# linnanwang/FastGen

Hardware: AMD Instinct MI355X
Metric: images/sec at 4-step distilled (DMD2) sampling (higher is better)
Workload: dtype fp32 (tensors, accumulate) with split-bf16 x3 MFMA conv products; 1 GPU; EDM CIFAR-10 32x32 SongUNet (55.7M params) DMD2 4-step 'sde' sampling, batch=512 per GPU; global_batch=512, sample_steps=4, parallelism=replicas x1 (no data-path collective), graph=True

## Files before the change

### fastgen_amd/_lib.py

```python
import ctypes
import os
from ctypes import POINTER, c_char_p, c_double, c_float, c_int, c_int64, c_size_t, c_uint64, c_void_p

_HERE = os.path.dirname(os.path.abspath(__file__))
LIB_PATH = os.path.join(_HERE, "libfastgen_amd.so")

FG_MAX_LEVELS = 8
FG_DTYPE_F32, FG_DTYPE_BF16, FG_DTYPE_BF16X3, FG_DTYPE_FP8 = 0, 1, 2, 3
DTYPE_NAMES = {"fp32": FG_DTYPE_F32, "bf16": FG_DTYPE_BF16, "bf16x3": FG_DTYPE_BF16X3, "fp8": FG_DTYPE_FP8}
FG_SAMPLE_SDE, FG_SAMPLE_ODE = 0, 1
SAMPLE_TYPES = {"sde": FG_SAMPLE_SDE, "ode": FG_SAMPLE_ODE}
FG_LOOP_X0, FG_LOOP_MEANFLOW, FG_LOOP_EULER = 0, 1, 2
LOOP_KINDS = {"x0": FG_LOOP_X0, "meanflow": FG_LOOP_MEANFLOW, "euler": FG_LOOP_EULER}
FG_SCHEDULE_EDM, FG_SCHEDULE_RF = 0, 1
FG_DROP_PRECOND_INPUT, FG_DROP_PRECOND_OUTPUT = 1, 2
FG_BWD_DECODER, FG_BWD_ENCODER, FG_BWD_EMBED = 1, 2, 4
FG_MODEL_SONGUNET, FG_MODEL_DHARIWAL = 0, 1
(FG_TRAIN_OP_HEAD_GRAD, FG_TRAIN_OP_STEM_OPERAND, FG_TRAIN_OP_INPUT_GRAD, FG_TRAIN_OP_ADD_NCHW_TO_NHWC, FG_TRAIN_OP_SILU_BWD, FG_TRAIN_OP_JVP_COEF,
 FG_TRAIN_OP_JVP_EMBED, FG_TRAIN_OP_JVP_INPUT, FG_TRAIN_OP_JVP_OUTPUT) = range(9)


class fg_edm_config(ctypes.Structure):
    _fields_ = [
        ("img_resolution", c_int), ("img_channels", c_int), ("label_dim", c_int), ("augment_dim", c_int),
# ... 16 lines not shown


class fg_dit_config(ctypes.Structure):
    _fields_ = [("input_size", c_int), ("patch_size", c_int), ("in_channels", c_int), ("hidden_size", c_int), ("depth", c_int),
                ("num_heads", c_int), ("mlp_hidden", c_int), ("embedding_rows", c_int), ("r_timestep", c_int), ("compute_dtype", c_int)]


class fg_wan_config(ctypes.Structure):
    _fields_ = [("num_heads", c_int), ("head_dim", c_int), ("in_channels", c_int), ("out_channels", c_int), ("text_dim", c_int),
                ("freq_dim", c_int), ("ffn_dim", c_int), ("num_layers", c_int), ("rope_max_seq_len", c_int), ("chunk_size", c_int),
                ("total_num_frames", c_int), ("eps", c_float), ("compute_dtype", c_int)]


class fg_wan_ext_config(ctypes.Structure):
    _fields_ = [("r_timestep", c_int), ("time_cond_diff", c_int)]


class fg_wan_i2v_config(ctypes.Structure):
    _fields_ = [("latent_channels", c_int), ("mask_channels", c_int), ("image_dim", c_int)]


class fg_wan_ti2v_config(ctypes.Structure):
    _fields_ = [("latent_channels", c_int)]


class fg_wan_vace_config(ctypes.Structure):
    _fields_ = [("vace_in_channels", c_int), ("num_vace_layers", c_int), ("vace_layers", c_int * 64)]


class fg_wan_block_taps(ctypes.Structure):
    _fields_ = [("attn1", c_void_p), ("x_attn1", c_void_p), ("attn2", c_void_p), ("x_attn2", c_void_p), ("x_ffn", c_void_p)]


class fg_dit_sampler_config(ctypes.Structure):
    _fields_ = [("t_scale", c_double), ("guidance_scale", c_double), ("use_sit_convention", c_int), ("time_cond_diff", c_int),
                ("net_pred_flow", c_int), ("schedule", c_int)]


class fg_wan_sampler_config(ctypes.Structure):
    _fields_ = [("t_scale", c_double), ("context_noise", c_double), ("net_pred_flow", c_int), ("schedule", c_int), ("prefill_frames", c_int)]


class fg_wan_guided_sampler_config(ctypes.Structure):
    _fields_ = [("t_scale", c_double), ("context_noise", c_double), ("guidance", c_int)]


class fg_attention_plan(ctypes.Structure):
    _fields_ = [("kernel", c_int), ("nsplit", c_int), ("t_cut", c_int), ("sample_major", c_int), ("refusal", c_int), ("grid", c_int64),
                ("scratch_bytes", c_size_t)]


class fg_edm_conv_plan(ctypes.Structure):
    _fields_ = [("kernel", c_int), ("stat_slots", c_int)]


FG_EDM_PACK_GENERIC, FG_EDM_PACK_WS, FG_EDM_PACK_X3WS, FG_EDM_PACK_X3SUB = range(4)
FG_EDM_CONV_GENERIC, FG_EDM_CONV_WS, FG_EDM_CONV_X3WS = 1, 2, 3
FG_EDM_PACK_STEM, FG_EDM_PACK_AUX = 0, 1


class fg_gemm_plan(ctypes.Structure):
    _fields_ = [("refusal", c_int), ("kernel", c_int), ("tile_n", c_int), ("epilogue", c_int), ("ksplit", c_int), ("xn", c_int), ("grid", c_int),
                ("lds_bytes", c_int), ("row0", c_int), ("rows", c_int), ("pieces", c_int)]


FG_FA_TILE128, FG_FA_TILE128_W3, FG_FA_TILE128_REG, FG_FA_WIDE, FG_FA_WIDE_CUT, FG_FA_SEQ72, FG_FA_TILE72, FG_FA_TILE72_W3 = range(1, 9)
FG_FA_REFUSE_ARG, FG_FA_REFUSE_OFFSET, FG_FA_REFUSE_PATH = 1, 2, 3
FG_GEMM_REG, FG_GEMM_PP, FG_GEMM_PP_NARROW, FG_GEMM_PP_SPLITK = range(1, 5)
FG_GEMM_EPI_TOK, FG_GEMM_EPI_HEADS, FG_GEMM_EPI_RAW, FG_GEMM_EPI_TOK32, FG_GEMM_EPI_SPLIT, FG_GEMM_EPI_HEADS32 = range(6)
FG_GEMM_REFUSE_ARG, FG_GEMM_REFUSE_OFFSET, FG_GEMM_REFUSE_FORM, FG_GEMM_REFUSE_PIECE = 1, 2, 3, 4


SIGNATURES = {
    "fg_last_error": (c_char_p, []),
    "fg_version": (c_char_p, []),
    "fg_graph_stats": (None, [POINTER(c_uint64), POINTER(c_uint64)]),
    "fg_edm_create": (c_int, [POINTER(fg_edm_config), POINTER(c_void_p)]),
    "fg_edm_destroy": (None, [c_void_p]),
    "fg_edm_num_params": (c_int, [c_void_p]),
    "fg_edm_param_info": (c_int, [c_void_p, c_int, POINTER(c_char_p), POINTER(c_int), POINTER(c_int64)]),
    "fg_edm_bind_param": (c_int, [c_void_p, c_char_p, c_void_p, c_int64]),
    "fg_edm_pack_weights": (c_int, [c_void_p, c_void_p]),
    "fg_edm_workspace_bytes": (c_size_t, [c_void_p, c_int]),
    "fg_edm_forward": (c_int, [c_void_p, c_void_p, c_void_p, c_void_p, c_void_p, c_void_p, c_void_p, c_int, c_void_p,
                               c_size_t, c_void_p]),
    "fg_edm_num_feature_taps": (c_int, [c_void_p]),
    "fg_edm_feature_info": (c_int, [c_void_p, c_int, POINTER(c_char_p), POINTER(c_int), POINTER(c_int)]),
    "fg_edm_forward_features": (c_int, [c_void_p, c_void_p, c_void_p, c_void_p, c_void_p, c_void_p, POINTER(c_void_p), c_int,
                                        c_void_p, c_size_t, c_void_p]),
    "fg_sampler_run": (c_int, [c_void_p, c_void_p, c_void_p, POINTER(c_double), c_int, c_int, c_int, c_void_p, c_uint64,
                               c_void_p, c_int, c_void_p, c_size_t, c_int, c_void_p]),
    "fg_edm_t_list": (c_int, [c_int, POINTER(c_double)]),
    "fg_rf_t_list": (c_int, [c_int, POINTER(c_double)]),
    "fg_edm_profile_begin": (c_int, [c_void_p]),
    "fg_edm_profile_end": (c_int, [c_void_p, POINTER(c_int64), POINTER(c_double), POINTER(c_double)]),
    "fg_edm_num_blocks": (c_int, [c_void_p]),
    "fg_edm_block_info": (c_int, [c_void_p, c_int, POINTER(c_char_p), POINTER(c_int), POINTER(c_int), POINTER(c_int),
                                  POINTER(c_int), POINTER(c_int)]),
    "fg_edm_run_block": (c_int, [c_void_p, c_int, c_void_p, c_int, c_void_p, c_int, c_void_p, c_void_p, c_int, c_void_p,
                                 c_size_t, c_void_p]),
    "fg_op_gn_coeffs": (c_int, [c_void_p, c_int, c_void_p, c_int, c_void_p, c_void_p, c_float, c_void_p, c_int, c_int, c_void_p]),
    "fg_op_adm_conv_pack_bytes": (c_size_t, [c_int, c_int, c_int, c_int]),
    "fg_op_adm_conv_pack": (c_int, [c_int, c_void_p, c_void_p, c_int, c_int, c_int, c_void_p]),
    "fg_op_adm_conv": (c_int, [c_int, c_int, c_void_p, c_int, c_void_p, c_int, c_int, c_int, c_int, c_int, c_void_p, c_int, c_void_p,
                               c_void_p, c_void_p, c_int, c_void_p, c_int, c_void_p]),
    "fg_op_adm_conv_ex": (c_int, [c_int, c_int, c_void_p, c_int, c_void_p, c_int, c_int, c_int, c_int, c_int, c_void_p, c_int, c_int, c_void_p,
# ... 130 lines not shown
    "fg_wan_create_ti2v": (c_int, [POINTER(fg_wan_config), POINTER(fg_wan_ext_config), POINTER(fg_wan_ti2v_config), POINTER(c_void_p)]),
    "fg_wan_set_first_frame": (c_int, [c_void_p, c_void_p, c_int, c_int, c_int, c_void_p]),
    "fg_wan_first_frame_read": (c_int, [c_void_p, c_void_p, c_void_p]),
    "fg_wan_create_vace": (c_int, [POINTER(fg_wan_config), POINTER(fg_wan_ext_config), POINTER(fg_wan_vace_config), POINTER(c_void_p)]),
    "fg_wan_set_vace_scale": (c_int, [c_void_p, POINTER(c_float), c_int, c_void_p]),
    "fg_wan_vace_context_workspace_bytes": (c_size_t, [c_void_p, c_int, c_int, c_int, c_int]),
    "fg_wan_set_vace_context": (c_int, [c_void_p, c_void_p, c_int, c_int, c_int, c_int, c_int, c_void_p, c_size_t, c_void_p]),
    "fg_wan_vace_context_read": (c_int, [c_void_p, c_void_p, c_void_p]),
    "fg_op_wan_vace_patch_embed": (c_int, [c_void_p, c_void_p, c_void_p, c_void_p, c_int, c_int, c_int, c_int, c_int, c_int, c_int, c_void_p]),
    "fg_op_wan_patch_embed": (c_int, [c_void_p, c_void_p, c_void_p, c_void_p, c_void_p, c_int, c_int, c_int, c_int, c_int, c_int, c_int, c_void_p]),
    "fg_op_wan_final": (c_int, [c_void_p, c_void_p, c_void_p, c_void_p, c_void_p, c_void_p, c_int, c_int, c_int, c_int, c_int, c_int, c_float, c_int,
                                c_void_p]),
    "fg_op_wan_dual_cross_attention": (c_int, [c_void_p, c_int, c_int64, c_void_p, c_void_p, c_int, c_int64, c_int, c_void_p, c_void_p, c_int,
                                               c_int64, c_int, c_void_p, c_int, c_int64, c_int, c_int, c_int, c_void_p]),
    "fg_disc_edm_num_params": (c_int, [c_int]),
    "fg_disc_edm_workspace_bytes": (c_size_t, [c_int, c_int]),
    "fg_disc_edm_run": (c_int, [c_void_p, c_int, c_void_p, c_void_p, c_void_p, c_void_p, c_void_p, c_int, c_void_p, c_size_t, c_void_p]),
    "fg_edm_jvp": (c_int, [c_void_p, c_void_p, c_void_p, c_void_p, c_void_p, c_void_p, c_void_p, c_void_p, c_void_p, c_void_p, c_int,
                           c_void_p, c_size_t, c_void_p]),
    "fg_edm_set_dropout": (c_int, [c_void_p, c_float, c_uint64]),
    "fg_op_gn_workspace_bytes": (c_size_t, [c_int, c_int]),
    "fg_op_gn_act": (c_int, [c_int, c_int, c_void_p, c_int, c_void_p, c_int, c_void_p, c_void_p, c_float, c_void_p, c_int, c_int, c_int,
                             c_float, ctypes.c_uint32, c_uint64, c_void_p, c_size_t, c_void_p]),
    "fg_op_gn_backward": (c_int, [c_int, c_int, c_void_p, c_int, c_void_p, c_int, c_void_p, c_int, c_void_p, c_void_p, c_float, c_void_p,
                                  c_void_p, c_void_p, c_int, c_float, c_void_p, c_void_p, c_int, c_int, c_int, c_int, c_float,
                                  ctypes.c_uint32, c_uint64, c_void_p, c_size_t, c_void_p]),
    "fg_op_gn_jvp": (c_int, [c_int, c_int, c_void_p, c_int, c_void_p, c_int, c_void_p, c_void_p, c_void_p, c_float, c_void_p, c_int, c_int,
                             c_float, ctypes.c_uint32, c_uint64, c_void_p, c_size_t, c_void_p]),
    "fg_op_attention_backward_workspace_bytes": (c_size_t, [c_int, c_int, c_int, c_int]),
    "fg_op_attention_backward": (c_int, [c_int, c_void_p, c_void_p, c_void_p, c_void_p, c_void_p, c_void_p, c_void_p, c_void_p, c_int, c_int,
                                         c_int, c_void_p, c_size_t, c_void_p]),
    "fg_op_attention_jvp": (c_int, [c_int, c_void_p, c_void_p, c_void_p, c_void_p, c_void_p, c_void_p, c_void_p, c_int, c_int, c_int,
                                    c_void_p, c_size_t, c_void_p]),
    "fg_op_colsum": (c_int, [c_int, c_void_p, c_int, c_int, c_void_p, c_int, c_int, c_float, c_int, c_void_p]),
    "fg_op_batchsum_add": (c_int, [c_void_p, c_void_p, c_void_p, c_int, c_int, c_int, c_void_p]),
    "fg_op_linear_backward": (c_int, [c_int, c_void_p, c_void_p, c_void_p, c_void_p, c_void_p, c_void_p, c_int, c_int, c_int, c_float, c_int,
                                      c_void_p]),
    "fg_op_dgrad_weights": (c_int, [c_void_p, c_void_p, c_int, c_int, c_int, c_int, c_void_p]),
    "fg_op_train_elementwise": (c_int, [c_int, c_int, c_void_p, c_void_p, c_void_p, c_void_p, c_void_p, c_void_p, c_int, c_int, c_int, c_int,
                                        c_double, c_double, c_int, c_void_p]),
    "fg_op_edm_conv_pack_bytes": (c_size_t, [c_int, c_int, c_int, c_int, c_int]),
    "fg_op_edm_conv_pack": (c_int, [c_int, c_int, c_void_p, c_void_p, c_int, c_int, c_int, c_int, c_void_p]),
    "fg_op_edm_conv_plan": (c_int, [c_int, c_int, c_int, c_int, c_int, c_int, c_int, c_int, c_int, c_int, c_int, c_int, c_int,
                                    POINTER(fg_edm_conv_plan)]),
    "fg_op_edm_conv": (c_int, [c_int, c_int, c_int, c_int, c_int, c_void_p, c_int, c_void_p, c_int, c_int, c_int, c_int, c_void_p, c_void_p,
                               c_void_p, c_void_p, c_void_p, c_int, c_void_p, c_int, c_float, c_void_p, c_int, c_void_p, c_void_p, c_void_p,
                               c_void_p, c_void_p]),
    "fg_op_edm_gn_finalize": (c_int, [c_void_p, c_int, c_int, c_void_p, c_int, c_int, c_void_p, c_void_p, c_float, c_void_p, c_void_p, c_int,
                                      c_int, c_void_p]),
    "fg_op_edm_gn_silu_pool": (c_int, [c_int, c_void_p, c_void_p, c_void_p, c_int, c_int, c_int, c_void_p]),
    "fg_op_edm_attention": (c_int, [c_int, c_void_p, c_void_p, c_void_p, c_void_p, c_int, c_int, c_void_p]),
    "fg_op_edm_attn_merge_weights": (c_int, [c_void_p, c_void_p, c_void_p, c_void_p, c_void_p, c_int, c_void_p]),
    "fg_op_edm_attention_merged": (c_int, [c_void_p, c_void_p, c_void_p, c_void_p, c_void_p, c_float, c_void_p, c_void_p, c_int, c_void_p]),
    "fg_op_edm_head_pack_bytes": (c_size_t, [c_int, c_int, c_int]),
    "fg_op_edm_stem": (c_int, [c_int, c_void_p, c_void_p, c_void_p, c_void_p, c_void_p, c_void_p, c_void_p, c_int, c_int, c_int, c_void_p]),
    "fg_op_edm_conv_in": (c_int, [c_int, c_void_p, c_void_p, c_void_p, c_void_p, c_void_p, c_int, c_int, c_int, c_int, c_void_p]),
    "fg_op_edm_aux_head": (c_int, [c_int, c_void_p, c_void_p, c_void_p, c_void_p, c_void_p, c_void_p, c_void_p, c_void_p, c_int, c_int, c_int,
                                   c_void_p]),
    "fg_op_edm_aux_out": (c_int, [c_int, c_void_p, c_void_p, c_void_p, c_void_p, c_void_p, c_void_p, c_void_p, c_int, c_int, c_int, c_int,
                                  c_void_p]),
    "fg_op_dropout_mask": (c_int, [c_void_p, c_int64, c_float, ctypes.c_uint32, c_uint64, c_void_p]),
    "fg_edm_set_augment": (c_int, [c_void_p, c_void_p]),
    "fg_edm_set_training": (c_int, [c_void_p, c_int]),
    "fg_op_images_to_u8": (c_int, [c_void_p, c_void_p, c_int64, c_int, c_int, c_int, c_void_p]),
    "fg_op_randn": (c_int, [c_void_p, c_int64, c_uint64, c_uint64, c_void_p]),
    "fg_op_attention": (c_int, [c_void_p, c_void_p, c_void_p, c_void_p, c_int, c_int, c_int, c_int, c_int, c_void_p]),
    "fg_op_attention_split": (c_int, [c_void_p, c_void_p, c_void_p, c_void_p, c_int, c_int, c_int, c_int, c_int, c_int, c_void_p]),
    "fg_op_attention_plan": (c_int, [c_int, c_int, c_int, c_int, c_int, c_int, c_int, c_int, c_int, POINTER(fg_attention_plan)]),
    "fg_op_attention_ex": (c_int, [c_void_p, c_int, c_int64, c_void_p, c_void_p, c_int, c_int64, c_void_p, c_int, c_int64, c_int, c_int, c_int,
                                   c_int, c_int, c_int, c_int, c_int, c_void_p]),
    "fg_op_dit_attention": (c_int, [c_int, c_void_p, c_void_p, c_void_p, c_void_p, c_int, c_int, c_int, c_int, c_size_t, c_int, c_void_p]),
    "fg_op_gemm_plan": (c_int, [c_int, c_int, c_int, c_int, c_int, c_int, c_size_t, c_int, c_int, c_int, c_int, POINTER(fg_gemm_plan)]),
    "fg_op_gemm_bf16": (c_int, [c_void_p, c_void_p, c_void_p, c_void_p, c_int, c_int, c_int, c_int, c_void_p, c_int, c_int, c_void_p,
                                c_int, c_void_p]),
    "fg_op_quant_rows_fp8": (c_int, [c_int, c_void_p, c_void_p, c_void_p, c_int64, c_int, c_void_p]),
    "fg_op_gemm_fp8": (c_int, [c_void_p, c_void_p, c_void_p, c_void_p, c_int, c_int, c_int, c_int, c_void_p, c_int, c_int, c_void_p,
                               c_int, c_void_p, c_void_p, c_void_p]),
    "fg_op_dit_ln_modulate_fp8": (c_int, [c_void_p, c_void_p, c_int, c_int, c_int, c_void_p, c_void_p, c_int, c_int, c_int, c_void_p]),
    "fg_op_gemm_x3": (c_int, [c_void_p, c_void_p, c_void_p, c_void_p, c_int, c_int, c_int, c_int, c_void_p, c_int, c_int, c_void_p,
                              c_int, c_void_p]),
}

_lib = None


def lib():
    global _lib
    if _lib is None:
        if not os.path.exists(LIB_PATH):
            raise RuntimeError(
                f"{LIB_PATH} not found: build it with `python -c 'import __graft_entry__ as g; g.build()'` "
                "(or `make -C fastgen_amd/csrc`).  fastgen_amd has no non-HIP fallback.")
        L = ctypes.CDLL(LIB_PATH)
        for name, (res, args) in SIGNATURES.items():
            fn = getattr(L, name)
            fn.restype = res
            fn.argtypes = args
        _lib = L
    return _lib


def graph_stats():
    c, n = c_uint64(), c_uint64()
    lib().fg_graph_stats(ctypes.byref(c), ctypes.byref(n))
    return c.value, n.value

# ... 10 lines not shown
```

### fastgen_amd/csrc/attn.hip

```cpp
#include <cstdlib>
#include "common.h"
#include "misc.h"

namespace {

template <typename T>
struct PFrag;
template <>
struct PFrag<__bf16> {
    static __device__ __forceinline__ Frag8<__bf16> make(const f32x16& p, int s) {
        Frag8<__bf16> f;
#pragma unroll
        for (int j = 0; j < 8; ++j) f.v[j] = (__bf16)p[8 * s + j];
        return f;
    }
};
template <>
struct PFrag<float> {
    static __device__ __forceinline__ Frag8<float> make(const f32x16& p, int s) {
        Frag8<float> f;
        f.lo = f32x4{p[8 * s + 0], p[8 * s + 1], p[8 * s + 2], p[8 * s + 3]};
        f.hi = f32x4{p[8 * s + 4], p[8 * s + 5], p[8 * s + 6], p[8 * s + 7]};
        return f;
    }
// ... 225 lines not shown
#pragma unroll
            for (int j = 0; j < 8; ++j) pf[kt][s2].v[j] = (__bf16)(st[kt][8 * s2 + j] * inv);
        __builtin_amdgcn_sched_barrier(0);
    }

    __builtin_amdgcn_sched_barrier(0);
    __bf16* obase = out + ((size_t)n * Tn + q0) * D + r;
#pragma unroll 1
    for (int dg = 0; dg < 2; ++dg) {
        f32x16 o[4];
#pragma unroll
        for (int d = 0; d < 4; ++d)
#pragma unroll
            for (int i = 0; i < 16; ++i) o[d][i] = 0.f;
        asm volatile("" ::: "memory");
        stage_v(0, smem);
        __syncthreads();
#pragma unroll
        for (int t = 0; t < 4; ++t) {
            const char* cur = smem + (t & 1) * ATT_BUF;
            if (t + 1 < 4) stage_v(t + 1, smem + ((t + 1) & 1) * ATT_BUF);
#pragma unroll
            for (int sub = 0; sub < 2; ++sub)
#pragma unroll
                for (int s2 = 0; s2 < 2; ++s2)
#pragma unroll
                    for (int d = 0; d < 4; ++d) {
                        const char* p = cur + ((dg * 4 + d) * 32 + r) * VPITCH + (sub * 32 + 16 * s2 + 4 * h) * 2;
                        const bf16x4 lo = *reinterpret_cast<const bf16x4*>(p);
                        const bf16x4 hi = *reinterpret_cast<const bf16x4*>(p + 16);
                        Frag8<__bf16> vf;
                        vf.v = bf16x8{lo[0], lo[1], lo[2], lo[3], hi[0], hi[1], hi[2], hi[3]};
                        mma16(o[d], pf[t * 2 + sub][s2], vf);
                    }
            __syncthreads();
            __builtin_amdgcn_sched_barrier(0);
        }
#pragma unroll
        for (int d = 0; d < 4; ++d)
#pragma unroll
            for (int i = 0; i < 16; ++i) obase[(size_t)acc_row(i, h) * D + (dg * 4 + d) * 32] = (__bf16)o[d][i];
    }
}

constexpr int X3_KP = 272, X3_VP = 136;
constexpr int X3_PLANE = 64 * X3_KP;
constexpr int X3_BUF = 2 * X3_PLANE;

struct AttnMerge {
    const float2* ab;
    const float* bp;
    float2* stats;
    float scale;
};

template <bool MRG>
__global__ __launch_bounds__(256, 2) void attention_x3_lds_kernel(const float* __restrict__ q, const float* __restrict__ k,
                                                                  const float* __restrict__ vt, float* __restrict__ out, int B,
                                                                  AttnMerge mg) {
    constexpr int Tn = 256, D = 256;
    extern __shared__ __attribute__((aligned(16))) char smem[];
    const int tid = threadIdx.x, lane = tid & 63, wave = tid >> 6;
    const int r = lane & 31, h = lane >> 5;
    const int n = blockIdx.x >> 1;
    const int q0 = (blockIdx.x & 1) * 128 + wave * 32;

    auto stage_k = [&](int s, char* buf) {
        const float* src = k + ((size_t)n * Tn + (s & 3) * 64) * D + (s >> 2) * 128;
        f32x4 cf[4];
        if constexpr (MRG) {
            const f32x4* cp = reinterpret_cast<const f32x4*>(mg.ab + (size_t)n * D + (s >> 2) * 128 + (tid & 15) * 8);
#pragma unroll
            for (int j = 0; j < 4; ++j) cf[j] = cp[j];
        }
#pragma unroll
        for (int b2 = 0; b2 < 2; ++b2) {
#pragma unroll
            for (int i = b2 * 2; i < b2 * 2 + 2; ++i) {
                const int idx = tid + 256 * i, row = idx >> 4, c = idx & 15;
                float x[8];
                widen8(load_frag(src + (size_t)row * D + c * 8), x);
                if constexpr (MRG) {
#pragma unroll
                    for (int j = 0; j < 8; ++j) x[j] = fmaf(x[j], cf[j >> 1][2 * (j & 1)], cf[j >> 1][2 * (j & 1) + 1]);
                }
                bf16x8 hi, lo;
                split8(x, hi, lo);
                *reinterpret_cast<bf16x8*>(buf + row * X3_KP + c * 16) = hi;
                *reinterpret_cast<bf16x8*>(buf + X3_PLANE + row * X3_KP + c * 16) = lo;
            }
            __builtin_amdgcn_sched_barrier(0);
        }
    };
    auto stage_v = [&](int s, char* buf) {
        const float* src = vt + ((size_t)n * D + (s >> 2) * 128) * Tn + (s & 3) * 64;
#pragma unroll
        for (int b2 = 0; b2 < 2; ++b2) {
#pragma unroll
            for (int i = b2 * 2; i < b2 * 2 + 2; ++i) {
                const int idx = tid + 256 * i, row = idx >> 3, c = idx & 7;
                float x[8];
                widen8(load_frag(src + (size_t)row * Tn + c * 8), x);
                bf16x8 hi, lo;
                split8(x, hi, lo);
                bf16x4* dh = reinterpret_cast<bf16x4*>(buf + row * X3_VP + c * 16);
                dh[0] = bf16x4{hi[0], hi[1], hi[2], hi[3]};
// ... 70 lines not shown
    }

    float* obase = out + ((size_t)n * Tn + q0) * D + r;
    stage_v(0, smem);
    __syncthreads();
    f32x16 o[4];
#pragma unroll
    for (int s = 0; s < 8; ++s) {
        const char* cur = smem + (s & 1) * X3_BUF;
        if ((s & 3) == 0) {
#pragma unroll
            for (int d = 0; d < 4; ++d)
#pragma unroll
                for (int i = 0; i < 16; ++i) o[d][i] = 0.f;
        }
        if (s + 1 < 8) stage_v(s + 1, smem + ((s + 1) & 1) * X3_BUF);
#pragma unroll
        for (int sub = 0; sub < 2; ++sub)
#pragma unroll
            for (int s2 = 0; s2 < 2; ++s2)
#pragma unroll
                for (int d = 0; d < 4; ++d) {
                    const char* p = cur + (d * 32 + r) * X3_VP + (sub * 32 + 16 * s2 + 4 * h) * 2;
                    const bf16x4 a0 = *reinterpret_cast<const bf16x4*>(p), a1 = *reinterpret_cast<const bf16x4*>(p + 16);
                    const bf16x4 b0 = *reinterpret_cast<const bf16x4*>(p + X3_PLANE), b1 = *reinterpret_cast<const bf16x4*>(p + X3_PLANE + 16);
                    Frag8<bf16x3> vf;
                    vf.hi = bf16x8{a0[0], a0[1], a0[2], a0[3], a1[0], a1[1], a1[2], a1[3]};
                    vf.lo = bf16x8{b0[0], b0[1], b0[2], b0[3], b1[0], b1[1], b1[2], b1[3]};
                    mma16(o[d], pf[(s & 3) * 2 + sub][s2], vf);
                }
        __syncthreads();
        __builtin_amdgcn_sched_barrier(0);
        if ((s & 3) == 3) {
            if constexpr (MRG) {
                const float* xbase = k + ((size_t)n * Tn + q0) * D + r;
#pragma unroll
                for (int d = 0; d < 4; ++d) {
                    const int col = ((s >> 2) * 4 + d) * 32;
                    const float bias = mg.bp[col + r];
                    float sv = 0.f, qv = 0.f;
#pragma unroll
                    for (int i = 0; i < 16; ++i) {
                        const size_t off = (size_t)acc_row(i, h) * D + col;
                        const float v = (o[d][i] + bias + xbase[off]) * mg.scale;
                        obase[off] = v;
                        sv += v;
                        qv += v * v;
                    }
                    if (mg.stats) {
                        sv += __shfl_xor(sv, 32), qv += __shfl_xor(qv, 32);
                        sv += __shfl_xor(sv, 1), qv += __shfl_xor(qv, 1);
                        sv += __shfl_xor(sv, 2), qv += __shfl_xor(qv, 2);
                        if (h == 0 && (r & 3) == 0)
                            mg.stats[((size_t)n * 8 + (blockIdx.x & 1) * 4 + wave) * (D / 4) + ((col + r) >> 2)] = make_float2(sv, qv);
                    }
                }
            } else {
#pragma unroll
                for (int d = 0; d < 4; ++d)
#pragma unroll
                    for (int i = 0; i < 16; ++i) obase[(size_t)acc_row(i, h) * D + ((s >> 2) * 4 + d) * 32] = o[d][i];
            }
        }
    }
}

__global__ void attn_merge_weights_kernel(const float* __restrict__ qkv_w, const float* __restrict__ qkv_b, const float* __restrict__ proj_w,
                                          float* __restrict__ w_out, float* __restrict__ b_out, int C) {
    const int o = blockIdx.x % C;
    const bool val = blockIdx.x >= C;
    for (int i = threadIdx.x; i <= C; i += blockDim.x) {
        double acc = 0.0;
        for (int c = 0; c < C; ++c) {
            const double l = val ? proj_w[(size_t)o * C + c] : qkv_w[(size_t)(3 * c + 1) * C + o];
            const int row = 3 * c + (val ? 2 : 0);
            acc += l * (double)(i < C ? qkv_w[(size_t)row * C + i] : qkv_b[row]);
        }
        if (i < C)
            w_out[(size_t)blockIdx.x * C + i] = (float)acc;
        else
            b_out[blockIdx.x] = (float)acc;
    }
}

template <bool MRG>
int x3_lds_prepare() {
    static bool done[16] = {};
    const int dev = fg_device_slot();
    if (dev < 0) return (int)hipErrorInvalidDevice;
    if (!done[dev]) {
        hipError_t e = hipFuncSetAttribute(reinterpret_cast<const void*>(attention_x3_lds_kernel<MRG>), hipFuncAttributeMaxDynamicSharedMemorySize, 2 * X3_BUF);
        if (e != hipSuccess) return (int)e;
        done[dev] = true;
    }
    return 0;
}

}

int launch_attn_merge_weights(const float* qkv_w, const float* qkv_b, const float* proj_w, float* w_out, float* b_out, int C, hipStream_t s) {
    hipLaunchKernelGGL(attn_merge_weights_kernel, dim3(2 * C), dim3(256), 0, s, qkv_w, qkv_b, proj_w, w_out, b_out, C);
    return (int)hipGetLastError();
}

int launch_attention_merged(const float* qm, const float* x_mid, const float2* ab, const float* vmt, const float* bp, float scale, float* out,
                            float2* stats, int B, hipStream_t s) {
    const int rc = x3_lds_prepare<true>();
    if (rc || !qm) return rc;
    hipLaunchKernelGGL(attention_x3_lds_kernel<true>, dim3(B * 2), dim3(256), 2 * X3_BUF, s, qm, x_mid, vmt, out, B, AttnMerge{ab, bp, stats, scale});
    return (int)hipGetLastError();
}

int launch_attention(int dtype, const void* q, const void* k, const void* vt, void* out, int B, int T, hipStream_t s) {
    if (T != 256 && T != 64) return (int)hipErrorInvalidValue;
    const int nt = T / 32;
    const int waves = B * nt;
    dim3 grid((waves + 3) / 4), block(256);
    if (dtype == 1 && nt == 8) {
        static bool attr_done_dev[16] = {};
        const int dev = fg_device_slot();
        if (dev < 0) return (int)hipErrorInvalidDevice;
        bool& attr_done = attr_done_dev[dev];
        if (!attr_done) {
            hipError_t e = hipFuncSetAttribute(reinterpret_cast<const void*>(attention_lds_kernel), hipFuncAttributeMaxDynamicSharedMemorySize, 2 * ATT_BUF);
            if (e != hipSuccess) return (int)e;
            attr_done = true;
        }
        if (!q) return 0;
        hipLaunchKernelGGL(attention_lds_kernel, dim3(B * 2), block, 2 * ATT_BUF, s, (const __bf16*)q, (const __bf16*)k, (const __bf16*)vt, (__bf16*)out, B);
        return (int)hipGetLastError();
    }
    static const bool x3_lds = [] {
        const char* e = getenv("FASTGEN_AMD_ATTN_X3_LDS");
        return !(e && e[0] == '0');
    }();
    if (dtype == 2 && nt == 8 && x3_lds) {
        const int rc = x3_lds_prepare<false>();
        if (rc || !q) return rc;
        hipLaunchKernelGGL(attention_x3_lds_kernel<false>, dim3(B * 2), block, 2 * X3_BUF, s, (const float*)q, (const float*)k, (const float*)vt, (float*)out, B,
                           AttnMerge{});
        return (int)hipGetLastError();
    }
    if (!q) return 0;
    if (dtype == 2) {
        if (nt == 8)
            hipLaunchKernelGGL((attention_kernel<bf16x3, 8>), grid, block, 0, s, (const float*)q, (const float*)k, (const float*)vt, (float*)out, B);
        else
            hipLaunchKernelGGL((attention_kernel<bf16x3, 2>), grid, block, 0, s, (const float*)q, (const float*)k, (const float*)vt, (float*)out, B);
    } else if (dtype) {
        if (nt == 8)
            hipLaunchKernelGGL((attention_kernel<__bf16, 8>), grid, block, 0, s, (const __bf16*)q, (const __bf16*)k, (const __bf16*)vt, (__bf16*)out, B);
        else
            hipLaunchKernelGGL((attention_kernel<__bf16, 2>), grid, block, 0, s, (const __bf16*)q, (const __bf16*)k, (const __bf16*)vt, (__bf16*)out, B);
    } else {
        if (nt == 8)
            hipLaunchKernelGGL((attention_kernel<float, 8>), grid, block, 0, s, (const float*)q, (const float*)k, (const float*)vt, (float*)out, B);
        else
            hipLaunchKernelGGL((attention_kernel<float, 2>), grid, block, 0, s, (const float*)q, (const float*)k, (const float*)vt, (float*)out, B);
    }
    return (int)hipGetLastError();
}
```

### fastgen_amd/csrc/conv.h

```cpp
#pragma once
#include <hip/hip_runtime.h>

struct ConvArgs {
    const void* src1;
    const void* src2;
    int C1, C2;
    int Hs, Ws;
    int H, W;
    int B;
    const float2* ab;
    const void* wpack;
    const void* wpack_ws;
    const float* bias;
    const float* temb;
    int temb_stride;
    const void* resid;
    int rshift = 0;
    float scale;
    void* out;
    int Cout;
    float2* stats;
    int dbg;
    void* q_out;
    void* k_out;
    void* vt_out;
    const float* gate = nullptr;
    int gate_stride = 0;
    int act = 0;
    int heads = 0, head_dim = 0;
    size_t heads_lo_off = 0;
};

enum { PRO_NONE = 0, PRO_GN = 1, PRO_GN_SILU = 2 };
enum { RES_NONE = 0, RES_DOWN = 1, RES_UP = 2, RES_SUBPIX = 3 };
enum { OUT_NHWC = 0, OUT_QKV = 1, OUT_TOK = 2, OUT_HEADS = 3, OUT_QV = 4 };

int launch_conv_fused(int dtype, int ks, int pro, int res, int outmode, const ConvArgs& a, hipStream_t stream);
int conv_stat_slots(int W);
bool conv_ws_supported(int dtype, int ks, int pro, int res, int outmode, const ConvArgs& a);
bool conv_ws_enabled();
int launch_conv_ws(int res, const ConvArgs& a, hipStream_t stream, bool prepare_only, int pro = PRO_GN_SILU);
bool conv_ws_shape_ok(int dtype, int cout, int cin, int res);
int launch_pack_conv_weights_ws(const float* w_oihw, void* wpack_ws, int cout, int cin, hipStream_t stream);
bool conv_x3ws_supported(int ks, int pro, int res, int outmode, const ConvArgs& a);
bool conv_x3ws_shape_ok(int cout, int cin, int res);
int conv_x3ws_stat_slots(int W, int res);
int launch_conv_x3ws(int res, const ConvArgs& a, hipStream_t stream, bool prepare_only, int pro = PRO_GN_SILU);
int launch_pack_conv_weights_x3ws(const float* w_oihw, void* wpack_ws, int cout, int cin, hipStream_t stream);
int launch_pack_conv_weights_x3sub(const float* w_oihw, void* wpack_sub, int cout, int cin, hipStream_t stream);
int conv_subpix_mode();
int conv_launch_stat_slots(int dtype, int ks, int pro, int res, int outmode, const ConvArgs& a);
int launch_conv_ws_debug(const ConvArgs& a, int abl, hipStream_t stream);
int launch_conv_debug(int dtype, const ConvArgs& a, hipStream_t stream);
int conv_prepare_all(int dtype);
size_t conv_pack_elems(int cout, int cin, int ks);
int launch_pack_conv_weights(int dtype, const float* w_oihw, void* wpack, int cout, int cin, int ks, int qkv_perm,
                             hipStream_t stream);
```

### fastgen_amd/csrc/conv.hip

```cpp
#include "common.h"
#include "conv.h"
#include <stdlib.h>
#include <string.h>

#include <type_traits>

namespace {

constexpr int PITCH = 144;
constexpr int NTHR = 256;

template <int KS, int LOGW>
struct Geom {
    static constexpr int W = 1 << LOGW;
    static constexpr int LOGTW = (LOGW == 5) ? 4 : LOGW;
    static constexpr int TW = 1 << LOGTW;
    static constexpr int LOGTH = 3;
    static constexpr int TH = 1 << LOGTH;
    static constexpr int IMGS = 128 / (TH * TW);
    static constexpr int TCOLS = W / TW;
    static constexpr int TPI = (IMGS > 1) ? 1 : (W / TH) * TCOLS;
    static constexpr int PAD = KS / 2;
    static constexpr int HW_ = TW + 2 * PAD;
    static constexpr int HH_ = TH + 2 * PAD;
// ... 535 lines not shown
        if (res == RES_NONE) return launch_w<T, 3, PRO_GN_SILU, RES_NONE, OUT_NHWC>(a, s);
        if (res == RES_UP) return launch_w<T, 3, PRO_GN_SILU, RES_UP, OUT_NHWC>(a, s);
    }
    if (ks == 3 && pro == PRO_NONE && res == RES_NONE) return launch_w<T, 3, PRO_NONE, RES_NONE, OUT_NHWC>(a, s);
    if (ks == 1 && pro == PRO_NONE) {
        if (res == RES_NONE) return launch_w<T, 1, PRO_NONE, RES_NONE, OUT_NHWC>(a, s);
        if (res == RES_DOWN) return launch_w<T, 1, PRO_NONE, RES_DOWN, OUT_NHWC>(a, s);
        if (res == RES_UP) return launch_w<T, 1, PRO_NONE, RES_UP, OUT_NHWC>(a, s);
    }
    return (int)hipErrorInvalidValue;
}

int dispatch_t(int dtype, int ks, int pro, int res, int outmode, const ConvArgs& a, hipStream_t s) {
    switch (dtype) {
        case 0: return launch_t<float>(ks, pro, res, outmode, a, s);
        case 1: return launch_t<__bf16>(ks, pro, res, outmode, a, s);
        case 2: return launch_t<bf16x3>(ks, pro, res, outmode, a, s);
    }
    return (int)hipErrorInvalidValue;
}

}

int launch_conv_debug(int dtype, const ConvArgs& a, hipStream_t stream) {
    if (dtype != 1 || a.W != 32) return (int)hipErrorInvalidValue;
    g_debug_extra_lds = (a.dbg & 16) ? 48 * 1024 : 0;
    switch (a.dbg & 15) {
        case 0: return launch_one<__bf16, 3, PRO_GN_SILU, RES_NONE, 5, OUT_NHWC, 0>(a, stream);
        case 1: return launch_one<__bf16, 3, PRO_GN_SILU, RES_NONE, 5, OUT_NHWC, 1>(a, stream);
        case 2: return launch_one<__bf16, 3, PRO_GN_SILU, RES_NONE, 5, OUT_NHWC, 2>(a, stream);
        case 3: return launch_one<__bf16, 3, PRO_GN_SILU, RES_NONE, 5, OUT_NHWC, 3>(a, stream);
        case 4: return launch_one<__bf16, 3, PRO_GN_SILU, RES_NONE, 5, OUT_NHWC, 4>(a, stream);
        case 5: return launch_one<__bf16, 3, PRO_GN_SILU, RES_NONE, 5, OUT_NHWC, 5>(a, stream);
        case 6: return launch_one<__bf16, 3, PRO_GN_SILU, RES_NONE, 5, OUT_NHWC, 6>(a, stream);
        case 7: return launch_one<__bf16, 3, PRO_GN_SILU, RES_NONE, 5, OUT_NHWC, 7>(a, stream);
    }
    return (int)hipErrorInvalidValue;
}

int launch_conv_fused(int dtype, int ks, int pro, int res, int outmode, const ConvArgs& a, hipStream_t stream) {
    const int kc = dtype == 1 ? DT<__bf16>::KC : DT<float>::KC;
    if (a.H != a.W || (a.W != 8 && a.W != 16 && a.W != 32)) return (int)hipErrorInvalidValue;
    const bool tok = outmode == OUT_TOK || outmode == OUT_HEADS;
    if ((a.C1 % kc) || (a.C2 % kc) || (a.Cout % (tok ? 64 : 256)) || a.B <= 0) return (int)hipErrorInvalidValue;
    if (outmode == OUT_HEADS && (a.heads <= 0 || (a.head_dim % 4) || a.Cout != 3 * a.heads * a.head_dim || ((a.heads * a.head_dim) % 64) ||
                                 !a.q_out || !a.k_out || !a.vt_out))
        return (int)hipErrorInvalidValue;
    if (res == RES_NONE && (a.Hs != a.H || a.Ws != a.W)) return (int)hipErrorInvalidValue;
    if (res == RES_DOWN && (a.Hs != 2 * a.H || a.Ws != 2 * a.W)) return (int)hipErrorInvalidValue;
    if ((res == RES_UP || res == RES_SUBPIX) && (2 * a.Hs != a.H || 2 * a.Ws != a.W)) return (int)hipErrorInvalidValue;
    if (pro != PRO_NONE && !a.ab) return (int)hipErrorInvalidValue;
    if (outmode == OUT_QKV && (a.Cout != 768 || a.W > 16)) return (int)hipErrorInvalidValue;
    if (outmode == OUT_QV && (a.Cout != 512 || a.W != 16 || dtype != 2 || !a.q_out || !a.vt_out)) return (int)hipErrorInvalidValue;
    if (conv_ws_enabled() && conv_ws_supported(dtype, ks, pro, res, outmode, a)) return launch_conv_ws(res, a, stream, false, pro);
    if (dtype == 2 && conv_ws_enabled() && conv_x3ws_supported(ks, pro, res, outmode, a)) return launch_conv_x3ws(res, a, stream, false, pro);
    if (res == RES_SUBPIX || a.rshift) return (int)hipErrorInvalidValue;
    return dispatch_t(dtype, ks, pro, res, outmode, a, stream);
}

bool conv_ws_enabled() {
    static const bool on = [] {
        const char* e = getenv("FASTGEN_AMD_CONV_WS");
        return !(e && e[0] == '0');
    }();
    return on;
}

int conv_subpix_mode() {
    static const int mode = [] {
        const char* e = getenv("FASTGEN_AMD_CONV_SUBPIX");
        if (e && e[0] == '0') return 0;
        return (e && !strcmp(e, "skip")) ? 1 : 2;
    }();
    return mode;
}

int conv_launch_stat_slots(int dtype, int ks, int pro, int res, int outmode, const ConvArgs& a) {
    if (dtype == 2 && conv_ws_enabled() && conv_x3ws_supported(ks, pro, res, outmode, a)) return conv_x3ws_stat_slots(a.W, res);
    return conv_stat_slots(a.W);
}

int conv_stat_slots(int W) { return W == 32 ? Geom<3, 5>::TPI : (W == 16 ? Geom<3, 4>::TPI : Geom<3, 3>::TPI); }

int conv_prepare_all(int dtype) {
    g_prepare_only = true;
    int rc = 0;
    ConvArgs a{};
    a.B = 1;
    a.Cout = 256;
    const int ws[3] = {8, 16, 32};
    for (int wi = 0; wi < 3 && !rc; ++wi) {
        a.W = a.H = ws[wi];
        for (int res = 0; res < 3 && !rc; ++res) {
            if (res != RES_DOWN)
                rc = dispatch_t(dtype, 3, PRO_GN_SILU, res, OUT_NHWC, a, nullptr);
            if (!rc) rc = dispatch_t(dtype, 1, PRO_NONE, res, OUT_NHWC, a, nullptr);
        }
        if (!rc) rc = dispatch_t(dtype, 3, PRO_NONE, RES_NONE, OUT_NHWC, a, nullptr);
        if (!rc && a.W <= 16) rc = dispatch_t(dtype, 1, PRO_GN, RES_NONE, OUT_QKV, a, nullptr);
        if (!rc && a.W == 16 && dtype == 2) rc = dispatch_t(dtype, 1, PRO_GN, RES_NONE, OUT_QV, a, nullptr);
        if (!rc && a.W == 16) rc = dispatch_t(dtype, 1, PRO_NONE, RES_NONE, OUT_TOK, a, nullptr);
        if (!rc && a.W == 16) rc = dispatch_t(dtype, 1, PRO_NONE, RES_NONE, OUT_HEADS, a, nullptr);
    }
    g_prepare_only = false;
    if (!rc && dtype == 2) {
        ConvArgs w{};
        for (int res : {RES_NONE, RES_UP})
            for (int ww : {32, 16, 8}) {
                if (ww == 8 && res != RES_NONE) continue;
                w.W = w.H = ww;
                if (!rc) rc = launch_conv_x3ws(res, w, nullptr, true, PRO_GN_SILU);
                if (!rc && res == RES_NONE) rc = launch_conv_x3ws(res, w, nullptr, true, PRO_NONE);
            }
        for (int ws_ : {16, 8}) {
            w.Ws = w.Hs = ws_;
            w.W = w.H = 2 * ws_;
            if (!rc) rc = launch_conv_x3ws(RES_SUBPIX, w, nullptr, true, PRO_GN_SILU);
        }
    }
    if (!rc && dtype == 1) {
        ConvArgs w{};
        for (int res : {RES_NONE, RES_UP}) {
            w.W = w.H = 32;
            if (!rc) rc = launch_conv_ws(res, w, nullptr, true);
            if (res == RES_NONE) {
                w.C1 = -128;
                if (!rc) rc = launch_conv_ws(res, w, nullptr, true);
                w.C1 = 0;
            }
            w.W = w.H = 16;
            if (!rc) rc = launch_conv_ws(res, w, nullptr, true);
        }
// ... 19 lines not shown
```

### fastgen_amd/csrc/conv_ws3.hip

```cpp
#include "common.h"
#include "conv.h"

namespace {

constexpr int X3_NTHR = 768;
constexpr int X3_KC = 32;
constexpr int X3_PA = 16;
constexpr int X3_PLANE = 3072;
constexpr int X3_ABUF = 8 * X3_PLANE;
constexpr int X3_RING = 4;
constexpr int X3_HOFF = 128 * 512;
constexpr int X3_LDS = X3_HOFF + X3_RING * X3_ABUF;
constexpr int X3_TAPB = 2048;

template <int LOGW>
struct X3Geom {
    static constexpr int W = 1 << LOGW;
    static constexpr int TW = 16, TH = 8;
    static constexpr int IPT = LOGW == 3 ? 2 : 1;
    static constexpr int TCOLS = LOGW == 3 ? 1 : W / TW;
    static constexpr int TPI = LOGW == 3 ? 1 : (W / TH) * TCOLS;
    static constexpr int HW_ = LOGW == 3 ? 2 * W + 3 : TW + 2, HH_ = TH + 2;
    static constexpr int HALO_PIX = HW_ * HH_;
    static constexpr int RS = HW_ * X3_PA;
    static_assert(HALO_PIX * X3_PA <= X3_PLANE && HALO_PIX <= 192, "one halo plane; three producer passes of 64 pixels");
};

__device__ __forceinline__ void x3_barrier() {
    asm volatile("s_waitcnt lgkmcnt(0)\n\ts_barrier" ::: "memory");
}

struct X3Frag {
    bf16x8 hi, lo;
};

template <int RES, int LOGW, int PRO>
__global__ __launch_bounds__(X3_NTHR) void conv3_x3ws_kernel(const ConvArgs a, const int ntiles) {
    using G = X3Geom<LOGW>;
    constexpr bool SUB = RES == RES_SUBPIX;
    constexpr int NTAP = SUB ? 4 : 9;
    constexpr int RN = SUB ? 4 : 3;
    constexpr int NQ = 4 * NTAP;
    constexpr int X3_STEPB = NTAP * X3_TAPB;
    extern __shared__ __attribute__((aligned(16))) char smem[];
    char* const hbuf = smem;
    char* const ring = smem + X3_HOFF;

    const int tid = threadIdx.x;
    const int lane = tid & 63;
    const int wave = __builtin_amdgcn_readfirstlane(tid >> 6);
    const int Cin = a.C1 + a.C2;
    const int nchunk = Cin / X3_KC;
    const int G8 = (int)gridDim.x >> 3;
    const int wg = ((gridDim.x & 7) == 0) ? ((int)blockIdx.x & 7) * G8 + ((int)blockIdx.x >> 3) : (int)blockIdx.x;
    const int gstride = (int)gridDim.x;
    const int my_tiles = (ntiles - wg + gstride - 1) / gstride;
    const int S = my_tiles * nchunk;
    const int NSTEP = S + 3;
    const int H = SUB ? a.Hs : a.H;

    if (wave < 8) {
        const int grp = wave >> 2, wl = wave & 3;
        const int col = lane & 15, g4 = lane >> 4;
        const size_t wstride = (size_t)nchunk * NTAP * 1024;
        const __amdgpu_buffer_rsrc_t wrs = __builtin_amdgcn_make_buffer_rsrc(
            const_cast<__bf16*>(reinterpret_cast<const __bf16*>(a.wpack_ws) + (size_t)(grp * 8 + wl * 2) * wstride), 0, 0x7fffffff,
            0x00020000);
        const int wvoff = lane * 16;
        const int wsb = (int)(wstride * 2);
        const int wphb = SUB ? 16 * wsb : 0;
        int tcur = wg;
        auto load_w = [&](int byte_off) -> X3Frag {
            X3Frag f;
            f.hi = __builtin_bit_cast(bf16x8, __builtin_amdgcn_raw_buffer_load_b128(wrs, wvoff, byte_off, 0));
            f.lo = __builtin_bit_cast(bf16x8, __builtin_amdgcn_raw_buffer_load_b128(wrs, wvoff, byte_off + 1024, 0));
            return f;
        };
        X3Frag wq[RN][2];
#pragma unroll
        for (int j = 0; j < RN; ++j)
#pragma unroll
            for (int nt = 0; nt < 2; ++nt) wq[j][nt] = load_w((tcur & 3) * wphb + nt * wsb + (SUB ? j : 3 * j) * X3_TAPB);

        f32x4 acc[8][2];
#pragma unroll
        for (int m = 0; m < 8; ++m)
#pragma unroll
            for (int nt = 0; nt < 2; ++nt) acc[m][nt] = f32x4{0.f, 0.f, 0.f, 0.f};

// ... 178 lines not shown
            off2[i] = (pix * (unsigned)a.C2 + oct * 8) * 4u;
        }
        abn = a.ab + (size_t)n * Cin;
    };
    auto stage_load = [&](Staged& st, int t, int c32) __attribute__((always_inline)) {
        if (c32 == 0) tile_setup(t);
        const bool first = c32 * X3_KC < a.C1;
        const char* base = first ? reinterpret_cast<const char*>(src1) + c32 * (X3_KC * 4)
                                 : reinterpret_cast<const char*>(src2) + (c32 * X3_KC - a.C1) * 4;
#pragma unroll
        for (int i = 0; i < 3; ++i) {
            const char* p = base + (first ? off1[i] : off2[i]);
            st.raw[i][0] = *reinterpret_cast<const f32x4*>(p);
            st.raw[i][1] = *reinterpret_cast<const f32x4*>(p + 16);
        }
        if (PRO == PRO_NONE) return;
        const float2* p = abn + c32 * X3_KC + oct * 8;
#pragma unroll
        for (int j = 0; j < 8; j += 2) {
            const f32x4 q = *reinterpret_cast<const f32x4*>(p + j);
            st.ab[j] = make_float2(q[0], q[1]);
            st.ab[j + 1] = make_float2(q[2], q[3]);
        }
    };
    auto stage_store = [&](const Staged& st, char* abuf) __attribute__((always_inline)) {
#pragma unroll
        for (int i = 0; i < 3; ++i) {
            float v[8];
#pragma unroll
            for (int j = 0; j < 8; ++j) {
                v[j] = st.raw[i][j >> 2][j & 3];
                if (PRO != PRO_NONE) v[j] = silu_f<true>(fmaf(v[j], st.ab[j].x, st.ab[j].y));
            }
            bf16x8 hi, lo;
            split8(v, hi, lo);
            typedef __attribute__((ext_vector_type(4))) unsigned u32x4;
            u32x4 wh = __builtin_bit_cast(u32x4, hi), wl_ = __builtin_bit_cast(u32x4, lo);
#pragma unroll
            for (int j = 0; j < 4; ++j) {
                wh[j] = valid[i] ? wh[j] : 0u;
                wl_[j] = valid[i] ? wl_[j] : 0u;
            }
            if (i < 2 || third) {
                *reinterpret_cast<u32x4*>(abuf + hlds[i]) = wh;
                *reinterpret_cast<u32x4*>(abuf + hlds[i] + 4 * X3_PLANE) = wl_;
            }
        }
    };

    const int chq = lane & 31, psub = lane >> 5;
    float* const out = reinterpret_cast<float*>(a.out);
    const float* const resid = reinterpret_cast<const float*>(a.resid);
    const bool has_resid = __builtin_amdgcn_readfirstlane(resid != nullptr);
    auto retire_half = [&](int t, int half) __attribute__((always_inline)) {
        int n, slot, row0, col0;
        tile_coord(t, n, slot, row0, col0);
        const int co = half * 128 + chq * 4;
        const int nimg = G::IPT == 2 ? min(2, a.B - n) : 1;
        f32x4 radd[G::IPT];
#pragma unroll
        for (int k = 0; k < G::IPT; ++k) {
            radd[k] = f32x4{0.f, 0.f, 0.f, 0.f};
            if (a.bias) radd[k] = *reinterpret_cast<const f32x4*>(a.bias + co);
            const int nk = G::IPT == 2 ? min(n + k, a.B - 1) : n;
            if (a.temb) radd[k] += *reinterpret_cast<const f32x4*>(a.temb + (size_t)nk * a.temb_stride + co);
            radd[k] *= a.scale;
        }
        constexpr int OW = SUB ? 2 * G::W : G::W, OST = SUB ? 2 : 1;
        const int ph = t & 3;
        const size_t tb = SUB ? (((size_t)n * (2 * H) + 2 * row0 + (ph >> 1)) * OW + 2 * col0 + (ph & 1)) * 256 + co
                              : (((size_t)n * H + row0) * G::W + col0) * 256 + co;
        const int rs = (SUB || G::IPT == 2) ? 0 : a.rshift;
        const size_t rtb = (SUB || G::IPT == 2) ? tb : (((size_t)n * (H >> rs) + (row0 >> rs)) * (G::W >> rs) + (col0 >> rs)) * 256 + co;
        float ssum[G::IPT] = {}, ssq[G::IPT] = {};
#pragma unroll 1
        for (int grp8 = 0; grp8 < 2; ++grp8) {
            f32x4 rr[8], dv[8];
            unsigned go[8];
#pragma unroll
            for (int j = 0; j < 8; ++j) {
                const int px = pw * 32 + 2 * (grp8 * 8 + j) + psub;
                unsigned rgo;
                if (G::IPT == 2) {
                    go[j] = (unsigned)((((j >> 2) * OW + OST * (px >> 4)) * OW + OST * (px & 7)) * 256);
                    rgo = go[j];
                } else {
                    go[j] = (unsigned)((OST * (px >> 4) * OW + OST * (px & 15)) * 256);
                    rgo = SUB ? go[j] : (unsigned)((((px >> 4) >> rs) * (G::W >> rs) + ((px & 15) >> rs)) * 256);
                }
                rr[j] = f32x4{0.f, 0.f, 0.f, 0.f};
                if (has_resid && (G::IPT == 1 || (j >> 2) < nimg)) rr[j] = *reinterpret_cast<const f32x4*>(resid + rtb + rgo);
                dv[j] = *reinterpret_cast<const f32x4*>(hbuf + px * 512 + ((chq ^ (px & 7)) << 4));
            }
#pragma unroll
            for (int j = 0; j < 8; ++j) {
                const int k = G::IPT == 2 ? j >> 2 : 0;
                if (G::IPT == 2 && k >= nimg) continue;
                f32x4 v;
#pragma unroll
                for (int e = 0; e < 4; ++e) v[e] = fmaf(dv[j][e], a.scale, radd[k][e]);
                if (has_resid) {
#pragma unroll
                    for (int e = 0; e < 4; ++e) v[e] = fmaf(rr[j][e], a.scale, v[e]);
                }
                *reinterpret_cast<f32x4*>(out + tb + go[j]) = v;
                ssum[k] += (v[0] + v[1]) + (v[2] + v[3]);
                ssq[k] += (v[0] * v[0] + v[1] * v[1]) + (v[2] * v[2] + v[3] * v[3]);
            }
        }
#pragma unroll
        for (int k = 0; k < G::IPT; ++k) {
            ssum[k] += __shfl_xor(ssum[k], 32);
            ssq[k] += __shfl_xor(ssq[k], 32);
            const size_t sl = SUB ? ((size_t)(n + k) * G::TPI + slot) * 4 + ph : (size_t)(n + k) * G::TPI + slot;
            if (a.stats && psub == 0 && k < nimg) a.stats[(sl * 4 + pw) * 64 + half * 32 + chq] = make_float2(ssum[k], ssq[k]);
        }
    };

    auto advance = [&](int& t, int& cc) {
        if (++cc == nchunk) {
            cc = 0;
            t += gstride;
        }
    };
    Staged st;
    int t1 = wg, c1 = 0;
    stage_load(st, t1, c1);
    stage_store(st, ring);
    advance(t1, c1);
    x3_barrier();
    int sa = 0;
    for (int s = 0; s < NSTEP; ++s) {
        const bool more = s + 1 < S;
        if (more) stage_load(st, t1, c1);
        if (sa == 0 && s >= nchunk && s <= S) retire_half(wg + (s / nchunk - 1) * gstride, 0);
        if (sa == 2 % nchunk && s - 2 >= nchunk && s - 2 <= S && (s - 2) % nchunk == 0) retire_half(wg + ((s - 2) / nchunk - 1) * gstride, 1);
        if (more) {
            stage_store(st, ring + ((s + 1) & 3) * X3_ABUF);
            advance(t1, c1);
        }
        if (++sa == nchunk) sa = 0;
        x3_barrier();
    }
}

__global__ void pack_conv_weights_x3ws_kernel(const float* __restrict__ w, __bf16* __restrict__ out, int cout, int cin) {
    const size_t total = (size_t)cout * cin * 9;
    const int nstep = cin / X3_KC;
    for (size_t idx = (size_t)blockIdx.x * blockDim.x + threadIdx.x; idx < total; idx += (size_t)gridDim.x * blockDim.x) {
        size_t t = idx;
        const int j = t % 8; t /= 8;
        const int lane = t % 64; t /= 64;
        const int tap = t % 9; t /= 9;
        const int step = t % nstep; t /= nstep;
        const int n16 = (int)t;
        const int co = n16 * 16 + (lane & 15);
        const int ci = step * X3_KC + 8 * (lane >> 4) + j;
        const float v = w[((size_t)co * cin + ci) * 9 + tap];
        const __bf16 hi = (__bf16)v;
        const size_t o = (idx / 512) * 1024 + (idx % 512);
        out[o] = hi;
        out[o + 512] = (__bf16)(v - (float)hi);
    }
}

__global__ void pack_conv_weights_x3sub_kernel(const float* __restrict__ w, __bf16* __restrict__ out, int cout, int cin) {
    const size_t total = (size_t)16 * cout * cin;
    const int nstep = cin / X3_KC, ng = cout / 16;
    for (size_t idx = (size_t)blockIdx.x * blockDim.x + threadIdx.x; idx < total; idx += (size_t)gridDim.x * blockDim.x) {
        size_t t = idx;
        const int j = t % 8; t /= 8;
        const int lane = t % 64; t /= 64;
        const int tap = t % 4; t /= 4;
        const int step = t % nstep; t /= nstep;
        const int n16 = t % ng; t /= ng;
        const int py = (int)t >> 1, px = (int)t & 1, ty = tap >> 1, tx = tap & 1;
        const int co = n16 * 16 + (lane & 15);
        const int ci = step * X3_KC + 8 * (lane >> 4) + j;
        const int ky0 = py ? 2 * ty : ty, ky1 = py ? ty + 1 : 2 * ty;
        const int kx0 = px ? 2 * tx : tx, kx1 = px ? tx + 1 : 2 * tx;
        const float* wp = w + ((size_t)co * cin + ci) * 9;
        float v = 0.f;
        for (int ky = ky0; ky <= ky1; ++ky)
            for (int kx = kx0; kx <= kx1; ++kx) v += wp[ky * 3 + kx];
        const __bf16 hi = (__bf16)v;
        const size_t o = (idx / 512) * 1024 + (idx % 512);
        out[o] = hi;
        out[o + 512] = (__bf16)(v - (float)hi);
    }
}

int g_x3_cus[16] = {};

template <int RES, int LOGW, int PRO>
int launch_x3_one(const ConvArgs& a, hipStream_t stream, bool prepare_only) {
    using G = X3Geom<LOGW>;
    auto kern = conv3_x3ws_kernel<RES, LOGW, PRO>;
    int dev = 0;
    if (hipGetDevice(&dev) != hipSuccess || dev < 0 || dev >= 16) return (int)hipErrorInvalidDevice;
    static bool attr_done[16] = {};
    if (!attr_done[dev]) {
        hipError_t e = hipFuncSetAttribute(reinterpret_cast<const void*>(kern), hipFuncAttributeMaxDynamicSharedMemorySize, X3_LDS);
        if (e != hipSuccess) return (int)e;
        attr_done[dev] = true;
    }
    if (!g_x3_cus[dev]) {
        int n = 0;
        if (hipDeviceGetAttribute(&n, hipDeviceAttributeMultiprocessorCount, dev) != hipSuccess || n <= 0) return (int)hipErrorUnknown;
        g_x3_cus[dev] = n;
    }
    if (prepare_only) return 0;
    const int ntiles = (a.B * G::TPI + G::IPT - 1) / G::IPT * (RES == RES_SUBPIX ? 4 : 1);
    const int grid = ntiles < g_x3_cus[dev] ? ntiles : g_x3_cus[dev];
    hipLaunchKernelGGL(kern, dim3(grid), dim3(X3_NTHR), X3_LDS, stream, a, ntiles);
    return (int)hipGetLastError();
}

}

int conv_x3ws_stat_slots(int W, int res) {
    if (res == RES_SUBPIX) return (W == 32 ? X3Geom<4>::TPI : X3Geom<3>::TPI) * 16;
    return (W == 32 ? X3Geom<5>::TPI : W == 16 ? X3Geom<4>::TPI : X3Geom<3>::TPI) * 4;
}

bool conv_x3ws_shape_ok(int cout, int cin, int res) {
    return cout == 256 && (res == 32 || res == 16 || res == 8) && (cin % X3_KC) == 0 && cin / X3_KC >= 4;
}

bool conv_x3ws_supported(int ks, int pro, int res, int outmode, const ConvArgs& a) {
    const int cin = a.C1 + a.C2;
    const size_t src_bytes = (size_t)a.B * a.Hs * a.Ws * (size_t)(a.C1 > a.C2 ? a.C1 : a.C2) * 4;
    if (src_bytes >= (1ull << 32)) return false;
    if (res == RES_SUBPIX)
        return ks == 3 && outmode == OUT_NHWC && pro == PRO_GN_SILU && a.ab && a.H == a.W && a.Hs == a.Ws && a.H == 2 * a.Hs && (a.Ws == 16 || a.Ws == 8) &&
               conv_x3ws_shape_ok(a.Cout, cin, a.Ws) && (a.C1 % X3_KC) == 0 && a.wpack_ws && !a.rshift;
    if (ks != 3 || outmode != OUT_NHWC || a.H != a.W || !conv_x3ws_shape_ok(a.Cout, cin, a.W) || (a.C1 % X3_KC) || !a.wpack_ws) return false;
    if (a.W == 8 && res != RES_NONE) return false;
    if (a.rshift && (a.rshift != 1 || !a.resid || a.W == 8 || res != RES_NONE)) return false;
    if (pro == PRO_NONE) return res == RES_NONE && a.Hs == a.H && a.Ws == a.W;
    return pro == PRO_GN_SILU && (res == RES_NONE || res == RES_UP) && a.ab != nullptr;
}

int launch_conv_x3ws(int res, const ConvArgs& a, hipStream_t stream, bool prepare_only, int pro) {
    if (res == RES_SUBPIX) {
        if (pro != PRO_GN_SILU || (a.Ws != 16 && a.Ws != 8)) return (int)hipErrorInvalidValue;
        return a.Ws == 16 ? launch_x3_one<RES_SUBPIX, 4, PRO_GN_SILU>(a, stream, prepare_only) : launch_x3_one<RES_SUBPIX, 3, PRO_GN_SILU>(a, stream, prepare_only);
    }
    if (pro == PRO_NONE || a.W == 8) {
        if (res != RES_NONE) return (int)hipErrorInvalidValue;
        if (a.W == 8)
            return pro == PRO_NONE ? launch_x3_one<RES_NONE, 3, PRO_NONE>(a, stream, prepare_only)
                                   : launch_x3_one<RES_NONE, 3, PRO_GN_SILU>(a, stream, prepare_only);
        return a.W == 32 ? launch_x3_one<RES_NONE, 5, PRO_NONE>(a, stream, prepare_only) : launch_x3_one<RES_NONE, 4, PRO_NONE>(a, stream, prepare_only);
    }
    if (a.W == 32)
        return res == RES_UP ? launch_x3_one<RES_UP, 5, PRO_GN_SILU>(a, stream, prepare_only) : launch_x3_one<RES_NONE, 5, PRO_GN_SILU>(a, stream, prepare_only);
    return res == RES_UP ? launch_x3_one<RES_UP, 4, PRO_GN_SILU>(a, stream, prepare_only) : launch_x3_one<RES_NONE, 4, PRO_GN_SILU>(a, stream, prepare_only);
}

int launch_pack_conv_weights_x3ws(const float* w_oihw, void* wpack_ws, int cout, int cin, hipStream_t stream) {
    const size_t total = (size_t)cout * cin * 9;
    const int grid = (int)((total + 255) / 256 < 4096 ? (total + 255) / 256 : 4096);
    hipLaunchKernelGGL(pack_conv_weights_x3ws_kernel, dim3(grid), dim3(256), 0, stream, w_oihw, (__bf16*)wpack_ws, cout, cin);
    return (int)hipGetLastError();
}

int launch_pack_conv_weights_x3sub(const float* w_oihw, void* wpack_sub, int cout, int cin, hipStream_t stream) {
    const size_t total = (size_t)16 * cout * cin;
    const int grid = (int)((total + 255) / 256 < 4096 ? (total + 255) / 256 : 4096);
    hipLaunchKernelGGL(pack_conv_weights_x3sub_kernel, dim3(grid), dim3(256), 0, stream, w_oihw, (__bf16*)wpack_sub, cout, cin);
    return (int)hipGetLastError();
}
```

### fastgen_amd/csrc/engine.hip

```cpp
#include <hip/hip_runtime.h>

#include <atomic>
#include <cmath>
#include <cstdarg>
#include <cstdio>
#include <cstdlib>
#include <cstring>
#include <string>
#include <map>
#include <vector>

#include "../../include/fastgen_amd.h"
#include "common.h"
#include "adm.h"
#include "edm2.h"
#include "conv.h"
#include "misc.h"

namespace {

thread_local std::string g_err;

int fail(int code, const char* fmt, ...) {
    char buf[512];
// ... 31 lines not shown
    int temb_off = 0;
    int norm0_w = -1, norm0_b = -1, conv0_w = -1, conv0_b = -1, aff_w = -1, aff_b = -1, norm1_w = -1, norm1_b = -1,
        conv1_w = -1, conv1_b = -1, skip_w = -1, skip_b = -1, norm2_w = -1, norm2_b = -1, qkv_w = -1, qkv_b = -1,
        proj_w = -1, proj_b = -1, w = -1, b = -1;
    void *p_conv0 = nullptr, *p_conv1 = nullptr, *p_skip = nullptr, *p_qkv = nullptr, *p_proj = nullptr;
    void *p_conv0_ws = nullptr, *p_conv1_ws = nullptr;
    void* p_conv0_sub = nullptr;
    int tap = -1;
    float* qkv_bias = nullptr;
    void* p_qv = nullptr;
    float* qv_bias = nullptr;
    void* p_aux = nullptr;
    void* p_stem = nullptr;
};

struct Arena {
    char* base = nullptr;
    size_t off = 0, cap = 0;
    bool dry = false;
    void* take(size_t bytes) {
        off = (off + 255) & ~(size_t)255;
        void* p = dry ? nullptr : base + off;
        off += bytes;
        return p;
    }
    template <typename T>
    T* get(size_t n) {
        return reinterpret_cast<T*>(take(n * sizeof(T)));
    }
};

struct Act {
    void* p = nullptr;
    float2* st = nullptr;
    int slots = 0;
};

struct AdmWs {
    float *e2 = nullptr, *lab = nullptr;
    float2* part = nullptr;
    std::vector<float*> skip;
    float *xa = nullptr, *xb = nullptr, *h = nullptr, *s = nullptr, *t1 = nullptr, *qkv = nullptr, *a = nullptr;
};
struct AdmNet;

struct Workspace {
    AdmWs adm;
    float *coef, *emb0, *emb1, *emb, *temb;
    float2 *ab0, *ab1, *ab2;
    float2 *mr0 = nullptr, *mr1 = nullptr, *mr2 = nullptr;
    void* a1d = nullptr;
    bool infer = false;
    DropArgs drop;
    std::vector<Act> skip;
    Act xa, xb, h, xattn;
    void *sbuf, *aout, *pool;
    void *cvt1, *cvt2;
    void *q, *k, *vt;
    float *x, *x_pred, *eps;
    double* tl;
    uint64_t* seed;
};

struct BlockStash {
    void* h = nullptr;
    float2 *ab0 = nullptr, *ab1 = nullptr, *ab2 = nullptr, *mr0 = nullptr, *mr1 = nullptr, *mr2 = nullptr;
    void *xattn = nullptr, *q = nullptr, *k = nullptr, *vt = nullptr, *aout = nullptr;
    void* a1d = nullptr;
    uint32_t index = 0;
};
struct TrainStash {
    std::vector<Act> dec_store;
    std::vector<BlockStash> blocks;
    float2* aux_ab = nullptr;
    float2* aux_mr = nullptr;
    float* raw_out = nullptr;
};

struct HandleBase {
    std::vector<Param> params;
    std::string name_prefix;
    std::vector<void*> owned;
    bool packed = false, device_ready = false;

    HandleBase() = default;
    HandleBase(const HandleBase&) = delete;
    HandleBase& operator=(const HandleBase&) = delete;
    ~HandleBase() {
        for (void* p : owned) (void)hipFree(p);
    }
    int find(const std::string& n) const {
        for (size_t i = 0; i < params.size(); ++i)
            if (params[i].name == n) return (int)i;
        return -1;
    }
    int add(const std::string& n, std::initializer_list<int64_t> shp) {
        Param p;
        p.name = name_prefix + n;
        p.ndim = (int)shp.size();
        p.numel = 1;
        int i = 0;
        for (int64_t s : shp) {
            p.shape[i++] = s;
            p.numel *= s;
        }
        params.push_back(p);
// ... 444 lines not shown
        if (b.kind == K_BLOCK) h->blocks.push_back(&b);
    for (auto& b : h->dec)
        if (b.kind == K_BLOCK) h->blocks.push_back(&b);
}

int check_supported(const fg_edm* h) {
    const fg_edm_config& c = h->cfg;
    const int kc = h->dtype ? 64 : 32;
    if (c.img_resolution != 32 && c.img_resolution != 16 && c.img_resolution != 8)
        return fail(FG_EINVAL, "img_resolution %d unsupported (8, 16, 32)", c.img_resolution);
    if ((c.img_resolution >> (c.num_levels - 1)) < 8)
        return fail(FG_EINVAL, "lowest resolution %d < 8 unsupported", c.img_resolution >> (c.num_levels - 1));
    if (c.img_channels > 4) return fail(FG_EINVAL, "img_channels %d > 4 unsupported", c.img_channels);
    for (const Block* b : h->blocks) {
        if (b->cout != 256) return fail(FG_EINVAL, "%s: out_channels %d unsupported (kernels are tiled for 256)", b->key.c_str(), b->cout);
        if (b->cin % kc || (b->cin - b->skip_c) % kc)
            return fail(FG_EINVAL, "%s: in_channels %d not a multiple of %d", b->key.c_str(), b->cin, kc);
        if (b->attn && b->res_out > 16) return fail(FG_EINVAL, "%s: attention at %dx%d unsupported", b->key.c_str(), b->res_out, b->res_out);
    }
    return FG_OK;
}

void adm_build_layout(fg_edm* h);
int adm_check_supported(const fg_edm* h);
size_t adm_plan_workspace(const fg_edm* h, int B, Arena& A, Workspace& w);
int adm_pack_weights(fg_edm* h, hipStream_t s);
int adm_forward(fg_edm* h, const float* x_t, const double* t, int t_stride, const float* labels, float* out, int B, Workspace& w,
                hipStream_t s);
int adm_refuse(const fg_edm* h, const char* what) {
    return fail(FG_EINVAL, "%s is not implemented for DhariwalUNet (forward and sampling only)", what);
}

size_t plan_workspace(const fg_edm* h, int B, Arena& A, Workspace& w) {
    if (h->adm) return adm_plan_workspace(h, B, A, w);
    const fg_edm_config& c = h->cfg;
    const size_t tsz = h->dtype ? 2 : 4;
    const int R = c.img_resolution;
    size_t max_act = 0;
    int max_c = 0, max_attn_hw = 0;
    for (const Block& b : h->enc) max_act = std::max(max_act, (size_t)b.res_out * b.res_out * b.cout);
    for (const Block* b : h->blocks) {
        max_act = std::max(max_act, (size_t)b->res_out * b->res_out * b->cout);
        max_c = std::max(max_c, std::max(b->cin, b->cout));
        if (b->attn) max_attn_hw = std::max(max_attn_hw, b->res_out * b->res_out);
    }
    w.coef = A.get<float>(5 * (size_t)B);
    w.emb0 = A.get<float>((size_t)B * h->cond_ch);
    w.emb1 = A.get<float>((size_t)B * h->emb_ch);
    w.emb = A.get<float>((size_t)B * h->emb_ch);
    w.temb = A.get<float>((size_t)B * h->temb_total);
    w.ab0 = A.get<float2>((size_t)B * max_c);
    w.ab1 = A.get<float2>((size_t)B * max_c);
    w.ab2 = A.get<float2>((size_t)B * max_c);
    const size_t st_elems = (size_t)B * 32 * 64;
    auto act = [&](size_t elems, size_t st_n) {
        Act a;
        a.p = A.take(elems * tsz);
        a.st = A.get<float2>(st_n);
        return a;
    };
    w.skip.clear();
    for (const Block& b : h->enc)
        w.skip.push_back(act((size_t)B * b.res_out * b.res_out * b.cout,
                             (b.kind == K_STEM && b.p_stem) ? (size_t)B * b.res_out * b.res_out : st_elems));
    w.xa = act((size_t)B * max_act, st_elems);
    w.xb = act((size_t)B * max_act, st_elems);
    w.h = act((size_t)B * max_act, st_elems);
    w.sbuf = A.take((size_t)B * max_act * tsz);
    w.pool = A.take((size_t)B * max_act * tsz);
    w.cvt1 = A.take((size_t)B * max_act * 4 * tsz);
    w.cvt2 = A.take((size_t)B * max_act * 4 * tsz);
    w.xattn = act((size_t)B * max_attn_hw * 256, st_elems);
    w.aout = A.take((size_t)B * max_attn_hw * 256 * tsz);
    w.q = A.take((size_t)B * max_attn_hw * 256 * tsz);
    w.k = A.take((size_t)B * max_attn_hw * 256 * tsz);
    w.vt = A.take((size_t)B * max_attn_hw * 256 * tsz);
    const size_t img = (size_t)B * c.img_channels * R * R;
    w.x = A.get<float>(img);
    w.x_pred = A.get<float>(img);
    w.eps = A.get<float>(img);
    w.tl = A.get<double>(ScalarRing::kDoubles);
    w.seed = A.get<uint64_t>(8);
    return (A.off + 255) & ~(size_t)255;
}

int conv_launch(fg_edm* h, int ks, int pro, int res, int outmode, const ConvArgs& a, hipStream_t s) {
    const bool timed = h->prof_on && ks == 3 && res == RES_NONE && a.W == 32 && outmode == OUT_NHWC;
    hipEvent_t e0 = nullptr, e1 = nullptr;
    if (timed) {
        if (hipEventCreate(&e0) != hipSuccess || hipEventCreate(&e1) != hipSuccess) return (int)hipErrorUnknown;
        (void)hipEventRecord(e0, s);
    }
    const int rc = launch_conv_fused(h->cmode, ks, pro, res, outmode, a, s);
    if (timed) {
        (void)hipEventRecord(e1, s);
        h->prof_ev.push_back(e0);
        h->prof_ev.push_back(e1);
        h->prof_flops += 2.0 * a.B * a.H * a.W * (double)a.Cout * 9.0 * (a.C1 + a.C2);
    }
    return rc;
}

const float kSkipScale = (float)std::sqrt(0.5);
const float kBlockEps = 1e-6f;

int norm_coeffs(int dtype, const Act& x1, int c1, const Act& x2, int c2, const float* gamma, const float* beta, float2* ab,
                int B, int hw, hipStream_t s, float2* mr = nullptr) {
    if (x1.st && (!c2 || x2.st))
        HIP_TRY(launch_gn_finalize(x1.st, c1, x1.slots, c2 ? x2.st : nullptr, c2, c2 ? x2.slots : 0, gamma, beta, kBlockEps, ab, B, hw, s, mr));
    else
        HIP_TRY(launch_gn_coeffs(dtype, x1.p, c1, c2 ? x2.p : nullptr, c2, gamma, beta, kBlockEps, ab, B, hw, s, mr));
    return FG_OK;
}

void use_stash(Workspace& w, const BlockStash& st) {
    w.h.p = st.h;
    w.ab0 = st.ab0, w.ab1 = st.ab1, w.mr0 = st.mr0, w.mr1 = st.mr1;
    w.a1d = st.a1d;
    w.drop.block = st.index;
    if (st.xattn) {
        w.xattn.p = st.xattn;
        w.ab2 = st.ab2, w.mr2 = st.mr2;
        w.q = st.q, w.k = st.k, w.vt = st.vt, w.aout = st.aout;
    }
}
int block_index(const fg_edm* h, const Block* b) {
    for (size_t i = 0; i < h->blocks.size(); ++i)
        if (h->blocks[i] == b) return (int)i;
    return -1;
}

bool attn_merge_enabled() {
    static const bool on = [] {
        const char* e = getenv("FASTGEN_AMD_ATTN_MERGE");
        return !(e && e[0] == '0');
    }();
    return on;
}

int run_block(fg_edm* h, const Block& b, const Act& x1, int c1, const Act& x2, int c2, const float* temb, Act& out, int B,
              Workspace& w, hipStream_t s) {
    if (c1 + c2 != b.cin) return fail(FG_EINVAL, "%s: got %d+%d input channels, expected %d", b.key.c_str(), c1, c2, b.cin);
    const int hw_in = b.res_in * b.res_in, hw = b.res_out * b.res_out;
    const int res_mode = b.down ? RES_DOWN : (b.up ? RES_UP : RES_NONE);
    const int slots = conv_stat_slots(b.res_out);
    int rc;
    if ((rc = norm_coeffs(h->dtype, x1, c1, x2, c2, h->P(b.norm0_w), h->P(b.norm0_b), w.ab0, B, hw_in, s, w.mr0))) return rc;
    ConvArgs a{};
    a.src1 = x1.p; a.src2 = c2 ? x2.p : nullptr; a.C1 = c1; a.C2 = c2;
    a.Hs = a.Ws = b.res_in; a.H = a.W = b.res_out; a.B = B;
    a.ab = w.ab0; a.wpack = b.p_conv0; a.wpack_ws = b.p_conv0_ws; a.bias = h->P(b.conv0_b);
    a.temb = temb + b.temb_off; a.temb_stride = h->temb_total;
    a.resid = nullptr; a.scale = 1.0f; a.out = w.h.p; a.Cout = b.cout; a.stats = w.h.st;
    const bool x3_up = b.up && w.infer && !w.a1d && h->cmode == FG_DTYPE_BF16X3 && conv_ws_enabled();
    bool sub0 = false;
    if (x3_up && conv_subpix_mode() == 2 && b.p_conv0_sub) {
        ConvArgs p = a;
        p.wpack_ws = b.p_conv0_sub;
        sub0 = conv_x3ws_supported(3, PRO_GN_SILU, RES_SUBPIX, OUT_NHWC, p);
    }
    if (sub0) {
        a.wpack_ws = b.p_conv0_sub;
        w.h.slots = conv_launch_stat_slots(h->cmode, 3, PRO_GN_SILU, RES_SUBPIX, OUT_NHWC, a);
        HIP_TRY(conv_launch(h, 3, PRO_GN_SILU, RES_SUBPIX, OUT_NHWC, a, s));
    } else if (b.down && !c2) {
        HIP_TRY(launch_gn_silu_pool(h->dtype, x1.p, w.ab0, w.pool, B, b.res_out, b.res_out, c1, s));
        a.src1 = w.pool; a.Hs = a.Ws = b.res_out; a.ab = nullptr;
        w.h.slots = conv_launch_stat_slots(h->cmode, 3, PRO_NONE, RES_NONE, OUT_NHWC, a);
        HIP_TRY(conv_launch(h, 3, PRO_NONE, RES_NONE, OUT_NHWC, a, s));
    } else {
        w.h.slots = conv_launch_stat_slots(h->cmode, 3, PRO_GN_SILU, res_mode, OUT_NHWC, a);
        HIP_TRY(conv_launch(h, 3, PRO_GN_SILU, res_mode, OUT_NHWC, a, s));
    }
    ConvArgs d{};
    d.src1 = w.h.p; d.C1 = b.cout; d.Hs = d.Ws = d.H = d.W = b.res_out; d.B = B;
    d.ab = w.ab1; d.wpack = b.p_conv1; d.wpack_ws = b.p_conv1_ws; d.bias = h->P(b.conv1_b);
    d.scale = kSkipScale; d.Cout = b.cout;
    const void* resid = x1.p;
    if (b.has_skip) {
        bool low = false;
        if (x3_up && conv_subpix_mode() >= 1) {
            ConvArgs p = d;
            p.resid = w.sbuf; p.rshift = 1;
            low = conv_x3ws_supported(3, PRO_GN_SILU, RES_NONE, OUT_NHWC, p);
        }
        ConvArgs k{};
        k.src1 = x1.p; k.src2 = c2 ? x2.p : nullptr; k.C1 = c1; k.C2 = c2;
        k.Hs = k.Ws = b.res_in; k.H = k.W = low ? b.res_in : b.res_out; k.B = B;
        k.wpack = b.p_skip; k.bias = h->P(b.skip_b); k.scale = 1.0f; k.out = w.sbuf; k.Cout = b.cout;
        HIP_TRY(conv_launch(h, 1, PRO_NONE, low ? RES_NONE : res_mode, OUT_NHWC, k, s));
        resid = w.sbuf;
        d.rshift = low ? 1 : 0;
    }
    HIP_TRY(launch_gn_finalize(w.h.st, b.cout, w.h.slots, nullptr, 0, 0, h->P(b.norm1_w), h->P(b.norm1_b), kBlockEps, w.ab1, B, hw, s, w.mr1));
    Act& x_mid = b.attn ? w.xattn : out;
    d.resid = resid; d.out = x_mid.p; d.stats = x_mid.st;
    if (w.a1d) {
        HIP_TRY(launch_gn_act(h->dtype, 0, w.h.p, b.cout, nullptr, 0, w.ab1, w.a1d, B, b.res_out, 0, s, w.drop));
        d.src1 = w.a1d; d.ab = nullptr;
        x_mid.slots = conv_launch_stat_slots(h->cmode, 3, PRO_NONE, RES_NONE, OUT_NHWC, d);
        HIP_TRY(conv_launch(h, 3, PRO_NONE, RES_NONE, OUT_NHWC, d, s));
    } else {
        x_mid.slots = conv_launch_stat_slots(h->cmode, 3, PRO_GN_SILU, RES_NONE, OUT_NHWC, d);
        HIP_TRY(conv_launch(h, 3, PRO_GN_SILU, RES_NONE, OUT_NHWC, d, s));
    }
    if (b.attn) {
        HIP_TRY(launch_gn_finalize(x_mid.st, b.cout, x_mid.slots, nullptr, 0, 0, h->P(b.norm2_w), h->P(b.norm2_b), kBlockEps, w.ab2, B, hw, s, w.mr2));
        ConvArgs q{};
        q.src1 = x_mid.p; q.C1 = b.cout; q.Hs = q.Ws = q.H = q.W = b.res_out; q.B = B;
        if (w.infer && !w.a1d && h->cmode == FG_DTYPE_BF16X3 && hw == 256 && b.cout == 256 && b.p_qv && attn_merge_enabled()) {
            q.ab = w.ab2; q.wpack = b.p_qv; q.bias = b.qv_bias; q.scale = 1.0f; q.Cout = 2 * b.cout;
            q.q_out = w.q; q.vt_out = w.vt;
            HIP_TRY(conv_launch(h, 1, PRO_GN, RES_NONE, OUT_QV, q, s));
            HIP_TRY(launch_attention_merged((const float*)w.q, (const float*)x_mid.p, w.ab2, (const float*)w.vt, h->P(b.proj_b), kSkipScale,
                                            (float*)out.p, out.st, B, s));
            out.slots = 8;
            return FG_OK;
        }
        q.ab = w.ab2; q.wpack = b.p_qkv; q.bias = b.qkv_bias; q.scale = 1.0f; q.Cout = 3 * b.cout;
        q.q_out = w.q; q.k_out = w.k; q.vt_out = w.vt;
        HIP_TRY(conv_launch(h, 1, PRO_GN, RES_NONE, OUT_QKV, q, s));
        HIP_TRY(launch_attention(h->cmode, w.q, w.k, w.vt, w.aout, B, hw, s));
        ConvArgs p{};
        p.src1 = w.aout; p.C1 = b.cout; p.Hs = p.Ws = p.H = p.W = b.res_out; p.B = B;
        p.wpack = b.p_proj; p.bias = h->P(b.proj_b); p.resid = x_mid.p; p.scale = kSkipScale; p.out = out.p; p.Cout = b.cout;
        p.stats = out.st;
        HIP_TRY(conv_launch(h, 1, PRO_NONE, RES_NONE, OUT_NHWC, p, s));
        out.slots = slots;
    }
    return FG_OK;
}

int run_mapping(fg_edm* h, const float* labels, int B, Workspace& w, hipStream_t s) {
    const fg_edm_config& c = h->cfg;
    HIP_TRY(launch_mapping_in(w.coef + B, w.coef + 4 * (size_t)B, h->freqs, labels, c.label_dim,
                              h->P(h->find("model.map_label.weight")), h->P(h->find("model.map_label.bias")), w.emb0, B,
                              h->cond_ch, h->noise_ch, s, h->augment, h->augment ? h->P(h->find("model.map_augment.weight")) : nullptr, c.augment_dim));
    HIP_TRY(launch_linear(w.emb0, h->P(h->find("model.map_layer0.weight")), h->P(h->find("model.map_layer0.bias")), w.emb1,
                          B, h->cond_ch, h->emb_ch, 1, s));
    HIP_TRY(launch_linear(w.emb1, h->P(h->find("model.map_layer1.weight")), h->P(h->find("model.map_layer1.bias")), w.emb, B,
                          h->emb_ch, h->emb_ch, 1, s));
    HIP_TRY(launch_linear(w.emb, h->aff_w, h->aff_b, w.temb, B, h->emb_ch, h->temb_total, 0, s));
    return FG_OK;
}

int run_forward(fg_edm* h, const float* x_t, const double* t, int t_stride, const double* r, int r_stride,
                const float* labels, float* out, int B, Workspace& w, hipStream_t s, float* const* feats = nullptr,
                bool early = false, TrainStash* ts = nullptr) {
    if (h->adm) return adm_forward(h, x_t, t, t_stride, labels, out, B, w, s);
    const fg_edm_config& c = h->cfg;
    HIP_TRY(launch_precond_coef(t, t_stride, c.r_timestep ? r : nullptr, r_stride, c.sigma_data, h->shift(), 1e-6,
                                c.drop_precond, w.coef, B, s));
    int rc = run_mapping(h, labels, B, w, s);
    if (rc) return rc;
    w.drop = DropArgs{};
    w.infer = ts == nullptr;
    if (ts && h->dropout_p > 0.f) w.drop.p = h->dropout_p, w.drop.seed = h->dropout_seed;
    const Act none;
    const Act* x = nullptr;
    for (size_t i = 0; i < h->enc.size(); ++i) {
        const Block& b = h->enc[i];
        if (b.kind == K_STEM) {
            if (b.p_stem) {
                HIP_TRY(launch_stem(h->dtype, x_t, w.coef, b.p_stem, h->P(b.b), w.skip[i].p, w.skip[i].st, B, b.res_out, b.cin, s));
                w.skip[i].slots = b.res_out * b.res_out / 32;
            } else {
                HIP_TRY(launch_conv_in(h->dtype, x_t, w.coef, h->P(b.w), h->P(b.b), w.skip[i].p, B, b.res_out, b.cin, b.cout, s));
                w.skip[i].st = nullptr;
            }
        } else {
            if (ts) use_stash(w, ts->blocks[block_index(h, &b)]);
            rc = run_block(h, b, *x, b.cin, none, 0, w.temb, w.skip[i], B, w, s);
            if (rc) return rc;
            if (feats && b.tap >= 0 && feats[b.tap])
                HIP_TRY(launch_act_to_nchw(h->dtype, w.skip[i].p, feats[b.tap], B, b.cout, b.res_out * b.res_out, s));
        }
        x = &w.skip[i];
    }
    if (early) return FG_OK;
    int sp = (int)h->enc.size();
    Act* pong[2] = {&w.xa, &w.xb};
    int cur = 0;
    size_t di = 0;
    const float2* aux_ab = nullptr;
    for (const Block& b : h->dec) {
        if (b.kind == K_BLOCK) {
            const Act& x2 = b.skip_c ? w.skip[--sp] : none;
            Act& dst = ts ? ts->dec_store[di++] : *pong[cur];
            if (ts) use_stash(w, ts->blocks[block_index(h, &b)]);
            rc = run_block(h, b, *x, b.cin - b.skip_c, x2, b.skip_c, w.temb, dst, B, w, s);
            if (rc) return rc;
            x = &dst;
            cur ^= 1;
        } else if (b.kind == K_AUX_NORM) {
            if (ts) w.ab0 = ts->aux_ab, w.mr0 = ts->aux_mr;
            if ((rc = norm_coeffs(h->dtype, *x, b.cin, none, 0, h->P(b.w), h->P(b.b), w.ab0, B, b.res_in * b.res_in, s, ts ? w.mr0 : nullptr))) return rc;
            aux_ab = w.ab0;
        } else if (b.kind == K_AUX_CONV) {
            if (b.p_aux)
                HIP_TRY(launch_aux_head(h->cmode, x->p, aux_ab, b.p_aux, h->P(b.b), x_t, w.coef, out, B, b.cin, b.cout, s, ts ? ts->raw_out : nullptr));
            else
                HIP_TRY(launch_aux_out(h->dtype, x->p, aux_ab, h->P(b.w), h->P(b.b), x_t, w.coef, out, B, b.res_out, b.cin, b.cout, s, ts ? ts->raw_out : nullptr));
        }
    }
    return FG_OK;
}

int enqueue_sampler(fg_edm* h, const float* noise, const float* labels, const double* t_list, int steps, int type,
                    int loop, const float* eps, float* out, int B, Workspace& w, hipStream_t s) {
    const fg_edm_config& c = h->cfg;
    const int64_t total = (int64_t)B * c.img_channels * c.img_resolution * c.img_resolution;
    const StudentLoop L{noise, t_list, steps, type, c.schedule, total, w.x, w.eps, eps, w.tl, w.seed, out, s};
    if (loop == FG_LOOP_MEANFLOW)
        return meanflow_loop(L, w.x_pred, [&](int i, float* u) {
            return run_forward(h, w.x, w.tl + i, 0, w.tl + (type == FG_SAMPLE_SDE ? steps : i + 1), 0, labels, u, B, w, s);
        });
    return x0_loop(L, w.x_pred, [&](int i, float* pred) { return run_forward(h, w.x, w.tl + i, 0, w.tl + steps, 0, labels, pred, B, w, s); });
}

int ensure_device_state(fg_edm* h) {
    if (h->device_ready) return FG_OK;
    int rc;
    const size_t tsz = h->dtype ? 2 : 4;
    for (Block* b : h->blocks) {
        if ((rc = h->alloc(&b->p_conv0, conv_pack_elems(b->cout, b->cin, 3) * tsz))) return rc;
        if ((rc = h->alloc(&b->p_conv1, conv_pack_elems(b->cout, b->cout, 3) * tsz))) return rc;
        const bool x3 = h->cmode == FG_DTYPE_BF16X3;
        if ((x3 ? conv_x3ws_shape_ok(b->cout, b->cin, b->res_out) : conv_ws_shape_ok(h->cmode, b->cout, b->cin, b->res_out)) && !b->down &&
            (rc = h->alloc(&b->p_conv0_ws, conv_pack_elems(b->cout, b->cin, 3) * tsz)))
            return rc;
        if ((x3 ? conv_x3ws_shape_ok(b->cout, b->cout, b->res_out) : conv_ws_shape_ok(h->cmode, b->cout, b->cout, b->res_out)) &&
            (rc = h->alloc(&b->p_conv1_ws, conv_pack_elems(b->cout, b->cout, 3) * tsz)))
            return rc;
        if (x3 && b->up && conv_x3ws_shape_ok(b->cout, b->cin, b->res_in) && (rc = h->alloc(&b->p_conv0_sub, conv_pack_elems(b->cout, b->cin, 4) * 4)))
            return rc;
        if (b->has_skip && (rc = h->alloc(&b->p_skip, conv_pack_elems(b->cout, b->cin, 1) * tsz))) return rc;
        if (b->attn) {
            if ((rc = h->alloc(&b->p_qkv, conv_pack_elems(3 * b->cout, b->cout, 1) * tsz))) return rc;
            if ((rc = h->alloc(&b->p_proj, conv_pack_elems(b->cout, b->cout, 1) * tsz))) return rc;
            if ((rc = h->alloc((void**)&b->qkv_bias, sizeof(float) * 3 * b->cout))) return rc;
            if (x3 && b->cout == 256 && b->res_out == 16) {
                if ((rc = h->alloc(&b->p_qv, conv_pack_elems(2 * b->cout, b->cout, 1) * tsz))) return rc;
                if ((rc = h->alloc((void**)&b->qv_bias, sizeof(float) * 2 * b->cout))) return rc;
                if (!h->qv_w && (rc = h->alloc((void**)&h->qv_w, sizeof(float) * 2 * b->cout * b->cout))) return rc;
            }
        }
    }
    for (Block& b : h->enc)
        if (b.kind == K_STEM && stem_supported(b.res_out, b.cin, b.cout))
// ... 326 lines not shown
    for (int i = 0; i < 3; ++i) HIP_TRY(run());
    HIP_TRY(hipEventRecord(e0, nullptr));
    for (int i = 0; i < iters; ++i) HIP_TRY(run());
    HIP_TRY(hipEventRecord(e1, nullptr));
    HIP_TRY(hipEventSynchronize(e1));
    float ms = 0.f;
    HIP_TRY(hipEventElapsedTime(&ms, e0, e1));
    if (ms_out) *ms_out = ms / iters;
    (void)hipEventDestroy(e0); (void)hipEventDestroy(e1);
    (void)hipFree(x); (void)hipFree(out); (void)hipFree(resid); (void)hipFree(bias); (void)hipFree(ab); (void)hipFree(wp);
    return FG_OK;
}

int fg_edm_num_blocks(const fg_edm* h) {
    if (h && h->adm) return adm_num_blocks(h);
    return h ? (int)h->blocks.size() : 0;
}

int fg_edm_block_info(const fg_edm* h, int index, const char** key, int* cin, int* cout, int* res_in, int* res_out,
                      int* has_attention) {
    if (h && h->adm) return adm_block_info(h, index, key, cin, cout, res_in, res_out, has_attention);
    if (!h || index < 0 || index >= (int)h->blocks.size()) return fail(FG_EINVAL, "block index out of range");
    const Block* b = h->blocks[index];
    if (key) *key = b->key.c_str();
    if (cin) *cin = b->cin;
    if (cout) *cout = b->cout;
    if (res_in) *res_in = b->res_in;
    if (res_out) *res_out = b->res_out;
    if (has_attention) *has_attention = b->attn ? 1 : 0;
    return FG_OK;
}

int fg_edm_run_block(fg_edm* h, int index, const float* x1, int c1, const float* x2, int c2, const float* emb, float* out,
                     int batch, void* workspace, size_t workspace_bytes, void* stream) {
    if (!h || !x1 || !emb || !out) return fail(FG_EINVAL, "null argument");
    if (h->adm) return adm_run_block(h, index, x1, c1, x2, c2, emb, out, batch, workspace, workspace_bytes, (hipStream_t)stream);
    if (!h->packed) return fail(FG_ENOTREADY, "weights are not packed (call fg_edm_pack_weights)");
    if (index < 0 || index >= (int)h->blocks.size()) return fail(FG_EINVAL, "block index out of range");
    Workspace w;
    int rc0 = setup_ws(plan_workspace, h, batch, workspace, workspace_bytes, w);
    if (rc0) return rc0;
    hipStream_t s = (hipStream_t)stream;
    HIP_TRY(launch_linear(emb, h->aff_w, h->aff_b, w.temb, batch, h->emb_ch, h->temb_total, 0, s));
    const Block& b = *h->blocks[index];
    const size_t npix_in = (size_t)batch * b.res_in * b.res_in, npix_out = (size_t)batch * b.res_out * b.res_out;
    Act a1, a2;
    HIP_TRY(launch_to_act(h->dtype, x1, w.cvt1, (int64_t)npix_in * c1, s));
    a1.p = w.cvt1;
    if (c2) {
        HIP_TRY(launch_to_act(h->dtype, x2, w.cvt2, (int64_t)npix_in * c2, s));
        a2.p = w.cvt2;
    }
    w.infer = true;
    int rc = run_block(h, b, a1, c1, a2, c2, w.temb, w.xa, batch, w, s);
    if (rc) return rc;
    HIP_TRY(launch_from_act(h->dtype, w.xa.p, out, (int64_t)npix_out * b.cout, s));
    return FG_OK;
}

#include "engine_train.inc"
#include "engine_dit.inc"
#include "engine_wan.inc"
#include "engine_wan_jvp.inc"
#include "engine_sampler.inc"
#include "engine_edm2.inc"
#include "engine_edm2_jvp.inc"
#include "engine_train_ops.inc"
#include "engine_edm_ops.inc"

int fg_op_gn_coeffs(const float* x1, int c1, const float* x2, int c2, const float* gamma, const float* beta, float eps,
                    float* ab_out, int batch, int hw, void* stream) {
    if (!x1 || !gamma || !beta || !ab_out) return fail(FG_EINVAL, "null argument");
    HIP_TRY(launch_gn_coeffs(0, x1, c1, c2 ? x2 : nullptr, c2, gamma, beta, eps, (float2*)ab_out, batch, hw, (hipStream_t)stream));
    return FG_OK;
}

size_t fg_op_adm_conv_pack_bytes(int mode, int cout, int cin, int ks) {
    if ((mode != FG_DTYPE_BF16 && mode != FG_DTYPE_BF16X3) || (ks != 1 && ks != 3) || cout <= 0 || cin <= 0 || cin % 32) return 0;
    return adm_conv_pack_elems(mode, cout, cin, ks) * sizeof(__bf16);
}
int fg_op_adm_conv_pack(int mode, const float* w_oihw, void* packed, int cout, int cin, int ks, void* stream) {
    if (!fg_op_adm_conv_pack_bytes(mode, cout, cin, ks))
        return fail(FG_EINVAL, "fg_op_adm_conv_pack: mode %d (1 bf16, 2 bf16x3), ks %d (1, 3), cout %d > 0, cin %d (multiple of 32)", mode,
                    ks, cout, cin);
    if (!w_oihw || !packed) return fail(FG_EINVAL, "fg_op_adm_conv_pack: null pointer");
    HIP_TRY(adm_pack_conv_weights(mode, w_oihw, packed, cout, cin, ks, (hipStream_t)stream));
    return FG_OK;
}
int fg_op_adm_conv_ex(int mode, int ks, const float* src1, int c1, const float* src2, int c2, int batch, int hs, int h, int res_mode,
                      const float* ab, int ab_stride, int silu, const void* packed, const float* bias, const float* resid, int resid_mode,
                      float resid_scale, float clip, float* out, int cout, void* stream) {
    if ((mode != FG_DTYPE_BF16 && mode != FG_DTYPE_BF16X3) || (ks != 1 && ks != 3))
        return fail(FG_EINVAL, "fg_op_adm_conv: mode %d (1 bf16, 2 bf16x3), ks %d (1, 3)", mode, ks);
    if (c1 <= 0 || c1 % 32 || c2 < 0 || c2 % 32 || cout <= 0 || batch <= 0 || batch > 65535)
        return fail(FG_EINVAL, "fg_op_adm_conv: c1 %d > 0 and c2 %d >= 0 multiples of 32, cout %d > 0, batch %d in 1 .. 65535", c1, c2,
                    cout, batch);
    const bool res_ok = (res_mode == 0 && hs == h) || (res_mode == 1 && hs == 2 * h) || (res_mode == 2 && h == 2 * hs);
    if (h <= 0 || h > 4096 || !res_ok) return fail(FG_EINVAL, "fg_op_adm_conv: res_mode %d with hs %d, h %d", res_mode, hs, h);
    if (resid && (resid_mode < 0 || resid_mode > 2 || (resid_mode == 2 && h % 2)))
        return fail(FG_EINVAL, "fg_op_adm_conv: resid_mode %d (0, 1, 2 with h even) at h %d", resid_mode, h);
    if (ab_stride != -1 && ab_stride != 0 && ab_stride < c1 + c2)
        return fail(FG_EINVAL, "fg_op_adm_conv_ex: ab_stride %d (-1, 0 or >= c1 + c2 = %d)", ab_stride, c1 + c2);
    if (!std::isfinite(resid_scale) || !(clip >= 0.0f) || !std::isfinite(clip))
        return fail(FG_EINVAL, "fg_op_adm_conv_ex: resid_scale %g must be finite, clip %g finite and >= 0 (0: no clamp)", (double)resid_scale,
                    (double)clip);
    if (!src1 || (c2 && !src2) || !packed || !out) return fail(FG_EINVAL, "fg_op_adm_conv: null pointer");
// ... 453 lines not shown
```

### fastgen_amd/csrc/engine_edm_ops.inc

```

namespace {

bool al16(const void* p) { return !(((uintptr_t)p) & 15); }
bool al8(const void* p) { return !(((uintptr_t)p) & 7); }
int edm_storage(int dtype) { return dtype == FG_DTYPE_BF16 ? 1 : 0; }

bool edm_conv_generic_form(int dtype, int ks, int pro, int res, int outmode, int W) {
    if (outmode == OUT_QKV) return ks == 1 && pro == PRO_GN && res == RES_NONE;
    if (outmode == OUT_QV) return dtype == FG_DTYPE_BF16X3 && ks == 1 && pro == PRO_GN && res == RES_NONE && W == 16;
    if (ks == 3 && pro == PRO_GN_SILU) return res == RES_NONE || res == RES_UP;
    if (ks == 3 && pro == PRO_NONE) return res == RES_NONE;
    if (ks == 1 && pro == PRO_NONE) return res == RES_NONE || res == RES_DOWN || res == RES_UP;
    return false;
}

const char* edm_conv_shape(int dtype, int ks, int pro, int res, int outmode, int c1, int c2, int batch, int hs, int h, int cout, int rshift,
                           ConvArgs& a) {
    if (dtype != FG_DTYPE_F32 && dtype != FG_DTYPE_BF16 && dtype != FG_DTYPE_BF16X3) return "dtype must be 0 (fp32), 1 (bf16) or 2 (bf16x3)";
    if (ks != 1 && ks != 3) return "ks must be 1 or 3";
    if (pro != PRO_NONE && pro != PRO_GN && pro != PRO_GN_SILU) return "pro must be 0 (none), 1 (a x + b) or 2 (silu(a x + b))";
    if (res != RES_NONE && res != RES_DOWN && res != RES_UP && res != RES_SUBPIX) return "res must be 0 (none), 1 (down), 2 (up) or 3 (sub-pixel up)";
    if (outmode != OUT_NHWC && outmode != OUT_QKV && outmode != OUT_QV) return "outmode must be 0 (NHWC), 1 (q | k | v^T planes) or 4 (q' | v'^T planes)";
    if (h != 8 && h != 16 && h != 32) return "the output resolution must be 8, 16 or 32";
    if ((res == RES_NONE && hs != h) || (res == RES_DOWN && hs != 2 * h) || ((res == RES_UP || res == RES_SUBPIX) && 2 * hs != h))
        return "the source resolution must be h (res 0), 2 h (res 1) or h / 2 (res 2, 3)";
    const int kc = dtype == FG_DTYPE_BF16 ? 64 : 32;
    if (c1 <= 0 || c2 < 0 || (c1 % kc) || (c2 % kc)) return "c1 > 0 and c2 >= 0 must be multiples of the K step (64 in bf16, else 32)";
    if (batch <= 0 || batch > 65535) return "batch must be 1 .. 65535";
    if (outmode == OUT_NHWC && (cout <= 0 || (cout % 256))) return "cout must be a positive multiple of 256";
    if (outmode == OUT_QKV && (cout != 768 || h > 16)) return "the q | k | v^T form needs cout 768 at 8x8 or 16x16";
    if (outmode == OUT_QV && (cout != 512 || h != 16 || dtype != FG_DTYPE_BF16X3)) return "the q' | v'^T form needs cout 512 at 16x16 in bf16x3";
    if (rshift != 0 && rshift != 1) return "rshift must be 0 or 1";
    a.C1 = c1, a.C2 = c2, a.Hs = a.Ws = hs, a.H = a.W = h, a.B = batch, a.Cout = cout, a.rshift = rshift;
    return nullptr;
}

int edm_conv_kernel(int dtype, int ks, int pro, int res, int outmode, const ConvArgs& a, int* slots) {
    int kernel = 0;
    if (a.rshift && !(dtype == FG_DTYPE_BF16X3 && conv_ws_enabled() && conv_x3ws_supported(ks, pro, res, outmode, a)))
        kernel = 0;
    else if (conv_ws_enabled() && conv_ws_supported(dtype, ks, pro, res, outmode, a)) {
        const bool four_steps = pro != PRO_NONE && (a.C1 + a.C2) / 32 == 4;
        kernel = (four_steps && (res != RES_NONE || a.W != 32)) ? 0 : FG_EDM_CONV_WS;
    }
    else if (dtype == FG_DTYPE_BF16X3 && conv_ws_enabled() && conv_x3ws_supported(ks, pro, res, outmode, a))
        kernel = FG_EDM_CONV_X3WS;
    else if (res != RES_SUBPIX && !a.rshift && edm_conv_generic_form(dtype, ks, pro, res, outmode, a.W))
        kernel = FG_EDM_CONV_GENERIC;
    if (slots) *slots = kernel ? conv_launch_stat_slots(dtype, ks, pro, res, outmode, a) : 0;
    return kernel;
}

bool edm_gn_ok(int c1, int c2) {
    const int C = c1 + c2;
    if (c1 <= 0 || c2 < 0 || (c1 % 4) || (c2 % 4) || C < 16 || C > 512) return false;
    const int groups = C / 4 < 32 ? C / 4 : 32;
    return !(C % groups) && !((C / groups) % 4);
}

}

size_t fg_op_edm_conv_pack_bytes(int dtype, int layout, int cout, int cin, int ks) {
    if (cout <= 0 || cin <= 0 || cout > 4096 || cin > 4096) return 0;
    switch (layout) {
    case FG_EDM_PACK_GENERIC:
        if ((dtype != FG_DTYPE_F32 && dtype != FG_DTYPE_BF16 && dtype != FG_DTYPE_BF16X3) || (ks != 1 && ks != 3)) return 0;
        if ((cout % 32) || (cin % (dtype == FG_DTYPE_BF16 ? 64 : 32))) return 0;
        return conv_pack_elems(cout, cin, ks) * (dtype == FG_DTYPE_BF16 ? 2 : 4);
    case FG_EDM_PACK_WS:
        return dtype == FG_DTYPE_BF16 && ks == 3 && conv_ws_shape_ok(dtype, cout, cin, 32) ? conv_pack_elems(cout, cin, 3) * 2 : 0;
    case FG_EDM_PACK_X3WS:
        return dtype == FG_DTYPE_BF16X3 && ks == 3 && conv_x3ws_shape_ok(cout, cin, 32) ? conv_pack_elems(cout, cin, 3) * 4 : 0;
    case FG_EDM_PACK_X3SUB:
        return dtype == FG_DTYPE_BF16X3 && ks == 3 && conv_x3ws_shape_ok(cout, cin, 16) ? conv_pack_elems(cout, cin, 4) * 4 : 0;
    }
    return 0;
}

int fg_op_edm_conv_pack(int dtype, int layout, const float* w_oihw, void* packed, int cout, int cin, int ks, int qkv_perm, void* stream) {
    if (!fg_op_edm_conv_pack_bytes(dtype, layout, cout, cin, ks))
        return fail(FG_EINVAL, "fg_op_edm_conv_pack: no layout %d packing in dtype %d for cout %d, cin %d, ks %d", layout, dtype, cout, cin, ks);
    if (qkv_perm && (layout != FG_EDM_PACK_GENERIC || (cout % 3) || ks != 1))
        return fail(FG_EINVAL, "fg_op_edm_conv_pack: the q | k | v de-interleave belongs to the generic 1x1 layout with cout %d a multiple of 3", cout);
    if (!w_oihw || !packed) return fail(FG_EINVAL, "fg_op_edm_conv_pack: null pointer");
    if (!al16(packed)) return fail(FG_EINVAL, "fg_op_edm_conv_pack: packed must be 16-byte aligned");
    hipStream_t s = (hipStream_t)stream;
    switch (layout) {
    case FG_EDM_PACK_GENERIC: HIP_TRY(launch_pack_conv_weights(dtype, w_oihw, packed, cout, cin, ks, qkv_perm ? 1 : 0, s)); break;
    case FG_EDM_PACK_WS: HIP_TRY(launch_pack_conv_weights_ws(w_oihw, packed, cout, cin, s)); break;
    case FG_EDM_PACK_X3WS: HIP_TRY(launch_pack_conv_weights_x3ws(w_oihw, packed, cout, cin, s)); break;
    default: HIP_TRY(launch_pack_conv_weights_x3sub(w_oihw, packed, cout, cin, s)); break;
    }
    return FG_OK;
}

int fg_op_edm_conv_plan(int dtype, int ks, int pro, int res, int outmode, int c1, int c2, int batch, int hs, int h, int cout, int has_wpack_ws,
                        int rshift, fg_edm_conv_plan* plan) {
    if (!plan) return fail(FG_EINVAL, "fg_op_edm_conv_plan: null plan");
    plan->kernel = 0, plan->stat_slots = 0;
    ConvArgs a{};
    if (const char* why = edm_conv_shape(dtype, ks, pro, res, outmode, c1, c2, batch, hs, h, cout, rshift, a))
        return fail(FG_EINVAL, "fg_op_edm_conv_plan: %s", why);
    static const float2 some{};
    a.ab = pro != PRO_NONE ? &some : nullptr;
    a.wpack = &some;
    a.wpack_ws = has_wpack_ws ? &some : nullptr;
    a.resid = rshift ? &some : nullptr;
    plan->kernel = edm_conv_kernel(dtype, ks, pro, res, outmode, a, &plan->stat_slots);
    if (!plan->kernel)
        return fail(FG_EINVAL, "fg_op_edm_conv_plan: no kernel for ks %d, pro %d, res %d, outmode %d, rshift %d in dtype %d at %dx%d (wave-specialised weights %s)",
                    ks, pro, res, outmode, rshift, dtype, h, h, has_wpack_ws ? "given" : "absent");
    return FG_OK;
}

int fg_op_edm_conv(int dtype, int ks, int pro, int res, int outmode, const void* src1, int c1, const void* src2, int c2, int batch, int hs, int h,
                   const float* ab, const void* wpack, const void* wpack_ws, const float* bias, const float* temb, int temb_stride, const void* resid,
                   int rshift, float scale, void* out, int cout, float* stats, void* q_out, void* k_out, void* vt_out, void* stream) {
    ConvArgs a{};
    if (const char* why = edm_conv_shape(dtype, ks, pro, res, outmode, c1, c2, batch, hs, h, cout, rshift, a)) return fail(FG_EINVAL, "fg_op_edm_conv: %s", why);
    if (!std::isfinite(scale)) return fail(FG_EINVAL, "fg_op_edm_conv: scale must be finite");
    if (!src1 || (c2 && !src2) || !wpack) return fail(FG_EINVAL, "fg_op_edm_conv: null src1 / src2 / wpack");
    if (pro != PRO_NONE && !ab) return fail(FG_EINVAL, "fg_op_edm_conv: pro %d needs the coefficients ab", pro);
    if (outmode == OUT_NHWC) {
        if (!out || q_out || k_out || vt_out) return fail(FG_EINVAL, "fg_op_edm_conv: the NHWC form writes out alone");
        if (temb && (temb_stride < cout || (temb_stride % 4))) return fail(FG_EINVAL, "fg_op_edm_conv: temb_stride %d must be a multiple of 4, at least cout %d", temb_stride, cout);
        if (rshift && !resid) return fail(FG_EINVAL, "fg_op_edm_conv: rshift without a residual");
    } else {
        if (out || temb || resid || stats || rshift) return fail(FG_EINVAL, "fg_op_edm_conv: the plane forms take no out, temb, resid, rshift or stats");
        if (!q_out || !vt_out || (outmode == OUT_QKV) != (k_out != nullptr)) return fail(FG_EINVAL, "fg_op_edm_conv: q_out, vt_out (and k_out of the q | k | v^T form alone)");
        if (scale != 1.0f) return fail(FG_EINVAL, "fg_op_edm_conv: the v^T plane is stored unscaled: scale must be 1");
    }
    if (!al16(src1) || !al16(src2) || !al16(wpack) || !al16(wpack_ws) || !al16(ab) || !al16(bias) || !al16(temb) || !al16(resid) || !al16(out) ||
        !al16(q_out) || !al16(k_out) || !al16(vt_out) || !al8(stats))
        return fail(FG_EINVAL, "fg_op_edm_conv: tensors, weights, ab, bias and temb must be 16-byte aligned, stats 8-byte aligned");
    a.src1 = src1, a.src2 = c2 ? src2 : nullptr, a.ab = pro != PRO_NONE ? (const float2*)ab : nullptr;
    a.wpack = wpack, a.wpack_ws = wpack_ws, a.bias = bias, a.temb = temb, a.temb_stride = temb_stride, a.resid = resid;
    a.scale = scale, a.out = out, a.stats = (float2*)stats, a.q_out = q_out, a.k_out = k_out, a.vt_out = vt_out;
    if (!edm_conv_kernel(dtype, ks, pro, res, outmode, a, nullptr))
        return fail(FG_EINVAL, "fg_op_edm_conv: no kernel for ks %d, pro %d, res %d, outmode %d, rshift %d in dtype %d at %dx%d (wave-specialised weights %s)", ks,
                    pro, res, outmode, rshift, dtype, h, h, wpack_ws ? "given" : "absent");
    static bool prepared[3][16] = {};
    const int dev = fg_device_slot();
    if (dev < 0) return fail(FG_EHIP, "fg_op_edm_conv: no current device");
    if (!prepared[dtype][dev]) {
        if (conv_prepare_all(dtype) != 0) return fail(FG_EHIP, "hipFuncSetAttribute(dynamic LDS) failed");
        prepared[dtype][dev] = true;
    }
    HIP_TRY(launch_conv_fused(dtype, ks, pro, res, outmode, a, (hipStream_t)stream));
    return FG_OK;
}

int fg_op_edm_gn_finalize(const float* st1, int c1, int s1, const float* st2, int c2, int s2, const float* gamma, const float* beta, float eps,
                          float* ab, float* mr, int batch, int hw, void* stream) {
    if (!edm_gn_ok(c1, c2))
        return fail(FG_EINVAL, "fg_op_edm_gn_finalize: c1 %d > 0, c2 %d >= 0 multiples of 4, 16 <= c1 + c2 <= 512, groups of a multiple of 4 channels", c1, c2);
    if (s1 <= 0 || s1 > 4096 || (c2 && (s2 <= 0 || s2 > 4096))) return fail(FG_EINVAL, "fg_op_edm_gn_finalize: slot counts s1 %d, s2 %d must be 1 .. 4096", s1, s2);
    if (batch <= 0 || batch > 65535 || hw <= 0 || hw > (1 << 22)) return fail(FG_EINVAL, "fg_op_edm_gn_finalize: batch %d (1 .. 65535), hw %d (1 .. 2^22)", batch, hw);
    if (!(eps >= 0.f) || !std::isfinite(eps)) return fail(FG_EINVAL, "fg_op_edm_gn_finalize: eps must be finite and >= 0");
    if (!st1 || (c2 && !st2) || !gamma || !beta || !ab) return fail(FG_EINVAL, "fg_op_edm_gn_finalize: null pointer");
    if (!al8(st1) || !al8(st2) || !al8(ab) || !al8(mr)) return fail(FG_EINVAL, "fg_op_edm_gn_finalize: st1 / st2 / ab / mr must be 8-byte aligned");
    HIP_TRY(launch_gn_finalize((const float2*)st1, c1, s1, c2 ? (const float2*)st2 : nullptr, c2, c2 ? s2 : 0, gamma, beta, eps, (float2*)ab, batch, hw,
                               (hipStream_t)stream, (float2*)mr));
    return FG_OK;
}

int fg_op_edm_gn_silu_pool(int dtype, const void* x, const float* ab, void* out, int batch, int res_out, int c, void* stream) {
    if (dtype != FG_DTYPE_F32 && dtype != FG_DTYPE_BF16 && dtype != FG_DTYPE_BF16X3) return fail(FG_EINVAL, "fg_op_edm_gn_silu_pool: dtype %d (0, 1, 2)", dtype);
    if (c <= 0 || (c % 8) || c > 4096 || batch <= 0 || batch > 65535 || res_out <= 0 || res_out > 512)
        return fail(FG_EINVAL, "fg_op_edm_gn_silu_pool: c %d (a multiple of 8 up to 4096), batch %d (1 .. 65535), res_out %d (1 .. 512)", c, batch, res_out);
    if (!x || !ab || !out) return fail(FG_EINVAL, "fg_op_edm_gn_silu_pool: null pointer");
    if (!al16(x) || !al16(out) || !al8(ab)) return fail(FG_EINVAL, "fg_op_edm_gn_silu_pool: x / out must be 16-byte aligned, ab 8-byte aligned");
    HIP_TRY(launch_gn_silu_pool(edm_storage(dtype), x, (const float2*)ab, out, batch, res_out, res_out, c, (hipStream_t)stream));
    return FG_OK;
}

int fg_op_edm_attention(int dtype, const void* q, const void* k, const void* vt, void* out, int batch, int t, void* stream) {
    if (dtype != FG_DTYPE_F32 && dtype != FG_DTYPE_BF16 && dtype != FG_DTYPE_BF16X3) return fail(FG_EINVAL, "fg_op_edm_attention: dtype %d (0, 1, 2)", dtype);
    if ((t != 64 && t != 256) || batch <= 0 || batch > 65535) return fail(FG_EINVAL, "fg_op_edm_attention: t %d (64, 256), batch %d (1 .. 65535)", t, batch);
    if (!q || !k || !vt || !out) return fail(FG_EINVAL, "fg_op_edm_attention: null pointer");
    if (!al16(q) || !al16(k) || !al16(vt) || !al16(out)) return fail(FG_EINVAL, "fg_op_edm_attention: tensors must be 16-byte aligned");
    HIP_TRY(launch_attention(dtype, q, k, vt, out, batch, t, (hipStream_t)stream));
    return FG_OK;
}

int fg_op_edm_attn_merge_weights(const float* qkv_w, const float* qkv_b, const float* proj_w, float* w_out, float* b_out, int c, void* stream) {
    if (c <= 0 || c > 4096) return fail(FG_EINVAL, "fg_op_edm_attn_merge_weights: c %d (1 .. 4096)", c);
    if (!qkv_w || !qkv_b || !proj_w || !w_out || !b_out) return fail(FG_EINVAL, "fg_op_edm_attn_merge_weights: null pointer");
    HIP_TRY(launch_attn_merge_weights(qkv_w, qkv_b, proj_w, w_out, b_out, c, (hipStream_t)stream));
    return FG_OK;
}

int fg_op_edm_attention_merged(const float* qm, const float* x_mid, const float* ab, const float* vmt, const float* bp, float scale, float* out,
                               float* stats, int batch, void* stream) {
    if (batch <= 0 || batch > 32767) return fail(FG_EINVAL, "fg_op_edm_attention_merged: batch %d (1 .. 32767)", batch);
    if (!std::isfinite(scale)) return fail(FG_EINVAL, "fg_op_edm_attention_merged: scale must be finite");
    if (!qm || !x_mid || !ab || !vmt || !bp || !out) return fail(FG_EINVAL, "fg_op_edm_attention_merged: null pointer");
    if (!al16(qm) || !al16(x_mid) || !al16(ab) || !al16(vmt) || !al16(bp) || !al16(out) || !al8(stats))
        return fail(FG_EINVAL, "fg_op_edm_attention_merged: tensors, ab and bp must be 16-byte aligned, stats 8-byte aligned");
    HIP_TRY(launch_attention_merged(qm, x_mid, (const float2*)ab, vmt, bp, scale, out, (float2*)stats, batch, (hipStream_t)stream));
    return FG_OK;
}

size_t fg_op_edm_head_pack_bytes(int which, int dtype, int c) {
    if (dtype != FG_DTYPE_F32 && dtype != FG_DTYPE_BF16 && dtype != FG_DTYPE_BF16X3) return 0;
    if (which == FG_EDM_PACK_STEM) return stem_pack_elems() * (edm_storage(dtype) ? 2 : 4);
    if (which == FG_EDM_PACK_AUX) return c > 0 && c <= 4096 && !(c % (dtype == FG_DTYPE_BF16 ? 64 : 32)) ? aux_pack_elems(c) * (dtype == FG_DTYPE_BF16 ? 2 : 4) : 0;
    return 0;
}

int fg_op_edm_stem(int dtype, const float* x, const float* coef, const float* w_oihw, void* packed, const float* bias, void* out, float* stats, int batch,
                   int res, int cin, void* stream) {
    if (dtype != FG_DTYPE_F32 && dtype != FG_DTYPE_BF16 && dtype != FG_DTYPE_BF16X3) return fail(FG_EINVAL, "fg_op_edm_stem: dtype %d (0, 1, 2)", dtype);
    if (cin <= 0 || res <= 0 || res > 1024 || !stem_supported(res, cin, 128))
        return fail(FG_EINVAL, "fg_op_edm_stem: cin %d (9 cin <= 32), res %d (res^2 a multiple of 32, up to 1024)", cin, res);
    if (batch <= 0 || batch > 65535) return fail(FG_EINVAL, "fg_op_edm_stem: batch %d (1 .. 65535)", batch);
    if (!x || !coef || !w_oihw || !packed || !bias || !out) return fail(FG_EINVAL, "fg_op_edm_stem: null pointer");
    if (!al16(packed) || !al16(out) || !al8(stats)) return fail(FG_EINVAL, "fg_op_edm_stem: packed / out must be 16-byte aligned, stats 8-byte aligned");
    hipStream_t s = (hipStream_t)stream;
    const int st = edm_storage(dtype);
    HIP_TRY(launch_pack_stem_weights(st, w_oihw, packed, cin, s));
    HIP_TRY(launch_stem(st, x, coef, packed, bias, out, (float2*)stats, batch, res, cin, s));
    return FG_OK;
}

int fg_op_edm_conv_in(int dtype, const float* x, const float* coef, const float* w_oihw, const float* bias, void* out, int batch, int res, int cin, int cout,
                      void* stream) {
    if (dtype != FG_DTYPE_F32 && dtype != FG_DTYPE_BF16 && dtype != FG_DTYPE_BF16X3) return fail(FG_EINVAL, "fg_op_edm_conv_in: dtype %d (0, 1, 2)", dtype);
    if (cin <= 0 || cout <= 0 || (cout % 16) || (size_t)cin * 9 * cout * sizeof(float) > 64 * 1024)
        return fail(FG_EINVAL, "fg_op_edm_conv_in: cin %d > 0, cout %d a multiple of 16, 36 cin cout <= 65536 bytes of LDS", cin, cout);
    if (batch <= 0 || res <= 0 || res > 1024 || (int64_t)batch * res > (1 << 30)) return fail(FG_EINVAL, "fg_op_edm_conv_in: batch %d, res %d (1 .. 1024)", batch, res);
    if (!x || !coef || !w_oihw || !bias || !out) return fail(FG_EINVAL, "fg_op_edm_conv_in: null pointer");
    if (!al16(out)) return fail(FG_EINVAL, "fg_op_edm_conv_in: out must be 16-byte aligned");
    HIP_TRY(launch_conv_in(edm_storage(dtype), x, coef, w_oihw, bias, out, batch, res, cin, cout, (hipStream_t)stream));
    return FG_OK;
}

int fg_op_edm_aux_head(int dtype, const void* x, const float* ab, const float* w_oihw, void* packed, const float* bias, const float* x_t, const float* coef,
                       float* out, int batch, int c, int cout, void* stream) {
    if (dtype != FG_DTYPE_F32 && dtype != FG_DTYPE_BF16 && dtype != FG_DTYPE_BF16X3) return fail(FG_EINVAL, "fg_op_edm_aux_head: dtype %d (0, 1, 2)", dtype);
    if (c <= 0 || c > 4096 || cout <= 0 || !aux_head_supported(dtype, 32, c, cout))
        return fail(FG_EINVAL, "fg_op_edm_aux_head: c %d (a multiple of the K step: 64 in bf16, else 32), cout %d (1 .. 32)", c, cout);
    if (batch <= 0 || batch > 65535) return fail(FG_EINVAL, "fg_op_edm_aux_head: batch %d (1 .. 65535)", batch);
    if (!x || !ab || !w_oihw || !packed || !bias || !x_t || !coef || !out) return fail(FG_EINVAL, "fg_op_edm_aux_head: null pointer");
    if (!al16(x) || !al16(ab) || !al16(packed)) return fail(FG_EINVAL, "fg_op_edm_aux_head: x / ab / packed must be 16-byte aligned");
    hipStream_t s = (hipStream_t)stream;
    HIP_TRY(launch_pack_aux_weights(dtype, w_oihw, packed, c, cout, s));
    HIP_TRY(launch_aux_head(dtype, x, (const float2*)ab, packed, bias, x_t, coef, out, batch, c, cout, s));
    return FG_OK;
}

int fg_op_edm_aux_out(int dtype, const void* x, const float* ab, const float* w_oihw, const float* bias, const float* x_t, const float* coef, float* out,
                      int batch, int res, int c, int cout, void* stream) {
// ... 10 lines not shown
```

### fastgen_amd/csrc/misc.h

```cpp
#pragma once
#include <hip/hip_runtime.h>
#include <stdint.h>

int launch_gn_coeffs(int dtype, const void* x1, int c1, const void* x2, int c2, const float* gamma, const float* beta,
                     float eps, float2* ab, int batch, int hw, hipStream_t s, float2* mr = nullptr);
int launch_gn_finalize(const float2* st1, int c1, int s1, const float2* st2, int c2, int s2, const float* gamma,
                       const float* beta, float eps, float2* ab, int batch, int hw, hipStream_t s, float2* mr = nullptr);
int launch_precond_coef(const double* t, int t_stride, const double* r, int r_stride, double sigma_data,
                        double sigma_shift, double clamp_min, int drop, float* coef, int B, hipStream_t s);
int launch_mapping_in(const float* c_noise, const float* r_noise, const float* freqs, const float* labels, int label_dim,
                      const float* wl, const float* bl, float* out, int B, int N, int noise_ch, hipStream_t s, const float* aug = nullptr, const float* wa = nullptr, int aug_dim = 0);
inline bool linear_on_matrix_pipe(int I, int O) { return I % 16 == 0 && O % 32 == 0; }
int launch_linear(const float* x, const float* w, const float* bias, float* y, int B, int I, int O, int act_silu,
                  hipStream_t s);
int launch_conv_in(int dtype, const float* x, const float* c_in, const float* w, const float* bias, void* out, int B,
                   int res, int cin, int cout, hipStream_t s);
int launch_aux_out(int dtype, const void* x, const float2* ab, const float* w, const float* bias, const float* x_t,
                   const float* coef, float* out, int B, int res, int C, int cout, hipStream_t s, float* raw = nullptr);
int launch_latents(const float* noise, double tv, const double* tp, int ti, float* out, int64_t total, hipStream_t s);
int launch_forward_process(const float* x0, const float* eps, double tv, const double* tp, int ti, int sched, float* out,
                           int64_t total, hipStream_t s);
int launch_x0_to_eps(const float* xt, const float* x0, double tv, const double* tp, int ti, int sched, double clamp_min,
                     float* out, int64_t total, hipStream_t s);
int launch_meanflow_update(const float* x, const float* u, const double* tp, int ia, int ib, float* out, int64_t total,
                           hipStream_t s);
int launch_randn(float* out, int64_t total, uint64_t seed, uint64_t offset, const uint64_t* seed_dev, hipStream_t s);
int launch_embed_times(const double* tp, int ti, double tv, int ri, double rv, double scale, int sit, int diff, int f32in, float* te, float* re,
                       int n, hipStream_t s);
int launch_flow_to_x0(const float* xt, const float* v, const double* tp, int ti, float sign, float* out, int64_t total, hipStream_t s);
int launch_euler_step(const float* x, const float* v, const double* tp, int ti, float g, int cfg, float sign, float* out, float* out2,
                      int64_t total, hipStream_t s);
int launch_guided_multistep(const float* v, float* x, float* x2, float* x_last, float* m_prev, const double* tab, int guided, int first,
                            int64_t total, hipStream_t s);
int launch_copy_rows(const float* src, int64_t src_pitch, float* dst, int64_t dst_pitch, int64_t run, int64_t rows, hipStream_t s);
int launch_gn_silu_pool(int dtype, const void* x, const float2* ab, void* out, int B, int H, int W, int C, hipStream_t s);
int launch_to_act(int dtype, const float* in, void* out, int64_t total, hipStream_t s);
int launch_from_act(int dtype, const void* in, float* out, int64_t total, hipStream_t s);
struct DropArgs {
    float p = 0.f;
    uint32_t block = 0;
    uint64_t seed = 0;
};
int launch_dropout_mask(float* out, int64_t total, DropArgs drop, hipStream_t s);
int launch_gn_act(int dtype, int mode, const void* x1, int c1, const void* x2, int c2, const float2* ab, void* out, int B, int res, int rm,
                  hipStream_t s, DropArgs drop = DropArgs{});
int launch_gn_bwd(int dtype, int mode, const void* x1, int c1, const void* x2, int c2, const void* dact, int cd, const float2* ab,
                  const float2* mr, const float* gamma, float2* P, float2* S, float* dgamma, float* dbeta, const void* add, int ca,
                  float add_scale, void* dx, int B, int res, int rm, hipStream_t s, void* dx2 = nullptr, int accumulate = 0,
                  DropArgs drop = DropArgs{});
int launch_colsum(int dtype, const void* t, int ct, int C, float* out, int B, int hw, float scale, hipStream_t s, int out_stride = 0);
int launch_transpose_f32(const float* in, float* out, int R, int Cc, hipStream_t s);
int launch_batchsum_add(const float* in, float* out, int B, int C, hipStream_t s, float* out2 = nullptr, int in_stride = 0);
int launch_scale_to_act(int dtype, const float* in, void* out, float scale, int64_t total, hipStream_t s);
int launch_slice_to_f32(int dtype, const void* in, int cs, int c_off, float* out, int C, int64_t npix, hipStream_t s);
int launch_affine_bwd(const float* dtemb, const float* emb, const float* w, float* dw, float* demb, int B, int C, int K, hipStream_t s);
int launch_dgrad_weights(const float* w, float* wt, int cout, int cin, int cin_pad, int taps, hipStream_t s);
int launch_head_grad(int dtype, const float* dout, const float* c_out, void* out, int B, int C, int Cp, int hw, hipStream_t s);
int launch_stem_operand(int dtype, const float* x, const float* c_in, void* out, int B, int C, int Cp, int hw, hipStream_t s);
int launch_add_sub_tensor(const float* src, int Is, float* dst, int O, int I, int T, hipStream_t s);
int launch_pad_rows(const float* src, float* dst, int O, int Op, int IT, hipStream_t s);
int launch_add_act(int dtype, void* dst, const void* src, int64_t total, hipStream_t s);
int launch_silu_bwd(const float* dy, const float* pre, float* dpre, int total, hipStream_t s);
int launch_linear_bwd(const float* dy, const float* x, const float* w, float* dw, float* db, float* dx, int B, int C, int K,
                      float scale, hipStream_t s, int dy_stride = 0);
int launch_add_nchw_to_nhwc(int dtype, const float* src, void* dst, int B, int C, int hw, hipStream_t s);
int launch_input_grad(int dtype, const void* da, int cd, const float* c_in, const float* c_skip, const float* dout, float* dx, int B, int C, int hw,
                      hipStream_t s);
int launch_gn_jvp(int dtype, int mode, const void* x1, int c1, const void* x2, int c2, const void* xd, const float2* ab, const float2* mr,
                  float2* P, float2* S, void* out, int B, int res, hipStream_t s, DropArgs drop = DropArgs{});
int launch_jvp_coef(const double* t, const double* r, const float* vt, const float* vr, double sigma_data, double sigma_shift, int drop,
                    float* ct, int B, hipStream_t s);
int launch_jvp_embed(const float* c_noise, const float* r_noise, const float* dc, const float* dr, const float* freqs, float* out, int B,
                     int N, int noise_ch, hipStream_t s);
int launch_jvp_input(const float* vx, const float* x, const float* c_in, const float* dc_in, float* out, int B, int chw, hipStream_t s);
int launch_jvp_output(int dtype, const void* fd, int cf, const float* out, const float* x, const float* vx, const float* ct, float* jvp, int B, int C,
                      int hw, hipStream_t s);
int launch_fill_f32(float* p, float v, int n, hipStream_t s);
int launch_fill_f2(float2* p, float a, float b, int n, hipStream_t s);
int launch_attention_jvp(int dtype, const void* q, const void* k, const void* vt, const void* qd, const void* kd, const void* vtd, void* od,
                         void* scratch, int B, int T, int C, hipStream_t s);
size_t attention_backward_scratch_bytes(int dtype, int B, int T, int C);
int launch_attention_backward(int dtype, const void* q, const void* k, const void* vt, const void* dO, void* dq, void* dk, void* dvt,
                              void* scratch, int B, int T, int C, hipStream_t s);
int launch_qkv_interleave(int dtype, const void* dq, const void* dk, const void* dvt, void* out, int B, int T, int C, hipStream_t s);
int launch_nt_gemm(const void* A, const void* Bm, void* C, int M, int N, int K, float scale, int out_bf16, hipStream_t s);
int launch_transpose_bf16(const void* in, void* out, int R, int Cc, hipStream_t s);
int disc_num_params(int res);
size_t disc_workspace_bytes(int res, int B);
int disc_run(const float* feat, int res, const float* const* params, float* logits, const float* dlogits, float* dfeat,
             float* const* grads, int B, void* ws, hipStream_t s);
int conv_wgrad_supported(int res, int cin, int cout, int ks);
size_t conv_wgrad_workspace_bytes(int B, int res, int cin, int cout, int ks);
int launch_conv_wgrad(int mode, const void* act, const void* dy, float* dw, int B, int res, int cin, int cout, int ks, int accumulate,
                      void* workspace, hipStream_t s, float scale = 1.0f);
int launch_images_to_u8(const float* x, uint8_t* out, int64_t B, int C, int HW, hipStream_t s);
int launch_act_to_nchw(int dtype, const void* in, float* out, int B, int C, int HW, hipStream_t s);
int launch_nchw_to_nhwc(const float* in, float* out, int B, int C, int HW, hipStream_t s);

int launch_attention(int dtype, const void* q, const void* k, const void* vt, void* out, int B, int T, hipStream_t s);
int launch_attn_merge_weights(const float* qkv_w, const float* qkv_b, const float* proj_w, float* w_out, float* b_out, int C, hipStream_t s);
int launch_attention_merged(const float* qm, const float* x_mid, const float2* ab, const float* vmt, const float* bp, float scale, float* out,
                            float2* stats, int B, hipStream_t s);

size_t aux_pack_elems(int C);
int launch_pack_aux_weights(int dtype, const float* w, void* out, int C, int cout, hipStream_t s);
int aux_head_supported(int dtype, int res, int C, int cout);
int launch_aux_head(int dtype, const void* x, const float2* ab, const void* wpack, const float* bias, const float* x_t,
                    const float* coef, float* out, int B, int C, int cout, hipStream_t s, float* raw = nullptr);

int stem_supported(int res, int cin, int cout);
size_t stem_pack_elems();
int launch_pack_stem_weights(int dtype, const float* w, void* out, int cin, hipStream_t s);
int launch_stem(int dtype, const float* x, const float* c_in, const void* wpack, const float* bias, void* out, float2* stats,
                int B, int res, int cin, hipStream_t s);

int launch_dit_ln_modulate(int dtype, int D, const void* x, const float* mod, int mod_stride, int shift_off, int scale_off, void* y,
                           int ntok, int tokens_per_image, hipStream_t s);
int launch_dit_ln_modulate_split(int D, const float* x, const float* mod, int mod_stride, int shift_off, int scale_off, void* y, int ntok,
                                 int tokens_per_image, hipStream_t s);
int launch_dit_ln_modulate_fp8(int D, const void* x, const float* mod, int mod_stride, int shift_off, int scale_off, void* y, float* y_scale,
                               int ntok, int tokens_per_image, hipStream_t s);
int launch_dit_final(int dtype, int D, const void* x, const float* mod, const float* w, const float* bias, float* out, int ntok, int grid,
                     int p, int C, hipStream_t s);
int launch_dit_patch_embed(int dtype, const float* x, const float* w, const float* bias, const float* pos, void* out, int B, int C, int grid,
                           int p, int D, hipStream_t s);
int launch_dit_fourier(const float* t, float* f, int B, int dim, hipStream_t s);
int launch_dit_cond(const float* t_emb, const float* r_emb, const float* table, const int64_t* cls, float* c, float* sc, int B, int D,
                    int rows, int* err, hipStream_t s);
int launch_dit_attention(int mode, const void* q, const void* k, const void* vt, void* out, int B, int heads, int head_dim, int T, size_t lo_off,
                         hipStream_t s, int path = 0);
int launch_dit_fourier_jvp(const float* t, const float* td, float* f, float* fd, int B, int dim, hipStream_t s);
int launch_dit_silu_jvp(const float* v, const float* da, const float* db, float* sout, float* sd, int n, hipStream_t s);
int launch_dit_ln_modulate_jvp(int D, const float* x, const float* xd, const float* mod, const float* modd, int mod_stride, int shift_off,
                               int scale_off, void* y, void* yd, int ntok, int tokens_per_image, hipStream_t s);
int launch_dit_attention_jvp(const void* q, const void* k, const void* vt, const void* qd, const void* kd, const void* vtd, float* out, float* outd,
                             int B, int heads, int head_dim, int T, size_t lo_off, hipStream_t s);
int launch_dit_gelu_jvp(const float* h, const float* hd, void* a, void* ad, int64_t M, int K, hipStream_t s);
int launch_dit_gate_update(const float* h, const float* g, const float* gd, int gate_stride, int gate_rows, const float* x, float* xo, float* xdo,
                           int64_t M, int N, hipStream_t s);
int launch_dit_final_jvp(int D, const float* x, const float* xd, const float* mod, const float* modd, const float* w, const float* bias, float* out,
                         float* outd, int ntok, int grid, int p, int C, hipStream_t s);

struct GemmArgs {
    const void* A = nullptr;
    const void* W = nullptr;
    const float* bias = nullptr;
    void* out = nullptr;
    int M = 0, N = 0, K = 0;
    int act = 0;
    const float* gate = nullptr;
    int gate_stride = 0, gate_rows = 1;
    const void* resid = nullptr;
    void *q = nullptr, *k = nullptr, *vt = nullptr;
    int heads = 0, head_dim = 0, T = 0;
    int row0 = 0;
// ... 79 lines not shown
```

### fastgen_amd/csrc/misc.hip

```cpp
#include "common.h"
#include "misc.h"

namespace {

template <typename AT>
__global__ __launch_bounds__(512) void gn_coeffs_kernel(const AT* __restrict__ x1, int C1, const AT* __restrict__ x2,
                                                        int C2, const float* __restrict__ gamma,
                                                        const float* __restrict__ beta, float eps, float2* __restrict__ ab,
                                                        int hw, float2* __restrict__ mr) {
    const int C = C1 + C2;
    const int Q = C >> 2;
    const int lanes = blockDim.x / Q;
    const int groups = min(32, C / 4);
    const int cpg = C / groups;
    const int n = blockIdx.x;
    const int t = threadIdx.x;
    __shared__ double s_sum[512], s_sq[512];
    __shared__ float s_mean[32], s_rstd[32];
    float s = 0.f, ss = 0.f;
    if (t < Q * lanes) {
        const int q = t % Q, pl = t / Q;
        const int c = q * 4;
        const AT* base = (c < C1) ? x1 + (size_t)n * hw * C1 + c : x2 + (size_t)n * hw * C2 + (c - C1);
        const int stride = (c < C1) ? C1 : C2;
        for (int p = pl; p < hw; p += lanes) {
            const f32x4 v = load4(base + (size_t)p * stride);
            s += (v[0] + v[1]) + (v[2] + v[3]);
            ss += (v[0] * v[0] + v[1] * v[1]) + (v[2] * v[2] + v[3] * v[3]);
        }
    }
    s_sum[t] = s;
    s_sq[t] = ss;
    __syncthreads();
    if (t < groups) {
        double a = 0.0, b = 0.0;
        const int q0 = t * cpg / 4, q1 = (t + 1) * cpg / 4;
        for (int pl = 0; pl < lanes; ++pl)
            for (int q = q0; q < q1; ++q) {
                a += s_sum[pl * Q + q];
                b += s_sq[pl * Q + q];
            }
        const double cnt = (double)cpg * hw;
        const double mean = a / cnt;
        double var = b / cnt - mean * mean;
        if (var < 0.0) var = 0.0;
        s_mean[t] = (float)mean;
        s_rstd[t] = (float)(1.0 / sqrt(var + (double)eps));
        if (mr) mr[(size_t)n * groups + t] = make_float2(s_mean[t], s_rstd[t]);
    }
    __syncthreads();
    for (int c = t; c < C; c += blockDim.x) {
        const int g = c / cpg;
        const float a = s_rstd[g] * gamma[c];
        ab[(size_t)n * C + c] = make_float2(a, fmaf(-a, s_mean[g], beta[c]));
    }
}

__global__ __launch_bounds__(512) void gn_finalize_kernel(const float2* __restrict__ st1, int C1, int S1, const float2* __restrict__ st2, int C2,
                                                         int S2, const float* __restrict__ gamma, const float* __restrict__ beta, float eps,
                                                         float2* __restrict__ ab, int hw, float2* __restrict__ mr) {
    const int C = C1 + C2, Qt = C >> 2;
    const int groups = min(32, C / 4);
    const int cpg = C / groups;
    const int n = blockIdx.x;
    const int SG = (int)blockDim.x / Qt;
    __shared__ double ps[512], pq[512];
    const int q = threadIdx.x % Qt, sg = threadIdx.x / Qt;
    if (sg < SG) {
        const bool first = q * 4 < C1;
        const float2* st = first ? st1 : st2;
        const int S = first ? S1 : S2;
        const int Q = (first ? C1 : C2) >> 2;
        const int ql = first ? q : q - (C1 >> 2);
        double s = 0.0, v2 = 0.0;
        for (int sl = sg; sl < S; sl += SG) {
            const float2 v = st[((size_t)n * S + sl) * Q + ql];
            s += v.x;
            v2 += v.y;
        }
        ps[sg * Qt + q] = s;
        pq[sg * Qt + q] = v2;
    }
    __syncthreads();
    for (int c = threadIdx.x; c < C; c += blockDim.x) {
        const int g = c / cpg;
        double s = 0.0, v2 = 0.0;
        for (int quad = g * cpg / 4; quad < (g + 1) * cpg / 4; ++quad)
            for (int l = 0; l < SG; ++l) {
                s += ps[l * Qt + quad];
                v2 += pq[l * Qt + quad];
            }
        const double cnt = (double)cpg * hw;
        const double mean = s / cnt;
        double var = v2 / cnt - mean * mean;
        if (var < 0.0) var = 0.0;
        const float m = (float)mean, rstd = (float)(1.0 / sqrt(var + (double)eps));
        const float a = rstd * gamma[c];
        ab[(size_t)n * C + c] = make_float2(a, fmaf(-a, m, beta[c]));
        if (mr && c % cpg == 0) mr[(size_t)n * groups + g] = make_float2(m, rstd);
    }
}

__global__ void precond_coef_kernel(const double* __restrict__ t, int t_stride, const double* __restrict__ r, int r_stride,
                                    double sigma_data, double sigma_shift, double clamp_min, int drop,
                                    float* __restrict__ coef, int B) {
    const int b = blockIdx.x * blockDim.x + threadIdx.x;
    if (b >= B) return;
    const double tv = t[(size_t)b * t_stride];
    const double rv = r ? r[(size_t)b * r_stride] : 0.0;
    const double sd2 = sigma_data * sigma_data;
    if (drop & 1) {
        coef[b] = 1.0f;
        coef[B + b] = (float)tv;
        coef[4 * B + b] = (float)rv;
    } else {
        coef[b] = (float)(1.0 / sqrt(sd2 + tv * tv));
        coef[B + b] = (float)(log(fmax(tv, clamp_min)) / 4.0);
        coef[4 * B + b] = (float)(log(fmax(rv, clamp_min)) / 4.0);
    }
    if (drop & 2) {
        coef[2 * B + b] = 0.0f;
        coef[3 * B + b] = 1.0f;
    } else {
        const double ts = tv - sigma_shift;
        coef[2 * B + b] = (float)(sd2 / (ts * ts + sd2));
        coef[3 * B + b] = (float)(ts * sigma_data / sqrt(ts * ts + sd2));
    }
}

__global__ void mapping_in_kernel(const float* __restrict__ c_noise, const float* __restrict__ r_noise,
                                  const float* __restrict__ freqs, const float* __restrict__ labels, int label_dim,
                                  const float* __restrict__ wl, const float* __restrict__ bl, float* __restrict__ out, int B,
                                  int N, int noise_ch, const float* __restrict__ aug, const float* __restrict__ wa, int aug_dim) {
    const int idx = blockIdx.x * blockDim.x + threadIdx.x;
    if (idx >= B * N) return;
    const int b = idx / N, j = idx % N;
    const int half = noise_ch / 2;
    const int jj = j % noise_ch;
    const float lab = (j < noise_ch) ? c_noise[b] : r_noise[b];
    const float ang = lab * freqs[jj % half];
    float v = (jj < half) ? sinf(ang) : cosf(ang);
    if (label_dim > 0) {
        float acc = 0.f;
        const float sc = sqrtf((float)label_dim);
        if (labels)
            for (int i = 0; i < label_dim; ++i) acc = fmaf(labels[(size_t)b * label_dim + i] * sc, wl[(size_t)j * label_dim + i], acc);
        v += acc + bl[j];
    }
    if (aug) {
        float acc = 0.f;
        for (int i = 0; i < aug_dim; ++i) acc = fmaf(aug[(size_t)b * aug_dim + i], wa[(size_t)j * aug_dim + i], acc);
// ... 649 lines not shown
```

### include/fastgen_amd.h

```cpp
#ifndef FASTGEN_AMD_H
#define FASTGEN_AMD_H

#include <stddef.h>
#include <stdint.h>

#ifdef __cplusplus
extern "C" {
#endif

#define FG_API __attribute__((visibility("default")))

#define FG_OK 0
#define FG_EINVAL 1
#define FG_ENOTREADY 2
#define FG_EHIP 3
#define FG_ENOMEM 4

#define FG_DTYPE_F32 0
#define FG_DTYPE_BF16 1
#define FG_DTYPE_BF16X3 2
#define FG_DTYPE_FP8 3

#define FG_SAMPLE_SDE 0
#define FG_SAMPLE_ODE 1
// ... 164 lines not shown
                             uint32_t drop_block, uint64_t drop_seed, void* workspace, size_t workspace_bytes, void* stream);
FG_API int fg_op_gn_jvp(int dtype, int mode, const void* x1, int c1, const void* x2, int c2, const void* xd, const float* gamma,
                        const float* beta, float eps, void* out, int batch, int res, float drop_p, uint32_t drop_block, uint64_t drop_seed,
                        void* workspace, size_t workspace_bytes, void* stream);
FG_API size_t fg_op_attention_backward_workspace_bytes(int dtype, int batch, int t, int c);
FG_API int fg_op_attention_backward(int dtype, const void* q, const void* k, const void* vt, const void* d_out, void* dq, void* dk, void* dvt,
                                    void* dqkv, int batch, int t, int c, void* workspace, size_t workspace_bytes, void* stream);
FG_API int fg_op_attention_jvp(int dtype, const void* q, const void* k, const void* vt, const void* qd, const void* kd, const void* vtd,
                               void* od, int batch, int t, int c, void* workspace, size_t workspace_bytes, void* stream);
FG_API int fg_op_colsum(int dtype, const void* t, int ct, int c, float* out, int batch, int hw, float scale, int out_stride, void* stream);
FG_API int fg_op_batchsum_add(const float* in, float* out, float* out2, int batch, int c, int in_stride, void* stream);
FG_API int fg_op_linear_backward(int affine, const float* dy, const float* x, const float* w, float* dw, float* db, float* dx, int batch,
                                 int c, int k, float scale, int dy_stride, void* stream);
FG_API int fg_op_dgrad_weights(const float* w, float* wt, int cout, int cin, int cin_pad, int taps, void* stream);
#define FG_TRAIN_OP_HEAD_GRAD 0
#define FG_TRAIN_OP_STEM_OPERAND 1
#define FG_TRAIN_OP_INPUT_GRAD 2
#define FG_TRAIN_OP_ADD_NCHW_TO_NHWC 3
#define FG_TRAIN_OP_SILU_BWD 4
#define FG_TRAIN_OP_JVP_COEF 5
#define FG_TRAIN_OP_JVP_EMBED 6
#define FG_TRAIN_OP_JVP_INPUT 7
#define FG_TRAIN_OP_JVP_OUTPUT 8
FG_API int fg_op_train_elementwise(int op, int dtype, const void* a, const void* b, const void* c, const void* d, const void* e, void* out,
                                   int batch, int ch, int ch_pad, int hw, double f0, double f1, int flag, void* stream);

#define FG_EDM_PACK_GENERIC 0
#define FG_EDM_PACK_WS 1
#define FG_EDM_PACK_X3WS 2
#define FG_EDM_PACK_X3SUB 3
#define FG_EDM_CONV_GENERIC 1
#define FG_EDM_CONV_WS 2
#define FG_EDM_CONV_X3WS 3
typedef struct fg_edm_conv_plan {
    int kernel;
    int stat_slots;
} fg_edm_conv_plan;
FG_API size_t fg_op_edm_conv_pack_bytes(int dtype, int layout, int cout, int cin, int ks);
FG_API int fg_op_edm_conv_pack(int dtype, int layout, const float* w_oihw, void* packed, int cout, int cin, int ks, int qkv_perm, void* stream);
FG_API int fg_op_edm_conv_plan(int dtype, int ks, int pro, int res, int outmode, int c1, int c2, int batch, int hs, int h, int cout,
                               int has_wpack_ws, int rshift, fg_edm_conv_plan* plan);
FG_API int fg_op_edm_conv(int dtype, int ks, int pro, int res, int outmode, const void* src1, int c1, const void* src2, int c2, int batch, int hs,
                          int h, const float* ab, const void* wpack, const void* wpack_ws, const float* bias, const float* temb, int temb_stride,
                          const void* resid, int rshift, float scale, void* out, int cout, float* stats, void* q_out, void* k_out, void* vt_out,
                          void* stream);
FG_API int fg_op_edm_gn_finalize(const float* st1, int c1, int s1, const float* st2, int c2, int s2, const float* gamma, const float* beta,
                                 float eps, float* ab, float* mr, int batch, int hw, void* stream);
FG_API int fg_op_edm_gn_silu_pool(int dtype, const void* x, const float* ab, void* out, int batch, int res_out, int c, void* stream);
FG_API int fg_op_edm_attention(int dtype, const void* q, const void* k, const void* vt, void* out, int batch, int t, void* stream);
FG_API int fg_op_edm_attn_merge_weights(const float* qkv_w, const float* qkv_b, const float* proj_w, float* w_out, float* b_out, int c,
                                        void* stream);
FG_API int fg_op_edm_attention_merged(const float* qm, const float* x_mid, const float* ab, const float* vmt, const float* bp, float scale,
                                      float* out, float* stats, int batch, void* stream);
#define FG_EDM_PACK_STEM 0
#define FG_EDM_PACK_AUX 1
FG_API size_t fg_op_edm_head_pack_bytes(int which, int dtype, int c);
FG_API int fg_op_edm_stem(int dtype, const float* x, const float* coef, const float* w_oihw, void* packed, const float* bias, void* out,
                          float* stats, int batch, int res, int cin, void* stream);
FG_API int fg_op_edm_conv_in(int dtype, const float* x, const float* coef, const float* w_oihw, const float* bias, void* out, int batch, int res,
                             int cin, int cout, void* stream);
FG_API int fg_op_edm_aux_head(int dtype, const void* x, const float* ab, const float* w_oihw, void* packed, const float* bias, const float* x_t,
                              const float* coef, float* out, int batch, int c, int cout, void* stream);
FG_API int fg_op_edm_aux_out(int dtype, const void* x, const float* ab, const float* w_oihw, const float* bias, const float* x_t,
                             const float* coef, float* out, int batch, int res, int c, int cout, void* stream);

typedef struct fg_dit_config {
    int input_size;
    int patch_size;
    int in_channels;
    int hidden_size;
    int depth;
    int num_heads;
    int mlp_hidden;
    int embedding_rows;
    int r_timestep;
    int compute_dtype;
} fg_dit_config;
typedef struct fg_dit fg_dit;

FG_API int fg_dit_create(const fg_dit_config* cfg, fg_dit** out);
FG_API void fg_dit_destroy(fg_dit* h);
FG_API int fg_dit_num_params(const fg_dit* h);
FG_API int fg_dit_param_info(const fg_dit* h, int index, const char** name, int* ndim, int64_t shape[4]);
FG_API int fg_dit_bind_param(fg_dit* h, const char* name, const float* device_ptr, int64_t numel);
FG_API int fg_dit_pack_weights(fg_dit* h, void* stream);
FG_API int fg_dit_pack_group(fg_dit* h, const char* prefix, const char* exclude, void* stream);
FG_API size_t fg_dit_workspace_bytes(const fg_dit* h, int batch);
FG_API int fg_dit_forward(fg_dit* h, const float* x_t, const float* t, const float* r, const int64_t* class_ids, float* out,
                          float* cond_out, int batch, void* workspace, size_t workspace_bytes, void* stream);

FG_API int fg_dit_forward_features(fg_dit* h, const float* x_t, const float* t, const float* r, const int64_t* class_ids, float* out,
                                   float* cond_out, const int* feature_blocks, float* const* features, int num_features, int batch,
                                   void* workspace, size_t workspace_bytes, void* stream);

FG_API size_t fg_dit_jvp_workspace_bytes(const fg_dit* h, int batch);
FG_API int fg_dit_jvp(fg_dit* h, const float* x_t, const float* t, const float* r, const int64_t* class_ids, const float* vx, const float* vt,
                      const float* vr, float* out, float* jvp, int batch, void* workspace, size_t workspace_bytes, void* stream);
FG_API int fg_op_dit_ln_modulate_jvp(const float* x, const float* xd, const float* mod, const float* modd, int mod_stride, int shift_off,
                                     int scale_off, void* y, void* yd, int ntok, int d, int tokens_per_image, void* stream);
FG_API int fg_op_dit_attention_jvp(const void* q, const void* k, const void* vt, const void* qd, const void* kd, const void* vtd, float* out,
                                   float* outd, int batch, int heads, int head_dim, int tokens, size_t lo_off, void* stream);
FG_API int fg_op_dit_gelu_jvp(const float* h, const float* hd, void* a, void* ad, int64_t m, int k, void* stream);

typedef struct fg_dit_sampler_config {
    double t_scale;
    double guidance_scale;
// ... 279 lines not shown
```

Before: 2877 img/s.

## Fuse GroupNorm coefficient finalize into conv and attention tails via arrival counters

Adds a 'GN tail' path: the bf16x3 weight-stationary conv and merged-attention kernels write per-tile stats with atomic stores, bump a per-image arrival counter, and the last arriving workgroup computes the next GroupNorm's scale/shift coefficients (for up to two targets, including decoder skip-concat inputs). This removes separate gn_finalize/norm_coeffs kernel launches and their stats re-reads between blocks. It costs extra atomics, serialized vmcnt waits and a counter-zeroing fill per forward, and is gated by shape-fit checks and an environment variable that defaults on.

```diff
diff --git a/fastgen_amd/_lib.py b/fastgen_amd/_lib.py
--- a/fastgen_amd/_lib.py
+++ b/fastgen_amd/_lib.py
@@ -92,6 +92,10 @@
 
 class fg_edm_conv_plan(ctypes.Structure):
     _fields_ = [("kernel", c_int), ("stat_slots", c_int)]
+
+
+class fg_edm_gn_target(ctypes.Structure):
+    _fields_ = [("gamma", c_void_p), ("beta", c_void_p), ("ab", c_void_p), ("mr", c_void_p), ("c_off", c_int), ("c_total", c_int)]
 
 
 FG_EDM_PACK_GENERIC, FG_EDM_PACK_WS, FG_EDM_PACK_X3WS, FG_EDM_PACK_X3SUB = range(4)
@@ -328,6 +332,11 @@
     "fg_op_edm_attention": (c_int, [c_int, c_void_p, c_void_p, c_void_p, c_void_p, c_int, c_int, c_void_p]),
     "fg_op_edm_attn_merge_weights": (c_int, [c_void_p, c_void_p, c_void_p, c_void_p, c_void_p, c_int, c_void_p]),
     "fg_op_edm_attention_merged": (c_int, [c_void_p, c_void_p, c_void_p, c_void_p, c_void_p, c_float, c_void_p, c_void_p, c_int, c_void_p]),
+    "fg_op_edm_conv_gn_tail": (c_int, [c_int, c_int, c_int, c_int, c_void_p, c_int, c_void_p, c_int, c_int, c_int, c_int, c_void_p, c_void_p, c_void_p,
+                                       c_void_p, c_void_p, c_int, c_void_p, c_int, c_float, c_void_p, c_int, c_void_p, POINTER(fg_edm_gn_target), c_int,
+                                       c_float, c_void_p, c_void_p]),
+    "fg_op_edm_attention_merged_gn_tail": (c_int, [c_void_p, c_void_p, c_void_p, c_void_p, c_void_p, c_float, c_void_p, c_void_p, c_int,
+                                                   POINTER(fg_edm_gn_target), c_int, c_float, c_void_p, c_void_p]),
     "fg_op_edm_head_pack_bytes": (c_size_t, [c_int, c_int, c_int]),
     "fg_op_edm_stem": (c_int, [c_int, c_void_p, c_void_p, c_void_p, c_void_p, c_void_p, c_void_p, c_void_p, c_int, c_int, c_int, c_void_p]),
     "fg_op_edm_conv_in": (c_int, [c_int, c_void_p, c_void_p, c_void_p, c_void_p, c_void_p, c_int, c_int, c_int, c_int, c_void_p]),
diff --git a/fastgen_amd/csrc/attn.hip b/fastgen_amd/csrc/attn.hip
--- a/fastgen_amd/csrc/attn.hip
+++ b/fastgen_amd/csrc/attn.hip
@@ -301,6 +301,7 @@
     const float* bp;
     float2* stats;
     float scale;
+    GnTail gn;
 };
 
 template <bool MRG>
@@ -477,7 +478,7 @@
                         sv += __shfl_xor(sv, 1), qv += __shfl_xor(qv, 1);
                         sv += __shfl_xor(sv, 2), qv += __shfl_xor(qv, 2);
                         if (h == 0 && (r & 3) == 0)
-                            mg.stats[((size_t)n * 8 + (blockIdx.x & 1) * 4 + wave) * (D / 4) + ((col + r) >> 2)] = make_float2(sv, qv);
+                            gn_slot_store_wt(&mg.stats[((size_t)n * 8 + (blockIdx.x & 1) * 4 + wave) * (D / 4) + ((col + r) >> 2)], sv, qv);
                     }
                 }
             } else {
@@ -486,6 +487,12 @@
 #pragma unroll
                     for (int i = 0; i < 16; ++i) obase[(size_t)acc_row(i, h) * D + ((s >> 2) * 4 + d) * 32] = o[d][i];
             }
+        }
+    }
+    if constexpr (MRG) {
+        if (mg.gn.n && gn_tail_arrive(mg.gn.cnt, n, 8u)) {
+            gn_tail_acquire();
+            gn_tail_finalize(mg.gn, mg.stats, 8, n);
         }
     }
 }
@@ -529,10 +536,19 @@
 }
 
 int launch_attention_merged(const float* qm, const float* x_mid, const float2* ab, const float* vmt, const float* bp, float scale, float* out,
-                            float2* stats, int B, hipStream_t s) {
+                            float2* stats, int B, hipStream_t s, const GnTail* gn) {
     const int rc = x3_lds_prepare<true>();
     if (rc || !qm) return rc;
-    hipLaunchKernelGGL(attention_x3_lds_kernel<true>, dim3(B * 2), dim3(256), 2 * X3_BUF, s, qm, x_mid, vmt, out, B, AttnMerge{ab, bp, stats, scale});
+    AttnMerge mg{ab, bp, stats, scale, GnTail{}};
+    if (gn && gn->n) {
+        if (gn->n < 0 || gn->n > 2 || !stats || !gn->cnt) return (int)hipErrorInvalidValue;
+        for (int i = 0; i < gn->n; ++i) {
+            const GnTarget& t = gn->t[i];
+            if (!t.gamma || !t.beta || !t.ab || t.hw != 256 || !gn_tail_target_ok(t.c_off, t.C_total)) return (int)hipErrorInvalidValue;
+        }
+        mg.gn = *gn;
+    }
+    hipLaunchKernelGGL(attention_x3_lds_kernel<true>, dim3(B * 2), dim3(256), 2 * X3_BUF, s, qm, x_mid, vmt, out, B, mg);
     return (int)hipGetLastError();
 }
 
diff --git a/fastgen_amd/csrc/conv.h b/fastgen_amd/csrc/conv.h
--- a/fastgen_amd/csrc/conv.h
+++ b/fastgen_amd/csrc/conv.h
@@ -1,5 +1,6 @@
 #pragma once
 #include <hip/hip_runtime.h>
+#include "gn_tail.h"
 
 struct ConvArgs {
     const void* src1;
@@ -29,6 +30,7 @@
     int act = 0;
     int heads = 0, head_dim = 0;
     size_t heads_lo_off = 0;
+    GnTail gn;
 };
 
 enum { PRO_NONE = 0, PRO_GN = 1, PRO_GN_SILU = 2 };
@@ -45,11 +47,13 @@
 bool conv_x3ws_supported(int ks, int pro, int res, int outmode, const ConvArgs& a);
 bool conv_x3ws_shape_ok(int cout, int cin, int res);
 int conv_x3ws_stat_slots(int W, int res);
+bool conv_x3ws_tail_fits(int res, const ConvArgs& a);
 int launch_conv_x3ws(int res, const ConvArgs& a, hipStream_t stream, bool prepare_only, int pro = PRO_GN_SILU);
 int launch_pack_conv_weights_x3ws(const float* w_oihw, void* wpack_ws, int cout, int cin, hipStream_t stream);
 int launch_pack_conv_weights_x3sub(const float* w_oihw, void* wpack_sub, int cout, int cin, hipStream_t stream);
 int conv_subpix_mode();
 int conv_launch_stat_slots(int dtype, int ks, int pro, int res, int outmode, const ConvArgs& a);
+bool conv_takes_gn_tail(int dtype, int ks, int pro, int res, int outmode, const ConvArgs& a);
 int launch_conv_ws_debug(const ConvArgs& a, int abl, hipStream_t stream);
 int launch_conv_debug(int dtype, const ConvArgs& a, hipStream_t stream);
 int conv_prepare_all(int dtype);
diff --git a/fastgen_amd/csrc/conv.hip b/fastgen_amd/csrc/conv.hip
--- a/fastgen_amd/csrc/conv.hip
+++ b/fastgen_amd/csrc/conv.hip
@@ -611,6 +611,7 @@
     if (pro != PRO_NONE && !a.ab) return (int)hipErrorInvalidValue;
     if (outmode == OUT_QKV && (a.Cout != 768 || a.W > 16)) return (int)hipErrorInvalidValue;
     if (outmode == OUT_QV && (a.Cout != 512 || a.W != 16 || dtype != 2 || !a.q_out || !a.vt_out)) return (int)hipErrorInvalidValue;
+    if (a.gn.n && !conv_takes_gn_tail(dtype, ks, pro, res, outmode, a)) return (int)hipErrorInvalidValue;
     if (conv_ws_enabled() && conv_ws_supported(dtype, ks, pro, res, outmode, a)) return launch_conv_ws(res, a, stream, false, pro);
     if (dtype == 2 && conv_ws_enabled() && conv_x3ws_supported(ks, pro, res, outmode, a)) return launch_conv_x3ws(res, a, stream, false, pro);
     if (res == RES_SUBPIX || a.rshift) return (int)hipErrorInvalidValue;
@@ -637,6 +638,11 @@
 int conv_launch_stat_slots(int dtype, int ks, int pro, int res, int outmode, const ConvArgs& a) {
     if (dtype == 2 && conv_ws_enabled() && conv_x3ws_supported(ks, pro, res, outmode, a)) return conv_x3ws_stat_slots(a.W, res);
     return conv_stat_slots(a.W);
+}
+
+bool conv_takes_gn_tail(int dtype, int ks, int pro, int res, int outmode, const ConvArgs& a) {
+    return dtype == 2 && conv_ws_enabled() && a.stats && a.Cout == GN_TAIL_C && !conv_ws_supported(dtype, ks, pro, res, outmode, a) &&
+           conv_x3ws_supported(ks, pro, res, outmode, a) && conv_x3ws_tail_fits(res, a);
 }
 
 int conv_stat_slots(int W) { return W == 32 ? Geom<3, 5>::TPI : (W == 16 ? Geom<3, 4>::TPI : Geom<3, 3>::TPI); }
diff --git a/fastgen_amd/csrc/conv_ws3.hip b/fastgen_amd/csrc/conv_ws3.hip
--- a/fastgen_amd/csrc/conv_ws3.hip
+++ b/fastgen_amd/csrc/conv_ws3.hip
@@ -1,5 +1,6 @@
 #include "common.h"
 #include "conv.h"
+#include <type_traits>
 
 namespace {
 
@@ -20,6 +21,8 @@
     static constexpr int IPT = LOGW == 3 ? 2 : 1;
     static constexpr int TCOLS = LOGW == 3 ? 1 : W / TW;
     static constexpr int TPI = LOGW == 3 ? 1 : (W / TH) * TCOLS;
+    using Owed = typename std::conditional<LOGW == 3, unsigned, unsigned long long>::type;
+    static constexpr int OWED_BITS = 8 * (int)sizeof(Owed);
     static constexpr int HW_ = LOGW == 3 ? 2 * W + 3 : TW + 2, HH_ = TH + 2;
     static constexpr int HALO_PIX = HW_ * HH_;
     static constexpr int RS = HW_ * X3_PA;
@@ -34,7 +37,7 @@
     bf16x8 hi, lo;
 };
 
-template <int RES, int LOGW, int PRO>
+template <int RES, int LOGW, int PRO, bool TAIL = false>
 __global__ __launch_bounds__(X3_NTHR) void conv3_x3ws_kernel(const ConvArgs a, const int ntiles) {
     using G = X3Geom<LOGW>;
     constexpr bool SUB = RES == RES_SUBPIX;
@@ -319,7 +322,11 @@
     float* const out = reinterpret_cast<float*>(a.out);
     const float* const resid = reinterpret_cast<const float*>(a.resid);
     const bool has_resid = __builtin_amdgcn_readfirstlane(resid != nullptr);
-    auto retire_half = [&](int t, int half) __attribute__((always_inline)) {
+    int arr = 0;
+    typename G::Owed owed = 0;
+    constexpr int SLOTS = (SUB ? 16 : 4) * G::TPI;
+    auto retire_half = [&](int kord, int half) __attribute__((always_inline)) {
+        const int t = wg + kord * gstride;
         int n, slot, row0, col0;
         tile_coord(t, n, slot, row0, col0);
         const int co = half * 128 + chq * 4;
@@ -380,7 +387,16 @@
             ssum[k] += __shfl_xor(ssum[k], 32);
             ssq[k] += __shfl_xor(ssq[k], 32);
             const size_t sl = SUB ? ((size_t)(n + k) * G::TPI + slot) * 4 + ph : (size_t)(n + k) * G::TPI + slot;
-            if (a.stats && psub == 0 && k < nimg) a.stats[(sl * 4 + pw) * 64 + half * 32 + chq] = make_float2(ssum[k], ssq[k]);
+            if constexpr (TAIL) {
+                if (psub == 0 && k < nimg) gn_slot_store_wt(&a.stats[(sl * 4 + pw) * 64 + half * 32 + chq], ssum[k], ssq[k]);
+                if constexpr (G::IPT == 2) {
+                    if (k < nimg && gn_tail_arrive(gn_tail_cnt<offsetof(ConvArgs, gn)>(), n + k, 2u * SLOTS)) owed |= 1u << (kord * 2 + k);
+                } else {
+                    arr = kord + 1;
+                }
+            } else {
+                if (a.stats && psub == 0 && k < nimg) a.stats[(sl * 4 + pw) * 64 + half * 32 + chq] = make_float2(ssum[k], ssq[k]);
+            }
         }
     };
 
@@ -400,14 +416,33 @@
     for (int s = 0; s < NSTEP; ++s) {
         const bool more = s + 1 < S;
         if (more) stage_load(st, t1, c1);
-        if (sa == 0 && s >= nchunk && s <= S) retire_half(wg + (s / nchunk - 1) * gstride, 0);
-        if (sa == 2 % nchunk && s - 2 >= nchunk && s - 2 <= S && (s - 2) % nchunk == 0) retire_half(wg + ((s - 2) / nchunk - 1) * gstride, 1);
+        if (sa == 0 && s >= nchunk && s <= S) retire_half(s / nchunk - 1, 0);
+        if (sa == 2 % nchunk && s - 2 >= nchunk && s - 2 <= S && (s - 2) % nchunk == 0) retire_half((s - 2) / nchunk - 1, 1);
         if (more) {
             stage_store(st, ring + ((s + 1) & 3) * X3_ABUF);
             advance(t1, c1);
         }
+        if constexpr (TAIL) {
+            if (G::IPT == 1 && arr) {
+                int n, slot, row0, col0;
+                tile_coord(wg + (arr - 1) * gstride, n, slot, row0, col0);
+                if (gn_tail_arrive(gn_tail_cnt<offsetof(ConvArgs, gn)>(), n, 2u * SLOTS)) owed |= 1ull << (arr - 1);
+                arr = 0;
+            }
+        }
         if (++sa == nchunk) sa = 0;
         x3_barrier();
+    }
+    if constexpr (TAIL) {
+        if (owed) {
+            gn_tail_acquire();
+            for (int b = 0; b < my_tiles * G::IPT; ++b) {
+                if (!((owed >> b) & 1)) continue;
+                int n, slot, row0, col0;
+                tile_coord(wg + (b / G::IPT) * gstride, n, slot, row0, col0);
+                gn_tail_finalize(a.gn, a.stats, SLOTS, n + b % G::IPT);
+            }
+        }
     }
 }
 
@@ -459,10 +494,10 @@
 
 int g_x3_cus[16] = {};
 
-template <int RES, int LOGW, int PRO>
-int launch_x3_one(const ConvArgs& a, hipStream_t stream, bool prepare_only) {
+template <int RES, int LOGW, int PRO, bool TAIL>
+int launch_x3_tail(const ConvArgs& a, hipStream_t stream, bool prepare_only) {
     using G = X3Geom<LOGW>;
-    auto kern = conv3_x3ws_kernel<RES, LOGW, PRO>;
+    auto kern = conv3_x3ws_kernel<RES, LOGW, PRO, TAIL>;
     int dev = 0;
     if (hipGetDevice(&dev) != hipSuccess || dev < 0 || dev >= 16) return (int)hipErrorInvalidDevice;
     static bool attr_done[16] = {};
@@ -483,11 +518,37 @@
     return (int)hipGetLastError();
 }
 
+template <int RES, int LOGW, int PRO>
+int launch_x3_one(const ConvArgs& a, hipStream_t stream, bool prepare_only) {
+    if (prepare_only) {
+        const int rc = launch_x3_tail<RES, LOGW, PRO, false>(a, stream, true);
+        return rc ? rc : launch_x3_tail<RES, LOGW, PRO, true>(a, stream, true);
+    }
+    if (!a.gn.n) return launch_x3_tail<RES, LOGW, PRO, false>(a, stream, false);
+    if (a.gn.n < 0 || a.gn.n > 2 || !a.stats || !a.gn.cnt || a.Cout != GN_TAIL_C || !conv_x3ws_tail_fits(RES, a)) return (int)hipErrorInvalidValue;
+    for (int i = 0; i < a.gn.n; ++i) {
+        const GnTarget& t = a.gn.t[i];
+        if (!t.gamma || !t.beta || !t.ab || t.hw != a.H * a.W || !gn_tail_target_ok(t.c_off, t.C_total)) return (int)hipErrorInvalidValue;
+    }
+    return launch_x3_tail<RES, LOGW, PRO, true>(a, stream, false);
+}
+
 }
 
 int conv_x3ws_stat_slots(int W, int res) {
     if (res == RES_SUBPIX) return (W == 32 ? X3Geom<4>::TPI : X3Geom<3>::TPI) * 16;
     return (W == 32 ? X3Geom<5>::TPI : W == 16 ? X3Geom<4>::TPI : X3Geom<3>::TPI) * 4;
+}
+
+bool conv_x3ws_tail_fits(int res, const ConvArgs& a) {
+    int dev = 0, cus = 0;
+    if (hipGetDevice(&dev) != hipSuccess || dev < 0 || dev >= 16) return false;
+    if (!(cus = g_x3_cus[dev]) && (hipDeviceGetAttribute(&cus, hipDeviceAttributeMultiprocessorCount, dev) != hipSuccess || cus <= 0)) return false;
+    const int W = res == RES_SUBPIX ? a.Ws : a.W;
+    const int ipt = W == 8 ? 2 : 1, tpi = W == 8 ? 1 : W * W / 128;
+    const int64_t ntiles = ((int64_t)a.B * tpi + ipt - 1) / ipt * (res == RES_SUBPIX ? 4 : 1);
+    const int64_t grid = ntiles < cus ? ntiles : cus;
+    return (ntiles + grid - 1) / grid * ipt <= (W == 8 ? 32 : 64);
 }
 
 bool conv_x3ws_shape_ok(int cout, int cin, int res) {
diff --git a/fastgen_amd/csrc/engine.hip b/fastgen_amd/csrc/engine.hip
--- a/fastgen_amd/csrc/engine.hip
+++ b/fastgen_amd/csrc/engine.hip
@@ -107,6 +107,10 @@
     void* a1d = nullptr;
     bool infer = false;
     DropArgs drop;
+    bool gn_tail = false;
+    unsigned* gn_cnt = nullptr;
+    int gn_cnt_launches = 0, gn_cnt_used = 0;
+    std::vector<float2*> dec_ab0;
     std::vector<Act> skip;
     Act xa, xb, h, xattn;
     void *sbuf, *aout, *pool;
@@ -657,6 +661,15 @@
     w.ab0 = A.get<float2>((size_t)B * max_c);
     w.ab1 = A.get<float2>((size_t)B * max_c);
     w.ab2 = A.get<float2>((size_t)B * max_c);
+    w.dec_ab0.assign(h->dec.size(), nullptr);
+    w.gn_cnt_launches = w.gn_cnt_used = 0;
+    if (h->cmode == FG_DTYPE_BF16X3) {
+        w.gn_cnt_launches = 3 * (int)h->blocks.size();
+        w.gn_cnt = A.get<unsigned>((size_t)w.gn_cnt_launches * (((size_t)B + 3) & ~(size_t)3));
+        for (size_t i = 0; i < h->dec.size(); ++i)
+            if (h->dec[i].kind == K_BLOCK && h->dec[i].skip_c && gn_tail_target_ok(h->dec[i].cin - h->dec[i].skip_c, h->dec[i].cin))
+                w.dec_ab0[i] = A.get<float2>((size_t)B * h->dec[i].cin);
+    }
     const size_t st_elems = (size_t)B * 32 * 64;
     auto act = [&](size_t elems, size_t st_n) {
         Act a;
@@ -743,18 +756,59 @@
     return on;
 }
 
+bool gn_tail_enabled() {
+    static const bool on = [] {
+        const char* e = getenv("FASTGEN_AMD_GN_TAIL");
+        return !(e && e[0] == '0');
+    }();
+    return on;
+}
+bool gn_tail_on(const fg_edm* h) { return gn_tail_enabled() && h->cmode == FG_DTYPE_BF16X3 && !h->adm && conv_ws_enabled(); }
+int gn_tail_begin(const fg_edm* h, Workspace& w, int B, hipStream_t s) {
+    w.gn_tail = gn_tail_on(h) && w.gn_cnt != nullptr;
+    w.gn_cnt_used = 0;
+    if (w.gn_tail) HIP_TRY(launch_fill_f32(reinterpret_cast<float*>(w.gn_cnt), 0.0f, w.gn_cnt_launches * ((B + 3) & ~3), s));
+    return FG_OK;
+}
+GnTarget gn_target(const float* gamma, const float* beta, float2* ab, float2* mr, int c_off, int C_total, int hw) {
+    GnTarget t;
+    t.gamma = gamma, t.beta = beta, t.ab = ab, t.mr = mr, t.c_off = c_off, t.C_total = C_total, t.hw = hw;
+    return t;
+}
+GnTail gn_tail_for_launch(Workspace& w, const GnTail* want, int B) {
+    GnTail g;
+    if (!w.gn_tail || !want || !want->n || w.gn_cnt_used >= w.gn_cnt_launches) return g;
+    g = *want;
+    g.cnt = w.gn_cnt + (size_t)w.gn_cnt_used++ * (((size_t)B + 3) & ~(size_t)3);
+    g.eps = kBlockEps;
+    return g;
+}
+
 int run_block(fg_edm* h, const Block& b, const Act& x1, int c1, const Act& x2, int c2, const float* temb, Act& out, int B,
-              Workspace& w, hipStream_t s) {
+              Workspace& w, hipStream_t s, const GnTail* out_gn = nullptr, bool* out_done = nullptr, float2* ab0_buf = nullptr,
+              bool ab0_done = false) {
     if (c1 + c2 != b.cin) return fail(FG_EINVAL, "%s: got %d+%d input channels, expected %d", b.key.c_str(), c1, c2, b.cin);
     const int hw_in = b.res_in * b.res_in, hw = b.res_out * b.res_out;
     const int res_mode = b.down ? RES_DOWN : (b.up ? RES_UP : RES_NONE);
     const int slots = conv_stat_slots(b.res_out);
     int rc;
-    if ((rc = norm_coeffs(h->dtype, x1, c1, x2, c2, h->P(b.norm0_w), h->P(b.norm0_b), w.ab0, B, hw_in, s, w.mr0))) return rc;
+    if (out_done) *out_done = false;
+    auto tail_conv = [&](ConvArgs& c, int pro, int res, const GnTail* want) {
+        ConvArgs probe = c;
+        if (!w.gn_tail || !want || !want->n || !conv_takes_gn_tail(h->cmode, 3, pro, res, OUT_NHWC, probe)) return false;
+        c.gn = gn_tail_for_launch(w, want, B);
+        return c.gn.n != 0;
+    };
+    float2* const ab0 = ab0_buf ? ab0_buf : w.ab0;
+    if (!ab0_done && (rc = norm_coeffs(h->dtype, x1, c1, x2, c2, h->P(b.norm0_w), h->P(b.norm0_b), ab0, B, hw_in, s, w.mr0))) return rc;
+    GnTail n1;
+    n1.n = 1;
+    n1.t[0] = gn_target(h->P(b.norm1_w), h->P(b.norm1_b), w.ab1, w.mr1, 0, b.cout, hw);
+    bool n1_done = false;
     ConvArgs a{};
     a.src1 = x1.p; a.src2 = c2 ? x2.p : nullptr; a.C1 = c1; a.C2 = c2;
     a.Hs = a.Ws = b.res_in; a.H = a.W = b.res_out; a.B = B;
-    a.ab = w.ab0; a.wpack = b.p_conv0; a.wpack_ws = b.p_conv0_ws; a.bias = h->P(b.conv0_b);
+    a.ab = ab0; a.wpack = b.p_conv0; a.wpack_ws = b.p_conv0_ws; a.bias = h->P(b.conv0_b);
     a.temb = temb + b.temb_off; a.temb_stride = h->temb_total;
     a.resid = nullptr; a.scale = 1.0f; a.out = w.h.p; a.Cout = b.cout; a.stats = w.h.st;
     const bool x3_up = b.up && w.infer && !w.a1d && h->cmode == FG_DTYPE_BF16X3 && conv_ws_enabled();
@@ -767,14 +821,17 @@
     if (sub0) {
         a.wpack_ws = b.p_conv0_sub;
         w.h.slots = conv_launch_stat_slots(h->cmode, 3, PRO_GN_SILU, RES_SUBPIX, OUT_NHWC, a);
+        n1_done = tail_conv(a, PRO_GN_SILU, RES_SUBPIX, &n1);
         HIP_TRY(conv_launch(h, 3, PRO_GN_SILU, RES_SUBPIX, OUT_NHWC, a, s));
     } else if (b.down && !c2) {
-        HIP_TRY(launch_gn_silu_pool(h->dtype, x1.p, w.ab0, w.pool, B, b.res_out, b.res_out, c1, s));
+        HIP_TRY(launch_gn_silu_pool(h->dtype, x1.p, ab0, w.pool, B, b.res_out, b.res_out, c1, s));
         a.src1 = w.pool; a.Hs = a.Ws = b.res_out; a.ab = nullptr;
         w.h.slots = conv_launch_stat_slots(h->cmode, 3, PRO_NONE, RES_NONE, OUT_NHWC, a);
+        n1_done = tail_conv(a, PRO_NONE, RES_NONE, &n1);
         HIP_TRY(conv_launch(h, 3, PRO_NONE, RES_NONE, OUT_NHWC, a, s));
     } else {
         w.h.slots = conv_launch_stat_slots(h->cmode, 3, PRO_GN_SILU, res_mode, OUT_NHWC, a);
+        n1_done = tail_conv(a, PRO_GN_SILU, res_mode, &n1);
         HIP_TRY(conv_launch(h, 3, PRO_GN_SILU, res_mode, OUT_NHWC, a, s));
     }
     ConvArgs d{};
@@ -797,9 +854,16 @@
         resid = w.sbuf;
         d.rshift = low ? 1 : 0;
     }
-    HIP_TRY(launch_gn_finalize(w.h.st, b.cout, w.h.slots, nullptr, 0, 0, h->P(b.norm1_w), h->P(b.norm1_b), kBlockEps, w.ab1, B, hw, s, w.mr1));
+    if (!n1_done)
+        HIP_TRY(launch_gn_finalize(w.h.st, b.cout, w.h.slots, nullptr, 0, 0, h->P(b.norm1_w), h->P(b.norm1_b), kBlockEps, w.ab1, B, hw, s, w.mr1));
     Act& x_mid = b.attn ? w.xattn : out;
     d.resid = resid; d.out = x_mid.p; d.stats = x_mid.st;
+    GnTail n2;
+    if (b.attn) {
+        n2.n = 1;
+        n2.t[0] = gn_target(h->P(b.norm2_w), h->P(b.norm2_b), w.ab2, w.mr2, 0, b.cout, hw);
+    }
+    bool mid_done = false;
     if (w.a1d) {
         HIP_TRY(launch_gn_act(h->dtype, 0, w.h.p, b.cout, nullptr, 0, w.ab1, w.a1d, B, b.res_out, 0, s, w.drop));
         d.src1 = w.a1d; d.ab = nullptr;
@@ -807,18 +871,23 @@
         HIP_TRY(conv_launch(h, 3, PRO_NONE, RES_NONE, OUT_NHWC, d, s));
     } else {
         x_mid.slots = conv_launch_stat_slots(h->cmode, 3, PRO_GN_SILU, RES_NONE, OUT_NHWC, d);
+        mid_done = tail_conv(d, PRO_GN_SILU, RES_NONE, b.attn ? &n2 : out_gn);
         HIP_TRY(conv_launch(h, 3, PRO_GN_SILU, RES_NONE, OUT_NHWC, d, s));
     }
+    if (!b.attn && out_done) *out_done = mid_done;
     if (b.attn) {
-        HIP_TRY(launch_gn_finalize(x_mid.st, b.cout, x_mid.slots, nullptr, 0, 0, h->P(b.norm2_w), h->P(b.norm2_b), kBlockEps, w.ab2, B, hw, s, w.mr2));
+        if (!mid_done)
+            HIP_TRY(launch_gn_finalize(x_mid.st, b.cout, x_mid.slots, nullptr, 0, 0, h->P(b.norm2_w), h->P(b.norm2_b), kBlockEps, w.ab2, B, hw, s, w.mr2));
         ConvArgs q{};
         q.src1 = x_mid.p; q.C1 = b.cout; q.Hs = q.Ws = q.H = q.W = b.res_out; q.B = B;
         if (w.infer && !w.a1d && h->cmode == FG_DTYPE_BF16X3 && hw == 256 && b.cout == 256 && b.p_qv && attn_merge_enabled()) {
             q.ab = w.ab2; q.wpack = b.p_qv; q.bias = b.qv_bias; q.scale = 1.0f; q.Cout = 2 * b.cout;
             q.q_out = w.q; q.vt_out = w.vt;
             HIP_TRY(conv_launch(h, 1, PRO_GN, RES_NONE, OUT_QV, q, s));
+            const GnTail og = out.st ? gn_tail_for_launch(w, out_gn, B) : GnTail{};
             HIP_TRY(launch_attention_merged((const float*)w.q, (const float*)x_mid.p, w.ab2, (const float*)w.vt, h->P(b.proj_b), kSkipScale,
-                                            (float*)out.p, out.st, B, s));
+                                            (float*)out.p, out.st, B, s, &og));
+            if (out_done) *out_done = og.n != 0;
             out.slots = 8;
             return FG_OK;
         }
@@ -861,6 +930,43 @@
     w.drop = DropArgs{};
     w.infer = ts == nullptr;
     if (ts && h->dropout_p > 0.f) w.drop.p = h->dropout_p, w.drop.seed = h->dropout_seed;
+    w.gn_tail = false;
+    if (!ts && (rc = gn_tail_begin(h, w, B, s))) return rc;
+    const size_t ne = h->enc.size(), nd = h->dec.size();
+    std::vector<GnTail> enc_want(ne), dec_want(nd);
+    std::vector<char> enc_req(ne, 0), dec_req(nd, 0), enc_done(ne, 0), dec_done(nd, 0);
+    if (w.gn_tail) {
+        auto add = [](GnTail& g, const GnTarget& t) { g.t[g.n++] = t; };
+        for (size_t i = 1; i < ne; ++i) {
+            const Block& b = h->enc[i];
+            if (h->enc[i - 1].kind != K_BLOCK || b.kind != K_BLOCK || !gn_tail_target_ok(0, b.cin)) continue;
+            add(enc_want[i - 1], gn_target(h->P(b.norm0_w), h->P(b.norm0_b), w.ab0, nullptr, 0, b.cin, b.res_in * b.res_in));
+            enc_req[i] = 1;
+        }
+        GnTail* prev = (ne && h->enc[ne - 1].kind == K_BLOCK) ? &enc_want[ne - 1] : nullptr;
+        int sp = (int)ne;
+        for (size_t i = 0; i < nd; ++i) {
+            const Block& b = h->dec[i];
+            if (b.kind == K_BLOCK) {
+                const int c1 = b.cin - b.skip_c, hw_in = b.res_in * b.res_in;
+                GnTail* sk = b.skip_c ? &enc_want[--sp] : nullptr;
+                float2* buf = b.skip_c ? w.dec_ab0[i] : w.ab0;
+                const bool ok = prev && buf && gn_tail_target_ok(0, b.cin) && prev->n < 2 &&
+                                (!b.skip_c || (h->enc[sp].kind == K_BLOCK && gn_tail_target_ok(c1, b.cin) && sk->n < 2));
+                if (ok) {
+                    add(*prev, gn_target(h->P(b.norm0_w), h->P(b.norm0_b), buf, nullptr, 0, b.cin, hw_in));
+                    if (b.skip_c) add(*sk, gn_target(h->P(b.norm0_w), h->P(b.norm0_b), buf, nullptr, c1, b.cin, hw_in));
+                    dec_req[i] = 1;
+                }
+                prev = &dec_want[i];
+            } else if (b.kind == K_AUX_NORM) {
+                if (prev && prev->n < 2 && gn_tail_target_ok(0, b.cin)) {
+                    add(*prev, gn_target(h->P(b.w), h->P(b.b), w.ab0, nullptr, 0, b.cin, b.res_in * b.res_in));
+                    dec_req[i] = 1;
+                }
+            }
+        }
+    }
     const Act none;
     const Act* x = nullptr;
     for (size_t i = 0; i < h->enc.size(); ++i) {
@@ -875,8 +981,10 @@
             }
         } else {
             if (ts) use_stash(w, ts->blocks[block_index(h, &b)]);
-            rc = run_block(h, b, *x, b.cin, none, 0, w.temb, w.skip[i], B, w, s);
+            bool done = false;
+            rc = run_block(h, b, *x, b.cin, none, 0, w.temb, w.skip[i], B, w, s, &enc_want[i], &done, nullptr, enc_req[i] && enc_done[i - 1]);
             if (rc) return rc;
+            enc_done[i] = done;
             if (feats && b.tap >= 0 && feats[b.tap])
                 HIP_TRY(launch_act_to_nchw(h->dtype, w.skip[i].p, feats[b.tap], B, b.cout, b.res_out * b.res_out, s));
         }
@@ -888,18 +996,24 @@
     int cur = 0;
     size_t di = 0;
     const float2* aux_ab = nullptr;
-    for (const Block& b : h->dec) {
+    bool x_done = ne && enc_done[ne - 1];
+    for (size_t bi = 0; bi < nd; ++bi) {
+        const Block& b = h->dec[bi];
         if (b.kind == K_BLOCK) {
+            const bool skip_done = b.skip_c ? enc_done[sp - 1] != 0 : true;
             const Act& x2 = b.skip_c ? w.skip[--sp] : none;
             Act& dst = ts ? ts->dec_store[di++] : *pong[cur];
             if (ts) use_stash(w, ts->blocks[block_index(h, &b)]);
-            rc = run_block(h, b, *x, b.cin - b.skip_c, x2, b.skip_c, w.temb, dst, B, w, s);
+            bool done = false;
+            rc = run_block(h, b, *x, b.cin - b.skip_c, x2, b.skip_c, w.temb, dst, B, w, s, &dec_want[bi], &done,
+                           (w.gn_tail && b.skip_c) ? w.dec_ab0[bi] : nullptr, dec_req[bi] && x_done && skip_done);
             if (rc) return rc;
+            x_done = done;
             x = &dst;
             cur ^= 1;
         } else if (b.kind == K_AUX_NORM) {
             if (ts) w.ab0 = ts->aux_ab, w.mr0 = ts->aux_mr;
-            if ((rc = norm_coeffs(h->dtype, *x, b.cin, none, 0, h->P(b.w), h->P(b.b), w.ab0, B, b.res_in * b.res_in, s, ts ? w.mr0 : nullptr))) return rc;
+            if (!(dec_req[bi] && x_done) && (rc = norm_coeffs(h->dtype, *x, b.cin, none, 0, h->P(b.w), h->P(b.b), w.ab0, B, b.res_in * b.res_in, s, ts ? w.mr0 : nullptr))) return rc;
             aux_ab = w.ab0;
         } else if (b.kind == K_AUX_CONV) {
             if (b.p_aux)
@@ -1332,6 +1446,7 @@
         a2.p = w.cvt2;
     }
     w.infer = true;
+    if (int rc1 = gn_tail_begin(h, w, batch, s)) return rc1;
     int rc = run_block(h, b, a1, c1, a2, c2, w.temb, w.xa, batch, w, s);
     if (rc) return rc;
     HIP_TRY(launch_from_act(h->dtype, w.xa.p, out, (int64_t)npix_out * b.cout, s));
diff --git a/fastgen_amd/csrc/engine_edm_ops.inc b/fastgen_amd/csrc/engine_edm_ops.inc
--- a/fastgen_amd/csrc/engine_edm_ops.inc
+++ b/fastgen_amd/csrc/engine_edm_ops.inc
@@ -58,6 +58,27 @@
     return !(C % groups) && !((C / groups) % 4);
 }
 
+const char* edm_gn_tail(const fg_edm_gn_target* targets, int n_targets, float eps, unsigned* counters, const float* stats, int hw, GnTail& g) {
+    if (n_targets < 1 || n_targets > 2 || !targets) return "1 or 2 targets";
+    if (!counters || (((uintptr_t)counters) & 3)) return "counters [batch] must be a 4-byte aligned device array";
+    if (!stats) return "the tail finalizes the statistics this launch writes: stats is required";
+    if (!(eps >= 0.f) || !std::isfinite(eps)) return "eps must be finite and >= 0";
+    for (int i = 0; i < n_targets; ++i) {
+        const fg_edm_gn_target& t = targets[i];
+        if (!t.gamma || !t.beta || !t.ab) return "a target needs gamma, beta and ab";
+        if (!al8(t.ab) || !al8(t.mr)) return "a target's ab / mr must be 8-byte aligned";
+        if (!gn_tail_target_ok(t.c_off, t.c_total)) return "a target is channels [c_off, c_off + 256) of c_total: (0, 256), (0, 512) or (256, 512)";
+        g.t[i] = gn_target(t.gamma, t.beta, (float2*)t.ab, (float2*)t.mr, t.c_off, t.c_total, hw);
+    }
+    g.n = n_targets, g.cnt = counters, g.eps = eps;
+    return nullptr;
+}
+
+int edm_conv_op(int dtype, int ks, int pro, int res, int outmode, const void* src1, int c1, const void* src2, int c2, int batch, int hs, int h,
+                const float* ab, const void* wpack, const void* wpack_ws, const float* bias, const float* temb, int temb_stride, const void* resid,
+                int rshift, float scale, void* out, int cout, float* stats, void* q_out, void* k_out, void* vt_out, const fg_edm_gn_target* targets,
+                int n_targets, float eps, unsigned* counters, void* stream);
+
 }
 
 size_t fg_op_edm_conv_pack_bytes(int dtype, int layout, int cout, int cin, int ks) {
@@ -116,6 +137,24 @@
 int fg_op_edm_conv(int dtype, int ks, int pro, int res, int outmode, const void* src1, int c1, const void* src2, int c2, int batch, int hs, int h,
                    const float* ab, const void* wpack, const void* wpack_ws, const float* bias, const float* temb, int temb_stride, const void* resid,
                    int rshift, float scale, void* out, int cout, float* stats, void* q_out, void* k_out, void* vt_out, void* stream) {
+    return edm_conv_op(dtype, ks, pro, res, outmode, src1, c1, src2, c2, batch, hs, h, ab, wpack, wpack_ws, bias, temb, temb_stride, resid, rshift, scale, out,
+                       cout, stats, q_out, k_out, vt_out, nullptr, 0, 0.f, nullptr, stream);
+}
+
+int fg_op_edm_conv_gn_tail(int dtype, int ks, int pro, int res, const void* src1, int c1, const void* src2, int c2, int batch, int hs, int h, const float* ab,
+                           const void* wpack, const void* wpack_ws, const float* bias, const float* temb, int temb_stride, const void* resid, int rshift,
+                           float scale, void* out, int cout, float* stats, const fg_edm_gn_target* targets, int n_targets, float eps, unsigned* counters,
+                           void* stream) {
+    if (n_targets < 1) return fail(FG_EINVAL, "fg_op_edm_conv_gn_tail: 1 or 2 targets");
+    return edm_conv_op(dtype, ks, pro, res, OUT_NHWC, src1, c1, src2, c2, batch, hs, h, ab, wpack, wpack_ws, bias, temb, temb_stride, resid, rshift, scale, out,
+                       cout, stats, nullptr, nullptr, nullptr, targets, n_targets, eps, counters, stream);
+}
+
+namespace {
+int edm_conv_op(int dtype, int ks, int pro, int res, int outmode, const void* src1, int c1, const void* src2, int c2, int batch, int hs, int h,
+                const float* ab, const void* wpack, const void* wpack_ws, const float* bias, const float* temb, int temb_stride, const void* resid,
+                int rshift, float scale, void* out, int cout, float* stats, void* q_out, void* k_out, void* vt_out, const fg_edm_gn_target* targets,
+                int n_targets, float eps, unsigned* counters, void* stream) {
     ConvArgs a{};
     if (const char* why = edm_conv_shape(dtype, ks, pro, res, outmode, c1, c2, batch, hs, h, cout, rshift, a)) return fail(FG_EINVAL, "fg_op_edm_conv: %s", why);
     if (!std::isfinite(scale)) return fail(FG_EINVAL, "fg_op_edm_conv: scale must be finite");
@@ -139,6 +178,15 @@
     if (!edm_conv_kernel(dtype, ks, pro, res, outmode, a, nullptr))
         return fail(FG_EINVAL, "fg_op_edm_conv: no kernel for ks %d, pro %d, res %d, outmode %d, rshift %d in dtype %d at %dx%d (wave-specialised weights %s)", ks,
                     pro, res, outmode, rshift, dtype, h, h, wpack_ws ? "given" : "absent");
+    if (n_targets) {
+        if (const char* why = edm_gn_tail(targets, n_targets, eps, counters, stats, h * h, a.gn)) return fail(FG_EINVAL, "fg_op_edm_conv_gn_tail: %s", why);
+        a.gn.n = 0;
+        const bool takes = conv_takes_gn_tail(dtype, ks, pro, res, outmode, a);
+        a.gn.n = n_targets;
+        if (!takes)
+            return fail(FG_EINVAL, "fg_op_edm_conv_gn_tail: only a launch on conv3_x3ws_kernel (bf16x3, 3x3, wave-specialised weights, cout 256, batch small "
+                                   "enough for 64 tiles per workgroup) has a tail");
+    }
     static bool prepared[3][16] = {};
     const int dev = fg_device_slot();
     if (dev < 0) return fail(FG_EHIP, "fg_op_edm_conv: no current device");
@@ -146,8 +194,10 @@
         if (conv_prepare_all(dtype) != 0) return fail(FG_EHIP, "hipFuncSetAttribute(dynamic LDS) failed");
         prepared[dtype][dev] = true;
     }
+    if (n_targets) HIP_TRY(hipMemsetAsync(counters, 0, sizeof(unsigned) * (size_t)batch, (hipStream_t)stream));
     HIP_TRY(launch_conv_fused(dtype, ks, pro, res, outmode, a, (hipStream_t)stream));
     return FG_OK;
+}
 }
 
 int fg_op_edm_gn_finalize(const float* st1, int c1, int s1, const float* st2, int c2, int s2, const float* gamma, const float* beta, float eps,
@@ -198,6 +248,20 @@
     if (!al16(qm) || !al16(x_mid) || !al16(ab) || !al16(vmt) || !al16(bp) || !al16(out) || !al8(stats))
         return fail(FG_EINVAL, "fg_op_edm_attention_merged: tensors, ab and bp must be 16-byte aligned, stats 8-byte aligned");
     HIP_TRY(launch_attention_merged(qm, x_mid, (const float2*)ab, vmt, bp, scale, out, (float2*)stats, batch, (hipStream_t)stream));
+    return FG_OK;
+}
+
+int fg_op_edm_attention_merged_gn_tail(const float* qm, const float* x_mid, const float* ab, const float* vmt, const float* bp, float scale, float* out,
+                                       float* stats, int batch, const fg_edm_gn_target* targets, int n_targets, float eps, unsigned* counters, void* stream) {
+    if (batch <= 0 || batch > 32767) return fail(FG_EINVAL, "fg_op_edm_attention_merged_gn_tail: batch %d (1 .. 32767)", batch);
+    if (!std::isfinite(scale)) return fail(FG_EINVAL, "fg_op_edm_attention_merged_gn_tail: scale must be finite");
+    if (!qm || !x_mid || !ab || !vmt || !bp || !out) return fail(FG_EINVAL, "fg_op_edm_attention_merged_gn_tail: null pointer");
+    if (!al16(qm) || !al16(x_mid) || !al16(ab) || !al16(vmt) || !al16(bp) || !al16(out) || !al8(stats))
+        return fail(FG_EINVAL, "fg_op_edm_attention_merged_gn_tail: tensors, ab and bp must be 16-byte aligned, stats 8-byte aligned");
+    GnTail g;
+    if (const char* why = edm_gn_tail(targets, n_targets, eps, counters, stats, 256, g)) return fail(FG_EINVAL, "fg_op_edm_attention_merged_gn_tail: %s", why);
+    HIP_TRY(hipMemsetAsync(counters, 0, sizeof(unsigned) * (size_t)batch, (hipStream_t)stream));
+    HIP_TRY(launch_attention_merged(qm, x_mid, (const float2*)ab, vmt, bp, scale, out, (float2*)stats, batch, (hipStream_t)stream, &g));
     return FG_OK;
 }
 
diff --git a/fastgen_amd/csrc/gn_tail.h b/fastgen_amd/csrc/gn_tail.h
--- /dev/null
+++ b/fastgen_amd/csrc/gn_tail.h
@@ -0,0 +1,136 @@
+#pragma once
+#include <hip/hip_runtime.h>
+#include <cstddef>
+
+struct GnTarget {
+    const float* gamma;
+    const float* beta;
+    float2* ab;
+    float2* mr;
+    int c_off, C_total, hw;
+};
+struct GnTail {
+    GnTarget t[2];
+    int n = 0;
+    unsigned* cnt = nullptr;
+    float eps = 0.f;
+};
+constexpr int GN_TAIL_C = 256;
+
+inline bool gn_tail_target_ok(int c_off, int C_total) {
+    return (C_total == 256 && c_off == 0) || (C_total == 512 && (c_off == 0 || c_off == 256));
+}
+
+#ifdef __HIPCC__
+__device__ __forceinline__ void gn_slot_sum(const float2* __restrict__ st, int S, int Q, int ql, int sg, int SG, double& s, double& v2) {
+    s = 0.0, v2 = 0.0;
+    for (int sl = sg; sl < S; sl += SG) {
+        const float2 v = st[(size_t)sl * Q + ql];
+        s += v.x;
+        v2 += v.y;
+    }
+}
+
+__device__ __forceinline__ void gn_mean_rstd(double s, double v2, int cpg, int hw, float eps, float& m, float& rstd) {
+    const double cnt = (double)cpg * hw;
+    const double mean = s / cnt;
+    double var = v2 / cnt - mean * mean;
+    if (var < 0.0) var = 0.0;
+    m = (float)mean;
+    rstd = (float)(1.0 / sqrt(var + (double)eps));
+}
+
+__device__ __forceinline__ float2 gn_coeff(float m, float rstd, float gamma, float beta) {
+    const float a = rstd * gamma;
+    return make_float2(a, fmaf(-a, m, beta));
+}
+
+__device__ __forceinline__ void gn_slot_store_wt(float2* p, float s, float q) {
+    __hip_atomic_store(reinterpret_cast<unsigned long long*>(p), (unsigned long long)__float_as_uint(s) | ((unsigned long long)__float_as_uint(q) << 32),
+                       __ATOMIC_RELAXED, __HIP_MEMORY_SCOPE_AGENT);
+}
+
+constexpr int GN_TAIL_SLOTS = 32;
+template <int SG>
+__device__ __forceinline__ void gn_tail_target_sg(const GnTarget& g, float eps, const float2* __restrict__ st, int S, int n, int lane) {
+    constexpr int QPG = 16 / SG, CPG = 4 * QPG, CT = 2048 / SG;
+    float2 v[GN_TAIL_SLOTS];
+#pragma unroll
+    for (int i = 0; i < GN_TAIL_SLOTS; ++i) v[i] = st[(size_t)min(i, S - 1) * (GN_TAIL_C / 4) + lane];
+    double ps[SG], pq[SG];
+#pragma unroll
+    for (int l = 0; l < SG; ++l) {
+        ps[l] = 0.0, pq[l] = 0.0;
+#pragma unroll
+        for (int i = l; i < GN_TAIL_SLOTS; i += SG) {
+            ps[l] += i < S ? v[i].x : 0.f;
+            pq[l] += i < S ? v[i].y : 0.f;
+        }
+        __builtin_amdgcn_sched_barrier(0);
+    }
+    const int q0 = lane - lane % QPG;
+    double s = 0.0, v2 = 0.0;
+#pragma unroll
+    for (int j = 0; j < QPG; ++j) {
+#pragma unroll
+        for (int l = 0; l < SG; ++l) {
+            s += __shfl(ps[l], q0 + j);
+            v2 += __shfl(pq[l], q0 + j);
+        }
+        __builtin_amdgcn_sched_barrier(0);
+    }
+    float m, rstd;
+    int hw = g.hw;
+    asm volatile("" : "+s"(hw));
+    gn_mean_rstd(s, v2, CPG, hw, eps, m, rstd);
+    const int c = g.c_off + 4 * lane;
+    float2* o = g.ab + (size_t)n * CT + c;
+#pragma unroll
+    for (int e = 0; e < 4; ++e) o[e] = gn_coeff(m, rstd, g.gamma[c + e], g.beta[c + e]);
+    if (g.mr && c % CPG == 0) g.mr[(size_t)n * 32 + c / CPG] = make_float2(m, rstd);
+}
+__device__ __forceinline__ void gn_tail_target(const GnTarget& g, float eps, const float2* __restrict__ st, int S, int n, int lane) {
+    if (g.C_total == 256)
+        gn_tail_target_sg<8>(g, eps, st, S, n, lane);
+    else
+        gn_tail_target_sg<4>(g, eps, st, S, n, lane);
+}
+
+__device__ __forceinline__ int gn_lane() {
+    int l;
+    asm volatile("v_mbcnt_lo_u32_b32 %0, -1, 0\n\tv_mbcnt_hi_u32_b32 %0, -1, %0" : "=v"(l));
+    return l;
+}
+
+template <int KOFF>
+__device__ __forceinline__ unsigned* gn_tail_cnt() {
+    const auto ka = __builtin_amdgcn_kernarg_segment_ptr();
+    unsigned* p;
+    asm volatile("s_load_dwordx2 %0, %1, %2\n\ts_waitcnt lgkmcnt(0)" : "=s"(p) : "s"(ka), "i"(KOFF + (int)offsetof(GnTail, cnt)));
+    return p;
+}
+
+__device__ __forceinline__ bool gn_tail_arrive(unsigned* cnt, int n, unsigned total) {
+    unsigned ticket;
+    asm volatile(
+        "s_waitcnt vmcnt(0)\n\t"
+        "s_mov_b64 exec, 1\n\t"
+        "global_atomic_add %0, %1, %2, %3 sc0\n\t"
+        "s_waitcnt vmcnt(0)\n\t"
+        "s_mov_b64 exec, -1"
+        : "=&v"(ticket)
+        : "v"(0), "v"(1u), "s"(cnt + n)
+        : "memory");
+    return (unsigned)__builtin_amdgcn_readfirstlane(ticket) == total - 1;
+}
+__device__ __forceinline__ void gn_tail_acquire() {
+    __builtin_amdgcn_fence(__ATOMIC_ACQUIRE, "agent");
+    asm volatile("s_waitcnt vmcnt(0)" ::: "memory");
+}
+__device__ __forceinline__ void gn_tail_finalize(const GnTail& gt, const float2* __restrict__ stats, int S, int n) {
+    const int lane = gn_lane();
+    const float2* st = stats + (size_t)n * S * (GN_TAIL_C / 4);
+    gn_tail_target(gt.t[0], gt.eps, st, S, n, lane);
+    if (gt.n > 1) gn_tail_target(gt.t[1], gt.eps, st, S, n, lane);
+}
+#endif
diff --git a/fastgen_amd/csrc/misc.h b/fastgen_amd/csrc/misc.h
--- a/fastgen_amd/csrc/misc.h
+++ b/fastgen_amd/csrc/misc.h
@@ -1,6 +1,7 @@
 #pragma once
 #include <hip/hip_runtime.h>
 #include <stdint.h>
+#include "gn_tail.h"
 
 int launch_gn_coeffs(int dtype, const void* x1, int c1, const void* x2, int c2, const float* gamma, const float* beta,
                      float eps, float2* ab, int batch, int hw, hipStream_t s, float2* mr = nullptr);
@@ -100,7 +101,7 @@
 int launch_attention(int dtype, const void* q, const void* k, const void* vt, void* out, int B, int T, hipStream_t s);
 int launch_attn_merge_weights(const float* qkv_w, const float* qkv_b, const float* proj_w, float* w_out, float* b_out, int C, hipStream_t s);
 int launch_attention_merged(const float* qm, const float* x_mid, const float2* ab, const float* vmt, const float* bp, float scale, float* out,
-                            float2* stats, int B, hipStream_t s);
+                            float2* stats, int B, hipStream_t s, const GnTail* gn = nullptr);
 
 size_t aux_pack_elems(int C);
 int launch_pack_aux_weights(int dtype, const float* w, void* out, int C, int cout, hipStream_t s);
diff --git a/fastgen_amd/csrc/misc.hip b/fastgen_amd/csrc/misc.hip
--- a/fastgen_amd/csrc/misc.hip
+++ b/fastgen_amd/csrc/misc.hip
@@ -1,5 +1,6 @@
 #include "common.h"
 #include "misc.h"
+#include "gn_tail.h"
 
 namespace {
 
@@ -72,12 +73,8 @@
         const int S = first ? S1 : S2;
         const int Q = (first ? C1 : C2) >> 2;
         const int ql = first ? q : q - (C1 >> 2);
-        double s = 0.0, v2 = 0.0;
-        for (int sl = sg; sl < S; sl += SG) {
-            const float2 v = st[((size_t)n * S + sl) * Q + ql];
-            s += v.x;
-            v2 += v.y;
-        }
+        double s, v2;
+        gn_slot_sum(st + (size_t)n * S * Q, S, Q, ql, sg, SG, s, v2);
         ps[sg * Qt + q] = s;
         pq[sg * Qt + q] = v2;
     }
@@ -90,13 +87,9 @@
                 s += ps[l * Qt + quad];
                 v2 += pq[l * Qt + quad];
             }
-        const double cnt = (double)cpg * hw;
-        const double mean = s / cnt;
-        double var = v2 / cnt - mean * mean;
-        if (var < 0.0) var = 0.0;
-        const float m = (float)mean, rstd = (float)(1.0 / sqrt(var + (double)eps));
-        const float a = rstd * gamma[c];
-        ab[(size_t)n * C + c] = make_float2(a, fmaf(-a, m, beta[c]));
+        float m, rstd;
+        gn_mean_rstd(s, v2, cpg, hw, eps, m, rstd);
+        ab[(size_t)n * C + c] = gn_coeff(m, rstd, gamma[c], beta[c]);
         if (mr && c % cpg == 0) mr[(size_t)n * groups + g] = make_float2(m, rstd);
     }
 }
diff --git a/include/fastgen_amd.h b/include/fastgen_amd.h
--- a/include/fastgen_amd.h
+++ b/include/fastgen_amd.h
@@ -240,6 +240,20 @@
                                         void* stream);
 FG_API int fg_op_edm_attention_merged(const float* qm, const float* x_mid, const float* ab, const float* vmt, const float* bp, float scale,
                                       float* out, float* stats, int batch, void* stream);
+typedef struct fg_edm_gn_target {
+    const float* gamma;
+    const float* beta;
+    float* ab;
+    float* mr;
+    int c_off, c_total;
+} fg_edm_gn_target;
+FG_API int fg_op_edm_conv_gn_tail(int dtype, int ks, int pro, int res, const void* src1, int c1, const void* src2, int c2, int batch, int hs, int h,
+                                  const float* ab, const void* wpack, const void* wpack_ws, const float* bias, const float* temb, int temb_stride,
+                                  const void* resid, int rshift, float scale, void* out, int cout, float* stats, const fg_edm_gn_target* targets,
+                                  int n_targets, float eps, unsigned* counters, void* stream);
+FG_API int fg_op_edm_attention_merged_gn_tail(const float* qm, const float* x_mid, const float* ab, const float* vmt, const float* bp, float scale,
+                                              float* out, float* stats, int batch, const fg_edm_gn_target* targets, int n_targets, float eps,
+                                              unsigned* counters, void* stream);
 #define FG_EDM_PACK_STEM 0
 #define FG_EDM_PACK_AUX 1
 FG_API size_t fg_op_edm_head_pack_bytes(int which, int dtype, int c);
```

After: 2850 img/s. About the same (-0.9%).
